# Fadi987/PL-BERT

Measured on AMD Instinct MI355X. Metric: phoneme-tokens/sec, higher is better.
Workload: dtype bf16; 1 GPU; PL-BERT masked-phoneme training step (fwd+loss+bwd+allreduce+AdamW), ALBERT hidden 768 / 12 shared layers / FFN 2048 / 12 heads, seq_len 512, batch 32 per GPU; global_batch=32, seq_len=512, parallelism=dp1

## Files before the change

plbert_amd/_lib.py:

```python
from __future__ import annotations

import ctypes as C
import os

import torch

HERE = os.path.dirname(os.path.abspath(__file__))
LIB_PATH = os.environ.get("PLBERT_HIP_LIB") or os.path.join(HERE, "libplbert_hip.so")

PLB_PARAM_NAMES = [
    "encoder.embeddings.word_embeddings.weight",
    "encoder.embeddings.position_embeddings.weight",
    "encoder.embeddings.token_type_embeddings.weight",
    "encoder.embeddings.LayerNorm.weight",
    "encoder.embeddings.LayerNorm.bias",
    "encoder.encoder.embedding_hidden_mapping_in.weight",
    "encoder.encoder.embedding_hidden_mapping_in.bias",
    "encoder.encoder.albert_layer_groups.0.albert_layers.0.full_layer_layer_norm.weight",
    "encoder.encoder.albert_layer_groups.0.albert_layers.0.full_layer_layer_norm.bias",
    "encoder.encoder.albert_layer_groups.0.albert_layers.0.attention.query.weight",
    "encoder.encoder.albert_layer_groups.0.albert_layers.0.attention.key.weight",
    "encoder.encoder.albert_layer_groups.0.albert_layers.0.attention.value.weight",
    "encoder.encoder.albert_layer_groups.0.albert_layers.0.attention.query.bias",
    "encoder.encoder.albert_layer_groups.0.albert_layers.0.attention.key.bias",
    "encoder.encoder.albert_layer_groups.0.albert_layers.0.attention.value.bias",
    "encoder.encoder.albert_layer_groups.0.albert_layers.0.attention.dense.weight",
    "encoder.encoder.albert_layer_groups.0.albert_layers.0.attention.dense.bias",
    "encoder.encoder.albert_layer_groups.0.albert_layers.0.attention.LayerNorm.weight",
    "encoder.encoder.albert_layer_groups.0.albert_layers.0.attention.LayerNorm.bias",
    "encoder.encoder.albert_layer_groups.0.albert_layers.0.ffn.weight",
    "encoder.encoder.albert_layer_groups.0.albert_layers.0.ffn.bias",
    "encoder.encoder.albert_layer_groups.0.albert_layers.0.ffn_output.weight",
    "encoder.encoder.albert_layer_groups.0.albert_layers.0.ffn_output.bias",
    "phoneme_predictor.weight",
    "phoneme_predictor.bias",
    "encoder.pooler.weight",
    "encoder.pooler.bias",
    "token_predictor.weight",
    "token_predictor.bias",
]
PLB_NPARAM = len(PLB_PARAM_NAMES)


class PlbConfig(C.Structure):
    _fields_ = [
        ("vocab_size", C.c_int32), ("embedding_size", C.c_int32), ("hidden_size", C.c_int32),
        ("num_attention_heads", C.c_int32), ("intermediate_size", C.c_int32), ("num_hidden_layers", C.c_int32),
        ("max_position_embeddings", C.c_int32), ("type_vocab_size", C.c_int32), ("layer_norm_eps", C.c_float),
        ("num_phonemes", C.c_int32), ("num_tokens", C.c_int32), ("max_batch", C.c_int32), ("max_seq", C.c_int32),
        ("inference_only", C.c_int32),
    ]


class PlbGemmNT(C.Structure):
    _fields_ = [
        ("A", C.c_void_p), ("lda", C.c_int), ("B", C.c_void_p), ("ldb", C.c_int),
        ("M", C.c_int), ("N", C.c_int), ("K", C.c_int), ("Mstore", C.c_int),
        ("bias", C.c_void_p), ("res", C.c_void_p), ("ldr", C.c_int), ("aux", C.c_void_p), ("ldaux", C.c_int),
        ("C", C.c_void_p), ("ldc", C.c_int), ("C2", C.c_void_p), ("ldc2", C.c_int), ("Cf", C.c_void_p), ("ldcf", C.c_int),
        ("colpart", C.c_void_p),
        ("ce_cols", C.c_int), ("ce_tgt", C.c_void_p), ("ce_pmax", C.c_void_p), ("ce_psum", C.c_void_p),
        ("ce_tlogit", C.c_void_p), ("ce_lse", C.c_void_p), ("ce_w", C.c_void_p),
        ("deq_a", C.c_void_p), ("deq_b", C.c_void_p), ("C8", C.c_void_p), ("ldc8", C.c_int), ("q_scale", C.c_void_p),
        ("q_amax", C.c_void_p), ("c8_bf8", C.c_int),
        ("ln_gamma", C.c_void_p), ("ln_beta", C.c_void_p), ("ln_mean", C.c_void_p), ("ln_rstd", C.c_void_p),
        ("ln_eps", C.c_float), ("ln_xchg", C.c_void_p), ("ln_err", C.c_void_p), ("ln_fault", C.c_int),
    ]


class PlbGemmTN(C.Structure):
    _fields_ = [
        ("A", C.c_void_p), ("lda", C.c_int), ("Ncols", C.c_int), ("B", C.c_void_p), ("ldb", C.c_int),
        ("Mtot", C.c_int), ("N", C.c_int), ("K", C.c_int), ("rows_per_split", C.c_int), ("splits", C.c_int),
        ("slab", C.c_void_p), ("deq_a", C.c_void_p), ("deq_b", C.c_void_p),
    ]


class PlbAttn(C.Structure):
    _fields_ = [
        ("qkv", C.c_void_p), ("ldqkv", C.c_int), ("lengths", C.c_void_p),
        ("B", C.c_int), ("S", C.c_int), ("NH", C.c_int), ("H", C.c_int), ("scale", C.c_float),
        ("ctx", C.c_void_p), ("ldctx", C.c_int), ("lse", C.c_void_p),
        ("dctx", C.c_void_p), ("lddctx", C.c_int), ("delta", C.c_void_p), ("dqkv", C.c_void_p), ("lddqkv", C.c_int),
        ("colpart", C.c_void_p), ("colpart_accumulate", C.c_int),
        ("ctx8", C.c_void_p), ("ldctx8", C.c_int), ("ctx_scale", C.c_void_p), ("ctx_amax", C.c_void_p),
        ("dqkv8", C.c_void_p), ("lddqkv8", C.c_int), ("dqkv_scale", C.c_void_p), ("dqkv_amax", C.c_void_p),
        ("qoff", C.c_void_p), ("q", C.c_void_p), ("ldq", C.c_int), ("nq_total", C.c_int), ("dq", C.c_void_p), ("lddq", C.c_int),
        ("dq8", C.c_void_p), ("lddq8", C.c_int),
        ("row_start", C.c_void_p),
    ]


class PlbEmbed(C.Structure):
    _fields_ = [
        ("ids", C.c_void_p), ("T", C.c_int), ("S", C.c_int), ("E", C.c_int), ("V", C.c_int),
        ("word", C.c_void_p), ("pos", C.c_void_p), ("type0", C.c_void_p), ("gamma", C.c_void_p), ("beta", C.c_void_p),
        ("eps", C.c_float), ("out", C.c_void_p), ("ldo", C.c_int), ("dout", C.c_void_p), ("lddo", C.c_int),
        ("dx", C.c_void_p), ("dword", C.c_void_p), ("dpos", C.c_void_p), ("partials", C.c_void_p), ("nblocks", C.c_int),
        ("row_start", C.c_void_p), ("lengths", C.c_void_p), ("B", C.c_int), ("fill_slots", C.c_int),
    ]


class PlbPacking(C.Structure):
    _fields_ = [("row_start", C.c_void_p), ("rows", C.c_int32), ("used", C.c_int32)]


class PlbMaskedReport(C.Structure):
    _fields_ = [
        ("pred", C.c_void_p), ("rank", C.c_void_p), ("nll", C.c_void_p), ("topk_ids", C.c_void_p), ("topk_logprob", C.c_void_p),
        ("logits", C.c_void_p), ("sample_loss", C.c_void_p), ("sample_top1", C.c_void_p), ("sample_topk", C.c_void_p),
        ("totals", C.c_void_p), ("token_totals", C.c_void_p),
    ]


class PlbLayerNorm(C.Structure):
    _fields_ = [
        ("x", C.c_void_p), ("ldx", C.c_int), ("gamma", C.c_void_p), ("beta", C.c_void_p), ("eps", C.c_float),
        ("y", C.c_void_p), ("ldy", C.c_int), ("mean", C.c_void_p), ("rstd", C.c_void_p),
        ("T", C.c_int), ("H", C.c_int), ("Tzero", C.c_int),
        ("dy", C.c_void_p), ("lddy", C.c_int), ("dx", C.c_void_p), ("lddx", C.c_int),
        ("partials", C.c_void_p), ("nblocks", C.c_int), ("accumulate", C.c_int),
        ("out8", C.c_void_p), ("ld8", C.c_int), ("q_scale", C.c_void_p), ("q_amax", C.c_void_p),
    ]


class PlbMask(C.Structure):
    _fields_ = [
        ("labels", C.c_void_p), ("lengths", C.c_void_p), ("B", C.c_int), ("S", C.c_int),
        ("seed", C.c_uint64), ("step", C.c_uint32),
        ("word_pred_prob", C.c_float), ("mask_prob", C.c_float), ("replace_prob", C.c_float),
        ("mask_id", C.c_int), ("sep_id", C.c_int),
        ("masked", C.c_void_p), ("counts", C.c_void_p), ("idx_padded", C.c_void_p), ("offsets", C.c_void_p),
        ("flat", C.c_void_p),
    ]


class PlbApplyMask(C.Structure):
    _fields_ = [
        ("ids", C.c_void_p), ("sample_off", C.c_void_p), ("word_off", C.c_void_p), ("word_begin", C.c_void_p),
        ("word_len", C.c_void_p), ("action", C.c_void_p), ("repl", C.c_void_p), ("word_token", C.c_void_p),
        ("sep_token", C.c_int64), ("crop_start", C.c_void_p), ("B", C.c_int), ("S", C.c_int), ("mask_id", C.c_int),
        ("labels", C.c_void_p), ("masked", C.c_void_p), ("tokens", C.c_void_p), ("lengths_out", C.c_void_p),
        ("counts", C.c_void_p), ("idx_padded", C.c_void_p), ("offsets", C.c_void_p), ("flat", C.c_void_p),
    ]


PLB_NORM_PARTS = 1024


def norm_chunk(n):
    return (n + PLB_NORM_PARTS * 1024 - 1) // (PLB_NORM_PARTS * 1024) * 1024


def norm_chain(n):
    return 4 * (norm_chunk(n) // 1024) + 6 + 3


vp, i32, u32, i64, u64, sz, f32, f64, P = (C.c_void_p, C.c_int32, C.c_uint32, C.c_int64, C.c_uint64, C.c_size_t, C.c_float,
                                           C.c_double, C.POINTER)
PUBLIC = {
    "plb_last_error": (C.c_char_p, []),
    "plb_create": (i32, [P(PlbConfig), P(vp)]),
    "plb_destroy": (None, [vp]),
    "plb_param_layout": (i32, [vp, P(i64), P(i64), P(i64), P(i64)]),
    "plb_workspace_bytes": (i64, [vp]),
    "plb_bind": (i32, [vp, vp, vp, vp, vp, vp, i64]),
    "plb_sync_weights": (i32, [vp, vp]),
    "plb_forward": (i32, [vp, vp, vp, i32, i32, vp, vp, vp, vp]),
    "plb_pooler": (i32, [vp, vp, i32, i32, vp, vp]),
    "plb_loss_fwd_bwd": (i32, [vp, vp, vp, vp, vp, vp, i32, i32, i32, vp, vp]),
    "plb_loss_fwd": (i32, [vp, vp, vp, vp, vp, vp, vp, i32, i32, i32, vp, vp, vp]),
    "plb_loss_fwd_bwd_dual": (i32, [vp, vp, vp, vp, vp, vp, vp, i32, i32, i32, vp, vp, vp]),
    "plb_adamw_step": (i32, [vp, f64, f64, f64, f64, f64, i32, f64, vp]),
    "plb_grad_norm_floats": (i64, [vp]),
    "plb_grad_accum_bind": (i32, [vp, vp]),
    "plb_grad_accum_add": (i32, [vp, i32, vp, vp]),
    "plb_grad_norm": (i32, [vp, f64, f64, vp, i32, vp]),
    "plb_adamw_step_clipped": (i32, [vp, f64, f64, f64, f64, f64, i32, f64, vp, vp]),
    "plb_set_fp8": (i32, [vp, i32, vp]),
    "plb_fp8_state": (i32, [vp, P(i32), P(i32)]),
    "plb_fp8_stats": (i32, [vp, P(f32), P(f32), vp]),
    "plb_token_head_steps": (i32, [vp]),
    "plb_set_token_head_steps": (i32, [vp, i32]),
    "plb_comm_unique_id": (i32, [vp]),
    "plb_comm_init": (i32, [vp, vp, i32, i32]),
    "plb_comm_destroy": (i32, [vp]),
    "plb_comm_info": (i32, [vp, P(i32), P(i32), P(i32)]),
    "plb_status": (i32, [vp, P(i32)]),
    "plb_status_ex": (i32, [vp, P(i32), P(i32)]),
    "plb_poll_status": (i32, [vp, P(i32)]),
    "plb_status_export": (i32, [vp, vp, vp]),
    "plb_status_import": (i32, [vp, vp, vp]),
    "plb_last_application_rows": (i32, [vp, P(i64), P(i64)]),
    "plb_packing_plan": (i32, [vp, i32, i32, vp, P(i32), P(i32)]),
    "plb_forward_packed": (i32, [vp, vp, vp, i32, i32, P(PlbPacking), vp, vp, vp, vp]),
    "plb_loss_fwd_bwd_packed": (i32, [vp, vp, vp, vp, vp, vp, i32, i32, i32, P(PlbPacking), vp, vp]),
    "plb_loss_fwd_packed": (i32, [vp, vp, vp, vp, vp, vp, vp, i32, i32, i32, P(PlbPacking), vp, vp, vp]),
    "plb_last_call_rows": (i32, [vp, P(i64), P(i64)]),
    "plb_set_packed_dual": (i32, [vp, i32]),
    "plb_loss_fwd_bwd_dual_packed": (i32, [vp, vp, vp, vp, vp, vp, vp, i32, i32, i32, P(PlbPacking), vp, vp, vp]),
    "plb_set_packed_fp8": (i32, [vp, i32]),
    "plb_encode": (i32, [vp, vp, vp, i32, i32, P(PlbPacking), vp, vp]),
    "plb_encode_bwd": (i32, [vp, vp, vp, i32, i32, P(PlbPacking), vp, vp]),
    "plb_masked_report": (i32, [vp, vp, i32, i32, P(PlbMaskedReport), vp]),
    "plb_comm_pieces": (i32, [vp, P(i32), P(i64)]),
    "plb_broadcast_params": (i32, [vp, i32, vp]),
    "plb_set_grad_overlap": (i32, [vp, i32]),
    "plb_allreduce_grads": (i32, [vp, vp]),
    "plb_apply_mask": (i32, [vp, vp, vp, vp, vp, vp, vp, vp, i64, vp, i32, i32, i32, vp, vp, vp, vp, vp, vp, vp, vp]),
    "plb_mask_batch": (i32, [vp, vp, i32, i32, u64, u32, f32, f32, f32, i32, i32, vp, vp, vp, vp, vp]),
    "plb_profile_enable": (None, [i32]),
    "plb_profile_num_classes": (i32, []),
    "plb_profile_class_name": (C.c_char_p, [i32]),
    "plb_profile_read": (i32, [P(f64), P(i64), P(f64), P(f64)]),
    "plb_debug_skip_piece": (None, [i32]),
    "plb_debug_ln_fault": (None, [i32, i32]),
    "plb_debug_hb_audit": (i32, [vp, i32, i32]),
    "plb_debug_hb_report": (i32, [vp, P(i64), P(i32), vp, i32]),
    "plb_comm_trace": (i32, [vp, i32]),
    "plb_comm_trace_read": (i32, [vp, i32, P(i32), P(i64), P(i64), P(f32), P(f32), P(f32)]),
    "plb_set_gemm_nt_tile": (None, [i32]),
    "plb_set_gemm_nt_prefetch": (None, [i32]),
    "plb_set_attn_bwd_fused": (None, [i32]),
    "plb_set_prune_last": (None, [i32]),
}
PUBLIC_SYMBOLS = list(PUBLIC)
INTERNAL = {
    **{name: PUBLIC[name] for name in ("plb_set_gemm_nt_tile", "plb_set_gemm_nt_prefetch", "plb_debug_skip_piece",
                                       "plb_debug_ln_fault", "plb_set_attn_bwd_fused")},
    "plb_prof_begin": (i32, [i32, vp, f64, f64]),
    "plb_prof_end": (None, [i32, vp]),
    "plb_launch_gemm_nt_ln": (i32, [P(PlbGemmNT), i32, vp]),
    "plb_launch_gemm_nt_gelud": (i32, [P(PlbGemmNT), i32, vp]),
    "plb_launch_gemm_nt_fp8": (i32, [P(PlbGemmNT), i32, i32, vp]),
    "plb_launch_gemm_nt_fp8_ln": (i32, [P(PlbGemmNT), i32, i32, vp]),
    "plb_launch_gemm_nt_fp8_gelud": (i32, [P(PlbGemmNT), i32, i32, vp]),
    "plb_gemm_nt_fp8_gelud_tile_rows": (i32, [i32]),
    "plb_ln_fault_take": (i32, []),
    "plb_launch_gemm_nt": (i32, [P(PlbGemmNT), i32, i32, vp]),
    "plb_launch_gemm_nt_big": (i32, [P(PlbGemmNT), i32, i32, i32, vp]),
    "plb_gemm_nt_colpart_rows": (i32, [i32, i32, i32]),
    "plb_launch_gemm_tn": (i32, [P(PlbGemmTN), vp]),
    "plb_launch_gemm_tn_fp8": (i32, [P(PlbGemmTN), vp]),
    "plb_launch_gemm_tn_big": (i32, [P(PlbGemmTN), vp]),
    "plb_launch_reduce_slabs": (i32, [vp, i32, sz, vp, i32, vp]),
    "plb_launch_embed_fwd": (i32, [P(PlbEmbed), vp]),
    "plb_launch_embed_bwd": (i32, [P(PlbEmbed), vp]),
    "plb_launch_embed_scatter": (i32, [P(PlbEmbed), i32, vp]),
    "plb_launch_amax": (i32, [vp, i32, sz, i32, i32, vp, vp]),
    "plb_launch_fp8_scales": (i32, [vp, vp, vp, i32, f32, i32, vp]),
    "plb_launch_fp8_scales2": (i32, [vp, vp, vp, i32, f32, i32, i32, f32, vp, i32, vp]),
    "plb_launch_quantize": (i32, [vp, i32, sz, i32, i32, vp, vp, i32, i32, vp]),
    "plb_launch_quantize_multi": (i32, [i32, vp, vp, vp, vp, vp, vp, vp]),
    "plb_launch_ln_fwd": (i32, [P(PlbLayerNorm), vp]),
    "plb_launch_ln_bwd": (i32, [P(PlbLayerNorm), vp]),
    "plb_launch_colsum": (i32, [vp, i32, sz, i32, i32, vp, i32, i32, vp, i32, vp]),
    "plb_launch_copy_cols": (i32, [vp, i32, i32, i32, i32, vp, vp]),
    "plb_launch_pooler": (i32, [vp, i32, i32, i32, vp, vp, vp, vp]),
    "plb_launch_attn_fwd": (i32, [P(PlbAttn), vp]),
    "plb_launch_attn_bwd": (i32, [P(PlbAttn), vp]),
    "plb_launch_attn_bwd_fused": (i32, [P(PlbAttn), vp]),
    "plb_launch_gather_rows": (i32, [vp, i32, vp, i32, i32, i32, vp, i32, vp]),
    "plb_launch_scatter_rows": (i32, [vp, i32, vp, i32, i32, vp, i32, vp]),
    "plb_launch_ce_prepare": (i32, [vp, vp, vp, i32, i32, vp, vp, vp, vp]),
    "plb_launch_ce_prepare_packed": (i32, [vp, vp, vp, i32, i32, vp, vp, vp, vp, vp]),
    "plb_launch_unpack_rows": (i32, [vp, i32, i32, vp, vp, i32, i32, i32, vp, vp]),
    "plb_launch_seed_dy": (i32, [vp, vp, vp, i32, i32, i32, i32, vp, vp]),
    "plb_launch_ce_fwd_bwd": (i32, [vp, i32, i32, vp, vp, i32, i32, vp, vp, i32, vp]),
    "plb_launch_sum_rows": (i32, [vp, i32, vp, vp]),
    "plb_launch_token_ce_combine": (i32, [vp, vp, i32, vp, vp, i32, i32, i32, vp, vp, vp, vp]),
    "plb_launch_token_ce_combine_packed": (i32, [vp, vp, i32, vp, vp, vp, i32, i32, i32, vp, vp, vp, vp]),
    "plb_launch_pack_token_targets": (i32, [vp, vp, vp, i32, i32, i32, vp, vp]),
    "plb_launch_add_scalar": (i32, [vp, vp, vp, vp]),
    "plb_launch_masked_report_rows": (i32, [vp, i32, i32, vp, i32, i32, vp, vp, vp, vp, vp, vp, vp]),
    "plb_launch_masked_report_samples": (i32, [vp, i32, vp, vp, i32, vp, vp, vp, vp, vp]),
    "plb_launch_token_top1": (i32, [vp, i32, vp, vp, i32, vp, vp, vp]),
    "plb_launch_mask": (i32, [P(PlbMask), vp]),
    "plb_launch_apply_mask": (i32, [P(PlbApplyMask), vp]),
    "plb_launch_adamw": (i32, [vp, vp, vp, vp, vp, sz, f64, f64, f64, f64, f64, i32, f64, vp, i32, vp]),
    "plb_launch_grad_accum": (i32, [vp, vp, sz, i32, vp, vp]),
    "plb_launch_grad_sumsq": (i32, [vp, sz, vp, vp]),
    "plb_launch_grad_norm_finish": (i32, [vp, i32, f64, f64, vp, vp]),
    "plb_launch_adamw_clipped": (i32, [vp, vp, vp, vp, vp, sz, f64, f64, f64, f64, f64, i32, f64, vp, i32, vp, i32, vp]),
    "plb_launch_step_status": (i32, [vp, vp, vp, vp, vp]),
    "plb_launch_status_export": (i32, [vp, vp, vp]),
    "plb_launch_cast_bf16": (i32, [vp, vp, sz, vp]),
    "plb_launch_transpose_cast": (i32, [vp, i32, i32, vp, i32, vp]),
    "plb_launch_transpose_cast_multi": (i32, [i32, vp, vp, vp, vp, vp, vp]),
    "plb_launch_bf16_to_f32": (i32, [vp, i32, vp, i32, i32, i32, vp]),
}


def declare(L):
    for name, (restype, argtypes) in {**PUBLIC, **INTERNAL}.items():
        fn = getattr(L, name, None)
        if fn is not None:
            fn.restype, fn.argtypes = restype, list(argtypes)
    return L


_lib = None


class HipLibraryMissing(RuntimeError):
    pass


def lib():
    global _lib
    if _lib is not None:
        return _lib
    if not os.path.exists(LIB_PATH):
        raise HipLibraryMissing(
            f"{LIB_PATH} is missing: build it with `python -m plbert_amd.build` (needs hipcc, gfx950). "
            "There is no CPU fallback for the PL-BERT hot path.")
    try:
        _lib = declare(C.CDLL(LIB_PATH, mode=C.RTLD_GLOBAL))
    except OSError as ex:
        raise HipLibraryMissing(f"cannot load {LIB_PATH}: {ex}") from ex
    return _lib


def profile_enable(on):
    lib().plb_profile_enable(int(bool(on)))


def profile_read():
    L = lib()
    n = L.plb_profile_num_classes()
    ms, fl, by = (C.c_double * n)(), (C.c_double * n)(), (C.c_double * n)()
    cnt = (C.c_int64 * n)()
    check(L.plb_profile_read(ms, cnt, fl, by), "plb_profile_read")
    return {L.plb_profile_class_name(i).decode(): dict(ms=ms[i], launches=int(cnt[i]), flops=fl[i], bytes=by[i])
            for i in range(n) if cnt[i]}


def check(rc, what):
    if rc != 0:
        msg = lib().plb_last_error().decode("utf-8", "replace")
        raise RuntimeError(f"{what} failed: {msg or 'rc=%d' % rc}")
```

plbert_amd/build.py:

```python
from __future__ import annotations

import os
import subprocess
import sys

HERE = os.path.dirname(os.path.abspath(__file__))
CSRC = os.path.join(HERE, "csrc")
LIB = os.path.join(HERE, "libplbert_hip.so")
SOURCES = ["gemm.hip", "gemm_big.hip", "gemm_fp8.hip", "gemm_fp8_ln.hip", "gemm_tn_fp8.hip", "gemm_ln.hip", "attn.hip", "attn_bwd_fused.hip", "mask.hip",
           "embed.hip", "layernorm.hip", "reduce.hip", "loss_rows.hip", "eval_rows.hip", "optim.hip", "operand_images.hip",
           "engine.cpp", "engine_prof.cpp", "engine_comm.cpp", "engine_fp8.cpp", "engine_layers.cpp", "engine_calls.cpp", "engine_eval.cpp", "engine_optim.cpp"]
HEADERS = ["exports.map", "common.h", "plbert_kernels.h", "gemm_epilogue.h", "gemm_nt_pipeline.h", "attn_common.h", "row_common.h", "engine_internal.h", os.path.join("..", "..", "include", "plbert.h")]
FLAGS = ["--offload-arch=gfx950", "-O3", "-std=c++17", "-fPIC", "-Wall", "-Wno-unused-function"]
_NO_SINK = ["-mllvm", "-disable-machine-sink"]
EXTRA_FLAGS = {"attn_bwd_fused.hip": ["-mllvm", "-amdgpu-mfma-vgpr-form=1"],
               "gemm_fp8.hip": _NO_SINK, "gemm_fp8_ln.hip": _NO_SINK, "gemm_tn_fp8.hip": _NO_SINK}


def _hipcc():
    for cand in (os.environ.get("HIPCC"), "/opt/rocm/bin/hipcc", "hipcc"):
        if cand and (os.path.isabs(cand) and os.path.exists(cand) or not os.path.isabs(cand)):
            return cand
    raise RuntimeError("hipcc not found")


def needs_build():
    if not os.path.exists(LIB):
        return True
    t = os.path.getmtime(LIB)
    deps = [os.path.join(CSRC, s) for s in SOURCES + HEADERS]
    return any(os.path.getmtime(d) > t for d in deps)


OBJDUMP = "/opt/rocm/lib/llvm/bin/llvm-objdump"


def disassemble_code_objects(lib, workdir):
    import glob
    import shutil
    cp = shutil.copy(lib, workdir)
    subprocess.run([OBJDUMP, "--offloading", cp], check=True, stdout=subprocess.PIPE, stderr=subprocess.STDOUT)
    cos = sorted(glob.glob(cp + ".*gfx950"))
    if not cos:
        raise RuntimeError("no gfx950 code object extracted from " + lib)
    for co in cos:
        yield co, subprocess.run([OBJDUMP, "-d", "--no-show-raw-insn", co], check=True, stdout=subprocess.PIPE,
                                 text=True).stdout


def verify_m0(lib=LIB, workdir=None):
    import re
    import tempfile
    if not os.path.exists(OBJDUMP):
        return None
    own = workdir is None
    tmp = tempfile.mkdtemp(prefix="plbert_m0_") if own else workdir
    n_asm = 0
    try:
        for co, text in disassemble_code_objects(lib, tmp):
            funcs, cur = {}, None
            for ln in text.splitlines():
                i = ln.split("//")[0].strip()
                m = re.match(r"^[0-9a-f]+ <(.+)>:$", i)
                if m:
                    cur = funcs.setdefault(m.group(1), [])
                elif cur is not None and i and not i.endswith(":"):
                    cur.append(i)
            for name, ins in funcs.items():
                def dma(i):
                    return i.startswith("global_load_lds") or (i.startswith("buffer_load") and i.rstrip().endswith("lds"))
                sig = [k for k in range(len(ins) - 2) if re.match(r"s_mov_b32 m0, s\d+$", ins[k]) and ins[k + 1] == "s_nop 0"
                       and dma(ins[k + 2]) and " s[" in ins[k + 2]]
                for i in ins:
                    if re.match(r"(s_movrel|v_movrel|ds_gws|ds_ordered|s_sendmsg|v_interp)", i):
                        raise RuntimeError(f"M0 check: {name}: instruction that reads M0: {i}")
                    if re.search(r"\bm0\b", i):
                        if not (re.match(r"s_\w+ m0, ", i) and not re.search(r"\bm0\b", i.split(",", 1)[1])):
                            raise RuntimeError(f"M0 check: {name}: M0 used as a source: {i}")
                if not sig:
                    continue
                n_asm += len(sig)
                owned = set(sig) | {k + 2 for k in sig}
                for k, i in enumerate(ins):
                    if (dma(i) or re.search(r"\bm0\b", i)) and k not in owned:
                        raise RuntimeError(f"M0 check: {name}: M0 / LDS-DMA outside the asm DMA statements: {ins[max(0, k - 2):k + 3]}")
    finally:
        if own:
            import shutil
            shutil.rmtree(tmp, ignore_errors=True)
    return n_asm


def build(force=False, verbose=True):
    if not force and not needs_build():
        return LIB
    hipcc = _hipcc()
    objdir = os.path.join(HERE, "build")
    os.makedirs(objdir, exist_ok=True)
    procs = []
    for src in SOURCES:
        obj = os.path.join(objdir, os.path.splitext(src)[0] + ".o")
        cmd = [hipcc, *FLAGS, *EXTRA_FLAGS.get(src, []), "-x", "hip", "-c", os.path.join(CSRC, src), "-o", obj]
        procs.append((src, obj, subprocess.Popen(cmd, stdout=subprocess.PIPE, stderr=subprocess.STDOUT, text=True)))
    objs = []
    for src, obj, p in procs:
        out, _ = p.communicate()
        if p.returncode != 0:
            raise RuntimeError(f"hipcc failed on {src}:\n{out}")
        if verbose and out.strip():
            print(out, file=sys.stderr)
        objs.append(obj)
    cmd = [hipcc, "--offload-arch=gfx950", "-shared", "-fPIC", "-Wl,--version-script=" + os.path.join(CSRC, "exports.map"),
           "-o", LIB, *objs]
    r = subprocess.run(cmd, stdout=subprocess.PIPE, stderr=subprocess.STDOUT, text=True)
    if r.returncode != 0:
        raise RuntimeError("link failed:\n" + r.stdout)
    try:
        verify_m0(LIB)
    except Exception:
        os.remove(LIB)
        raise
    return LIB


if __name__ == "__main__":
    print(build(force="--force" in sys.argv))
```

plbert_amd/csrc/engine_internal.h:

```cpp
#pragma once
#include <hip/hip_runtime.h>
#include <stdint.h>
#include <stdio.h>
#include <stdlib.h>
#include <string.h>

#include <array>
#include <map>
#include <string>
#include <vector>

#include "../../include/plbert.h"
#include "plbert_kernels.h"

#pragma GCC visibility push(hidden)

int fail(const char* fmt, ...);

static const unsigned kStreamOrderEvent = hipEventDisableTiming | hipEventReleaseToDevice;

inline int64_t rup(int64_t x, int64_t m) { return (x + m - 1) / m * m; }

#define TRY(x)                                                                    \
  do {                                                                            \
    int rc_ = (x);                                                                \
    if (rc_) return fail("%s failed (rc %d) at %s:%d", #x, rc_, __FILE__, __LINE__); \
  } while (0)
#define HIPTRY(x)                                                                                   \
  do {                                                                                              \
    hipError_t e_ = (x);                                                                            \
    if (e_ != hipSuccess) return fail("%s: %s at %s:%d", #x, hipGetErrorString(e_), __FILE__, __LINE__); \
  } while (0)
#define HB_R(stream, ptr, bytes, what) do { if (e->hb.on) e->hb.access(hb_idx(e, stream), (ptr), (size_t)(bytes), false, what); } while (0)
#define HB_W(stream, ptr, bytes, what) do { if (e->hb.on) e->hb.access(hb_idx(e, stream), (ptr), (size_t)(bytes), true, what); } while (0)

typedef void* RcclComm;

struct HbAudit {
  enum { MAIN = 0, SIDE = 1, COMM = 2, NS = 3 };
  typedef std::array<uint64_t, NS> VC;
  struct Acc { const char* what; uintptr_t a, b; int st; uint64_t tick; bool wr; };
  bool on = false;
  int break_wait = -1;
  int waits = 0;
  VC vc[NS] = {{0, 0, 0}, {0, 0, 0}, {0, 0, 0}};
  std::map<hipEvent_t, VC> ev;
  std::vector<Acc> log;
  int64_t checks = 0;
  int violations = 0;
  std::string first;
  static const char* name(int st) { return st == MAIN ? "main" : st == SIDE ? "side" : "comm"; }
  void record(hipEvent_t e, int st) { vc[st][st] += 1; ev[e] = vc[st]; }
  void wait(int st, hipEvent_t e);
  void access(int st, const void* p, size_t bytes, bool wr, const char* what);
  void new_call() { log.clear(); waits = 0; }
};

struct PlbEngine {
  PlbConfig c;
  int64_t poff[PLB_NPARAM], psize[PLB_NPARAM], ptotal, ptrain;
  int E, H, I, L, NH, V, P, NP, NT;
  int64_t Tcap;
  int64_t NMcap;
  int NTp = 0;
  bool infer = false;
  int qkvcol_rows = 0;
  int64_t slab2_floats;
  int64_t slab_floats;
  int64_t ws_bytes;
  int ln_blocks, emb_blocks;
  int part_rows = 0;
  int ln_fuse = 3;
  int64_t lnx_bytes = 0;
  bool gelu_dstash_on = true;
  bool fp8_tn = true;
  int f8n = 0;
  bool packed_dual = false;
  bool packed_fp8 = false;
  int64_t o_wbf, o_wqkvT, o_wdT, o_w1T, o_w2T, o_wpT, o_winT;
  int64_t o_e, o_x, o_qkv, o_ctx, o_pre1, o_a, o_u, o_g, o_pre2;
  int64_t o_lse, o_delta, o_mean1, o_rstd1, o_mean2, o_rstd2;
  int64_t o_dqkv, o_dpre1, o_du, o_dpre2;
  int64_t o_dy0, o_dy1, o_da, o_dctx, o_de;
  int64_t o_hm, o_logm, o_dlog, o_dhm, o_rows, o_tgt, o_w, o_lrows;
  int64_t o_slab, o_part1, o_part2, o_parte, o_scratch, o_dxe, o_ducol, o_slab2, o_scratch2, o_qkvcol = 0;
  int64_t o_lnx = 0, o_lnerr = 0;
  int64_t o_rep_rank = 0, o_rep_nll = 0, o_rep_tok = 0;
  int64_t o_bt = 0, o_wtT = 0, o_tdl = 0, o_tlrows = 0, o_tscr = 0, o_tgrad = 0, o_tloss = 0;
  int64_t o_tpmax = 0, o_tpsum = 0, o_ttl = 0, o_tlse = 0, o_tw = 0, o_ttgt = 0, o_tcolp = 0;
  int64_t o_x8 = 0, o_a8 = 0, o_g8 = 0, o_c8 = 0, o_dp8 = 0, o_du8 = 0, o_dp18 = 0, o_dq8 = 0;
  int64_t o_wq8 = 0, o_wd8 = 0, o_w18 = 0, o_w28 = 0, o_w2T8 = 0, o_w1T8 = 0, o_wqT8 = 0, o_wdT8 = 0;
  int64_t o_f8amax = 0, o_f8scale = 0, o_f8deq = 0, o_f8stats = 0;
  bool fp8_on = false, fp8_ready = false, fp8_bwd_ready = false, fp8_wstale = true;
  bool u_is_derivative = false;
  bool tn8_call = false;
  int part_rows_used = 0;
  int pruned_rows = 0;
  int64_t last_app_rows[2] = {0, 0};
  int64_t last_exec_rows[2] = {0, 0};
  bool tok_grads_live = false;
  bool head_grads_live = true;
  bool tok_pad_zeroed = false;
  int tok_steps = 0;
  bool rep_valid = false, rep_dual = false;
  int rep_n = 0, rep_B = 0;
  int64_t rep_tok_rows = 0;
  float* accum = nullptr;
  bool grads_fresh = false;
  bool win_open = false;
  const char* win_closed_by = "no FIRST add has opened one";
  bool win_head = false, win_tok = false;
  bool win_reduced = false;
  const float* norm_src = nullptr;
  int norm_nparts = 0;
  bool norm_reduced = false;
  bool stash_live = false;
  const char* stash_dead_by = "no plb_encode has run on this engine";
  int stash_B = 0, stash_S = 0;
  int64_t stash_rows = 0, stash_used = 0;
  const int32_t* stash_row_start = nullptr;
  RcclComm comm = nullptr;
  int comm_rank = 0, comm_world = 1;
  hipStream_t comm_stream = nullptr;
  hipEvent_t ev_piece = nullptr, ev_comm_done = nullptr;
  bool overlap = true;
  bool comm_pending = false;
  bool grads_reduced = false;
  int64_t piece_floats = 0;
  int32_t piece_count = 0;
  hipEvent_t ev_status = nullptr;
  bool status_pending = false;
  int32_t status_collectives = 0;
  float* last_loss = nullptr;
  HbAudit hb;
  struct PieceTrace { int64_t a, b; hipEvent_t released, done; };
  bool trace_on = false;
  std::vector<PieceTrace> trace;
  std::vector<hipEvent_t> trace_pool;
  hipEvent_t tr_call0 = nullptr, tr_tail0 = nullptr, tr_tail1 = nullptr;
  bool tr_tail_valid = false;
  hipStream_t side = nullptr;
  hipEvent_t ev_fork = nullptr, ev_join = nullptr;
  unsigned int* host_err = nullptr;
  unsigned int* host_err_dev = nullptr;
  float *params = nullptr, *grads = nullptr, *m = nullptr, *v = nullptr;
  char* ws = nullptr;

  template <typename T>
  T* at(int64_t off) const { return reinterpret_cast<T*>(ws + off); }
  bf16_t* wbf(int which) const { return at<bf16_t>(o_wbf) + poff[which]; }
  float* par(int which) const { return params + poff[which]; }
  float* grd(int which) const { return grads + poff[which]; }
};

enum { F8_X = 0, F8_A, F8_G, F8_C, F8_DP, F8_DU, F8_DP1, F8_DQ, F8_NSITE };
enum { F8_AMAX_WORDS = 64 * 16 };
enum { F8W_QKV = 0, F8W_D, F8W_1, F8W_2, F8W_2T, F8W_1T, F8W_QKVT, F8W_DT, F8W_N };

struct Rows {
  const int32_t* row_start;
  int T; int64_t Tp;
};

struct F8Site {
  float* scale = nullptr;
  float* amax = nullptr;
  float* deq = nullptr;
  F8Site() = default;
  F8Site(const PlbEngine* e, int kind, int l);
};
struct F8Weight {
  const uint8_t* img;
  const float* deq;
  F8Weight(const PlbEngine* e, int w);
};

struct F8Op { const uint8_t* A8; const uint8_t* B8; const float* deq_a; const float* deq_b; int a_bf8; };

struct Slots {
  bf16_t *x, *y;
  bf16_t *qkv, *ctx, *pre1, *a, *u, *g, *pre2;
  float *mean1, *rstd1, *mean2, *rstd2, *lse;
  uint8_t *x8, *x8n, *c8, *a8, *g8;
  bf16_t *dqkv, *dpre1, *du, *dpre2;
  uint8_t *dp8, *du8, *dp18, *dq8;
  float *part1, *part2, *qkvcol, *ducol;
};

struct LnSlot { const float* gamma; const float* beta; const bf16_t* pre; float* mean; float* rstd; float* partials; };

struct Prune { const int32_t* rows; int n; int Mc; };

struct Bwd {
  const int32_t* lengths;
  const int32_t* row_start;
  int B, S, T;
  int64_t Tp;
  bool f8, calib;
  bool fuse_b;
  int prows;
  int du_rows;
  hipStream_t s;
};

enum { kPieceHead = 0, kPieceQkvW, kPieceFfnW, kPieceSmall, kPieceFfnoW = kPieceSmall + 5, kPieceDenseW, kNPieces };

int hb_idx(const PlbEngine* e, hipStream_t s);
hipError_t ev_record(PlbEngine* e, hipEvent_t ev, hipStream_t s);
hipError_t ev_wait(PlbEngine* e, hipStream_t s, hipEvent_t ev);
int reduce_piece(PlbEngine* e, int64_t a, int64_t b, hipStream_t after);
bool overlapping(const PlbEngine* e);
int pieces_done(PlbEngine* e);
int64_t piece_begin(const PlbEngine* e, int i);
int64_t piece_end(const PlbEngine* e, int i);
int reduce_pieces(PlbEngine* e, int from, int to, hipStream_t after);
int status_exchange(PlbEngine* e, hipStream_t s);
int status_finish(PlbEngine* e, float* loss, hipStream_t s);
int f8_site(const PlbEngine* e, int site, int l);
float* f8_deq(const PlbEngine* e, int i);
int fp8_quantize_weights(PlbEngine* e, hipStream_t s, bool exact = true);
int fp8_update_scales(PlbEngine* e, hipStream_t s);
bool f8_call(const PlbEngine* e, int64_t Tp, bool train);
bool tn8_ok(const PlbEngine* e, int64_t Mtot);
PlbGemmNT nt_desc(const bf16_t* A, const bf16_t* B, int64_t M, int N, int K);
int qkvcol_rows(int B, int S);
Slots slots(const PlbEngine* e, int64_t Tp, int B, int S, int l, bool stash, int prows = 0, int du_rows = 0);
bool prune_enabled();
int run_encoder(PlbEngine* e, const int64_t* ids, const int32_t* lengths, int B, int S, const Rows& rw, bool stash,
                bf16_t** xout, hipStream_t s, const Prune* pr = nullptr);
int tn_splits(int64_t Mtot, int N, int K, int* rows_per_split);
int weight_grad(PlbEngine* e, const bf16_t* A, int lda, int Ncols, const bf16_t* Bm, int ldb, int64_t Mtot, int N,
                int K, float* out, hipStream_t s, bool side_slab = false);
int weight_grad8(PlbEngine* e, const uint8_t* A8, const uint8_t* B8, int64_t Mtot, int N, int K, int site_a, int site_b,
                 float* out, hipStream_t s);
int encoder_bwd(PlbEngine* e, const Prune* pr, const int32_t* lengths, int B, int S, const Rows& rw, bf16_t** dy,
                int* du_rows, hipStream_t s);
void drop_stash(PlbEngine* e, const char* by);
int sync_transposes(PlbEngine* e, hipStream_t s, bool exact_fp8 = true);
void end_accum_window(PlbEngine* e, const char* by);

#pragma GCC visibility pop
```

plbert_amd/csrc/engine_layers.cpp:

```cpp
#include "engine_internal.h"

static bool tn_big(int64_t Mtot, int Ncols, int K) { return Ncols % 256 == 0 && K % 256 == 0 && Mtot >= 8192; }
static bool tn_fill_chip() {
  static const bool v = [] { const char* e = getenv("PLBERT_TN_SPLITS"); return !(e && !strcmp(e, "xcd")); }();
  return v;
}
static int tn_cus() {
  static const int v = [] {
    const char* e = getenv("PLBERT_TN_CUS");
    const int n = e ? atoi(e) : 256;
    return (n >= 64 && n <= 256) ? n : 256;
  }();
  return v;
}
int tn_splits(int64_t Mtot, int N, int K, int* rows_per_split) {
  const bool big = tn_big(Mtot, N, K);
  const int tiles = big ? (N / 256) * (K / 256) : ((N + 127) / 128) * ((K + 127) / 128);
  int splits = 768 / tiles;
  if (big) {
    int s = 32 / tiles;
    if (s < 1) s = 1;
    splits = tiles >= 256 ? 1 : (tn_fill_chip() ? (tn_cus() / tiles > 0 ? tn_cus() / tiles : 1) : 8 * s);
  }
  const int64_t maxs = Mtot / 64;
  if (splits > maxs) splits = (int)maxs;
  if (splits < 1) splits = 1;
  int64_t rps = rup((Mtot + splits - 1) / splits, 64);
  splits = (int)((Mtot + rps - 1) / rps);
  *rows_per_split = (int)rps;
  return splits;
}

PlbGemmNT nt_desc(const bf16_t* A, const bf16_t* B, int64_t M, int N, int K) {
  PlbGemmNT g;
  memset(&g, 0, sizeof(g));
  g.A = A; g.lda = K; g.B = B; g.ldb = K; g.M = (int)M; g.N = N; g.K = K; g.Mstore = (int)M;
  return g;
}

static F8Op f8_op(const uint8_t* a8, const F8Site& a, const F8Weight& w, int a_bf8) { return F8Op{a8, w.img, a.deq, w.deq, a_bf8}; }
static PlbGemmNT f8_operands(const PlbGemmNT* g, const F8Op* f8) {
  PlbGemmNT q = *g;
  q.A = reinterpret_cast<const bf16_t*>(f8->A8); q.B = reinterpret_cast<const bf16_t*>(f8->B8);
  q.deq_a = f8->deq_a; q.deq_b = f8->deq_b;
  return q;
}
static int gemm_nt_any(PlbGemmNT* g, int act, const F8Op* f8, hipStream_t s) {
  if (!f8) return plb_launch_gemm_nt(g, act, 0, s);
  PlbGemmNT q = f8_operands(g, f8);
  return plb_launch_gemm_nt_fp8(&q, act, f8->a_bf8, s);
}
static int gemm_nt_ln_any(PlbGemmNT* g, int mode, const F8Op* f8, hipStream_t s) {
  if (!f8) return plb_launch_gemm_nt_ln(g, mode, s);
  PlbGemmNT q = f8_operands(g, f8);
  return plb_launch_gemm_nt_fp8_ln(&q, mode, f8->a_bf8, s);
}
static int gemm_nt_gelud_any(PlbGemmNT* g, int backward, const F8Op* f8, hipStream_t s) {
  if (!f8) return plb_launch_gemm_nt_gelud(g, backward, s);
  PlbGemmNT q = f8_operands(g, f8);
  return plb_launch_gemm_nt_fp8_gelud(&q, backward, f8->a_bf8, s);
}
static void f8_out(PlbGemmNT* g, uint8_t* img, int ld, const F8Site& q, int bf8) {
  g->C8 = img; g->ldc8 = ld; g->q_scale = q.scale; g->q_amax = q.amax; g->c8_bf8 = bf8;
}

int qkvcol_rows(int B, int S) { return B * ((S + 127) / 128) * 4; }
Slots slots(const PlbEngine* e, int64_t Tp, int B, int S, int l, bool stash, int prows, int du_rows) {
  const int64_t H = e->H, I = e->I, sl = stash ? l : 0;
  auto bf = [&](int64_t off, int64_t width) { return e->at<bf16_t>(off) + sl * Tp * width; };
  auto u8 = [&](int64_t off, int64_t width) { return e->at<uint8_t>(off) + sl * Tp * width; };
  auto f32 = [&](int64_t off, int64_t per_layer) { return e->at<float>(off) + sl * per_layer; };
  Slots v;
  memset(&v, 0, sizeof(v));
  v.x = e->at<bf16_t>(e->o_x) + (int64_t)(stash ? l : l & 1) * Tp * H;
  v.y = e->at<bf16_t>(e->o_x) + (int64_t)(stash ? l + 1 : (l + 1) & 1) * Tp * H;
  v.qkv = bf(e->o_qkv, 3 * H); v.ctx = bf(e->o_ctx, H); v.pre1 = bf(e->o_pre1, H); v.a = bf(e->o_a, H);
  v.u = bf(e->o_u, I); v.g = bf(e->o_g, I); v.pre2 = bf(e->o_pre2, H);
  v.mean1 = f32(e->o_mean1, Tp); v.rstd1 = f32(e->o_rstd1, Tp); v.mean2 = f32(e->o_mean2, Tp); v.rstd2 = f32(e->o_rstd2, Tp);
  v.lse = f32(e->o_lse, (int64_t)B * e->NH * S);
  v.x8 = u8(e->o_x8, H); v.c8 = u8(e->o_c8, H); v.a8 = u8(e->o_a8, H); v.g8 = u8(e->o_g8, I);
  v.x8n = e->at<uint8_t>(e->o_x8) + (stash ? l + 1 : 0) * Tp * H;
  if (stash) {
    v.dqkv = bf(e->o_dqkv, 3 * H); v.dpre1 = bf(e->o_dpre1, H); v.du = bf(e->o_du, I); v.dpre2 = bf(e->o_dpre2, H);
    v.dp8 = u8(e->o_dp8, H); v.du8 = u8(e->o_du8, I); v.dp18 = u8(e->o_dp18, H); v.dq8 = u8(e->o_dq8, 3 * H);
    v.part1 = f32(e->o_part1, (int64_t)prows * 3 * H); v.part2 = f32(e->o_part2, (int64_t)prows * 3 * H);
    v.qkvcol = f32(e->o_qkvcol, (int64_t)qkvcol_rows(B, S) * 3 * H); v.ducol = f32(e->o_ducol, (int64_t)du_rows * I);
  }
  return v;
}

static bool ln_fusable(const PlbEngine* e, int64_t Tp, int bit) {
  const int H = e->H;
  return (e->ln_fuse & bit) && Tp % 1024 == 0 && (H % 384 == 0 ? H / 384 : H % 256 == 0 ? H / 256 : 99) <= 4;
}
static bool gelu_dstash(PlbEngine* e, int64_t Tp, bool f8_call) {
  e->u_is_derivative = e->gelu_dstash_on && (f8_call ? Tp % 128 == 0 : Tp % 256 == 0) && e->I % 256 == 0;
  return e->u_is_derivative;
}
static void ln_fields(const PlbEngine* e, PlbGemmNT* g, const float* gamma, const float* beta, float* mean, float* rstd) {
  g->ln_gamma = gamma; g->ln_beta = beta; g->ln_mean = mean; g->ln_rstd = rstd; g->ln_eps = e->c.layer_norm_eps;
  g->ln_xchg = e->at<unsigned long long>(e->o_lnx); g->ln_err = e->at<unsigned int>(e->o_lnerr);
}
static LnSlot ln1_slot(const PlbEngine* e, const Slots& v) {
  return LnSlot{e->par(PLB_LN1_W), e->par(PLB_LN1_B), v.pre1, v.mean1, v.rstd1, v.part1};
}
static LnSlot ln2_slot(const PlbEngine* e, const Slots& v) {
  return LnSlot{e->par(PLB_LN2_W), e->par(PLB_LN2_B), v.pre2, v.mean2, v.rstd2, v.part2};
}
static int gemm_ln_fwd(PlbEngine* e, PlbGemmNT* g, const F8Op* f8, bool fused, const LnSlot& ln, bf16_t* y, int T,
                       uint8_t* y8, const F8Site& q, hipStream_t s) {
  const int H = e->H;
  if (fused) {
    g->C2 = y; g->ldc2 = H;
    ln_fields(e, g, ln.gamma, ln.beta, ln.mean, ln.rstd);
    if (y8) f8_out(g, y8, H, q, 0);
    TRY(gemm_nt_ln_any(g, 5, f8, s));
    return 0;
  }
  TRY(gemm_nt_any(g, 0, f8, s));
  PlbLayerNorm p;
  memset(&p, 0, sizeof(p));
  p.x = g->C; p.ldx = H; p.gamma = ln.gamma; p.beta = ln.beta; p.eps = e->c.layer_norm_eps;
  p.y = y; p.ldy = H; p.T = T; p.H = H; p.mean = ln.mean; p.rstd = ln.rstd;
  if (y8) { p.out8 = y8; p.ld8 = H; p.q_scale = q.scale; p.q_amax = q.amax; }
  TRY(plb_launch_ln_fwd(&p, s));
  return 0;
}
static int ln_bwd(PlbEngine* e, const LnSlot& ln, int nblocks, const bf16_t* dy, bf16_t* dx, int T, int Tzero, uint8_t* dx8,
                  const F8Site& q, hipStream_t s) {
  const int H = e->H;
  PlbLayerNorm p;
  memset(&p, 0, sizeof(p));
  p.x = ln.pre; p.ldx = H; p.gamma = ln.gamma; p.T = T; p.H = H; p.Tzero = Tzero; p.mean = ln.mean; p.rstd = ln.rstd;
  p.dy = dy; p.lddy = H; p.dx = dx; p.lddx = H; p.partials = ln.partials; p.nblocks = nblocks;
  if (dx8) { p.out8 = dx8; p.ld8 = H; p.q_scale = q.scale; p.q_amax = q.amax; }
  TRY(plb_launch_ln_bwd(&p, s));
  return 0;
}
static int gemm_ln_bwd(PlbEngine* e, PlbGemmNT* g, const F8Op* f8, bool fused, const LnSlot& ln, int nblocks, bf16_t* dx, int T,
                       int Tzero, uint8_t* dx8, const F8Site& q, hipStream_t s) {
  if (fused) {
    g->C = dx; g->aux = ln.pre; g->ldaux = e->H; g->colpart = ln.partials;
    ln_fields(e, g, ln.gamma, nullptr, ln.mean, ln.rstd);
    if (dx8) f8_out(g, dx8, e->H, q, 1);
    TRY(gemm_nt_ln_any(g, 6, f8, s));
    return 0;
  }
  TRY(gemm_nt_any(g, 0, f8, s));
  return ln_bwd(e, ln, nblocks, g->C, dx, T, Tzero, dx8, q, s);
}

static int g_prune_last = -1;
extern "C" void plb_set_prune_last(int on) { g_prune_last = on < 0 ? -1 : (on ? 1 : 0); }
bool prune_enabled() {
  static const bool v = [] { const char* e = getenv("PLBERT_PRUNE_LAST"); return !(e && !strcmp(e, "0")); }();
  return g_prune_last < 0 ? v : g_prune_last != 0;
}
static int last_application_fwd_pruned(PlbEngine* e, const Prune* pr, bool stash, bool calib, bool tn8, const Slots& sl,
                                       const bf16_t* ctx_att, hipStream_t s) {
  const int H = e->H, I = e->I, L = e->L, Mc = pr->Mc, n = pr->n;
  const F8Site sA(e, F8_A, L - 1), sG(e, F8_G, L - 1), sC(e, F8_C, L - 1);
  bf16_t* ctxc = stash ? sl.ctx : sl.pre1;
  bf16_t* xc = stash ? e->at<bf16_t>(e->o_da) : sl.a;
  bf16_t* pre1c = stash ? sl.pre1 : sl.ctx;
  bf16_t* ac = stash ? sl.a : sl.pre1;
  TRY(plb_launch_gather_rows(ctx_att, H, pr->rows, n, Mc, H, ctxc, H, s));
  TRY(plb_launch_gather_rows(sl.x, H, pr->rows, n, Mc, H, xc, H, s));
  PlbGemmNT g = nt_desc(ctxc, e->wbf(PLB_DENSE_W), Mc, H, H);
  g.bias = e->par(PLB_DENSE_B); g.res = xc; g.ldr = H; g.C = pre1c; g.ldc = H;
  const LnSlot ln1 = {e->par(PLB_LN1_W), e->par(PLB_LN1_B), pre1c, sl.mean1, sl.rstd1, nullptr};
  if (gemm_ln_fwd(e, &g, nullptr, false, ln1, ac, Mc, nullptr, F8Site(), s)) return 1;
  if (calib) TRY(plb_launch_amax(ac, 1, (size_t)n, H, H, sA.amax, s));
  g = nt_desc(ac, e->wbf(PLB_FFN_W), Mc, I, H);
  g.bias = e->par(PLB_FFN_B); g.C = sl.u; g.ldc = I; g.C2 = sl.g; g.ldc2 = I;
  TRY(plb_launch_gemm_nt(&g, 1, 0, s));
  if (calib) TRY(plb_launch_amax(sl.g, 1, (size_t)n, I, I, sG.amax, s));
  g = nt_desc(sl.g, e->wbf(PLB_FFNO_W), Mc, H, I);
  g.bias = e->par(PLB_FFNO_B); g.res = ac; g.ldr = H; g.C = sl.pre2; g.ldc = H;
  if (gemm_ln_fwd(e, &g, nullptr, false, ln2_slot(e, sl), e->at<bf16_t>(e->o_hm), Mc, nullptr, F8Site(), s)) return 1;
  if (tn8) {
    const void* src[3] = {ctxc, ac, sl.g}; const int fl[3] = {1, 1, 1};
    const size_t nel[3] = {(size_t)Mc * H, (size_t)Mc * H, (size_t)Mc * I};
    const float* sc[3] = {sC.scale, sA.scale, sG.scale};
    uint8_t* dst[3] = {sl.c8, sl.a8, sl.g8};
    float* am[3] = {sC.amax, sA.amax, sG.amax};
    TRY(plb_launch_quantize_multi(3, src, fl, nel, sc, dst, am, s));
  }
  return 0;
}

int run_encoder(PlbEngine* e, const int64_t* ids, const int32_t* lengths, int B, int S, const Rows& rw, bool stash,
                       bf16_t** xout, hipStream_t s, const Prune* pr) {
  const int E = e->E, H = e->H, I = e->I, L = e->L;
  const int T = rw.T;
  const int64_t Tp = rw.Tp;
  const bool f8 = f8_call(e, Tp, stash);
  const bool calib = e->fp8_on && !f8;
  const int T8 = (f8 && rw.row_start) ? (int)Tp : T;
  if (e->fp8_on && e->fp8_wstale) TRY(fp8_quantize_weights(e, s));
  PlbEmbed em;
  memset(&em, 0, sizeof(em));
  em.ids = ids; em.T = T; em.S = S; em.E = E; em.V = e->V;
  em.word = e->par(PLB_WORD_EMB); em.pos = e->par(PLB_POS_EMB); em.type0 = e->par(PLB_TYPE_EMB);
  em.gamma = e->par(PLB_EMB_LN_W); em.beta = e->par(PLB_EMB_LN_B); em.eps = e->c.layer_norm_eps;
  em.out = e->at<bf16_t>(e->o_e); em.ldo = E;
  if (rw.row_start) {
    em.row_start = rw.row_start; em.lengths = lengths; em.B = B; em.T = (int)Tp;
    em.fill_slots = e->fp8_on;
  }
  TRY(plb_launch_embed_fwd(&em, s));

  const Slots first = slots(e, Tp, B, S, 0, stash);
  PlbGemmNT g = nt_desc(em.out, e->wbf(PLB_MAP_W), Tp, H, E);
  g.bias = e->par(PLB_MAP_B); g.C = first.x; g.ldc = H;
  TRY(plb_launch_gemm_nt(&g, 0, 0, s));
  if (f8) {
    const F8Site sX(e, F8_X, 0);
    const void* src1[1] = {first.x}; const int bf1[1] = {1}; const size_t n1[1] = {(size_t)T8 * H};
    const float* sc1[1] = {sX.scale}; uint8_t* dst1[1] = {first.x8}; float* am1[1] = {sX.amax};
    TRY(plb_launch_quantize_multi(1, src1, bf1, n1, sc1, dst1, am1, s));
  }
  const bool fuse_f = ln_fusable(e, Tp, 1);
  const bool dstash = gelu_dstash(e, Tp, f8);
  if (stash) e->tn8_call = f8 && e->fp8_tn && dstash && tn8_ok(e, (int64_t)L * Tp);
  const bool tn8 = stash && e->tn8_call;

  for (int l = 0; l < L; ++l) {
    const Slots sl = slots(e, Tp, B, S, l, stash);
    const F8Site sX(e, F8_X, l), sA(e, F8_A, l), sG(e, F8_G, l), sC(e, F8_C, l);
    if (calib) TRY(plb_launch_amax(sl.x, 1, (size_t)T, H, H, sX.amax, s));
    g = nt_desc(sl.x, e->wbf(PLB_Q_W), Tp, 3 * H, H);
    g.bias = e->par(PLB_Q_B); g.C = sl.qkv; g.ldc = 3 * H;
    const F8Op oq = f8_op(sl.x8, sX, F8Weight(e, F8W_QKV), 0);
    TRY(gemm_nt_any(&g, 0, f8 ? &oq : nullptr, s));
    PlbAttn at;
    memset(&at, 0, sizeof(at));
    at.qkv = sl.qkv; at.ldqkv = 3 * H; at.lengths = lengths; at.B = B; at.S = S; at.NH = e->NH; at.H = H;
    at.row_start = rw.row_start;
    const bool pruned_layer = pr != nullptr && l == L - 1;
    bf16_t* const ctx_att = (pruned_layer && stash) ? e->at<bf16_t>(e->o_dy1) : sl.ctx;
    at.scale = 0.125f; at.ctx = ctx_att; at.ldctx = H; at.lse = sl.lse;
    if (f8 && !pruned_layer) { at.ctx8 = sl.c8; at.ldctx8 = H; at.ctx_scale = sC.scale; at.ctx_amax = sC.amax; }
    if (rw.row_start && e->fp8_on && S % 128) {
      HIPTRY(hipMemsetAsync(ctx_att, 0, (size_t)T * H * 2, s));
      if (at.ctx8) HIPTRY(hipMemsetAsync(sl.c8, 0, (size_t)T * H, s));
    }
    TRY(plb_launch_attn_fwd(&at, s));
    if (rw.row_start && Tp > T) {
      HIPTRY(hipMemsetAsync(ctx_att + (int64_t)T * H, 0, (size_t)(Tp - T) * H * 2, s));
      if (at.ctx8) HIPTRY(hipMemsetAsync(sl.c8 + (int64_t)T * H, 0, (size_t)(Tp - T) * H, s));
    }
    if (calib) TRY(plb_launch_amax(ctx_att, 1, (size_t)T, H, H, sC.amax, s));
    if (pruned_layer) {
      if (last_application_fwd_pruned(e, pr, stash, calib, tn8, sl, ctx_att, s)) return 1;
      *xout = e->at<bf16_t>(e->o_hm);
      break;
    }
    g = nt_desc(sl.ctx, e->wbf(PLB_DENSE_W), Tp, H, H);
    g.bias = e->par(PLB_DENSE_B); g.res = sl.x; g.ldr = H; g.C = sl.pre1; g.ldc = H;
    const F8Op od = f8_op(sl.c8, sC, F8Weight(e, F8W_D), 0);
    if (gemm_ln_fwd(e, &g, f8 ? &od : nullptr, fuse_f, ln1_slot(e, sl), sl.a, T8, f8 ? sl.a8 : nullptr, sA, s)) return 1;
    if (calib) TRY(plb_launch_amax(sl.a, 1, (size_t)T, H, H, sA.amax, s));
    g = nt_desc(sl.a, e->wbf(PLB_FFN_W), Tp, I, H);
    g.bias = e->par(PLB_FFN_B); g.C = sl.u; g.ldc = I; g.C2 = sl.g; g.ldc2 = I;
    if (f8) f8_out(&g, sl.g8, I, sG, 0);
    const F8Op o1 = f8_op(sl.a8, sA, F8Weight(e, F8W_1), 0);
    if (dstash) {
      if (tn8) { g.C2 = nullptr; g.ldc2 = 0; }
      TRY(gemm_nt_gelud_any(&g, 0, f8 ? &o1 : nullptr, s));
    } else {
      TRY(gemm_nt_any(&g, 1, f8 ? &o1 : nullptr, s));
    }
    if (calib) TRY(plb_launch_amax(sl.g, 1, (size_t)T, I, I, sG.amax, s));
    g = nt_desc(sl.g, e->wbf(PLB_FFNO_W), Tp, H, I);
    g.bias = e->par(PLB_FFNO_B); g.res = sl.a; g.ldr = H; g.C = sl.pre2; g.ldc = H;
    const F8Op o2 = f8_op(sl.g8, sG, F8Weight(e, F8W_2), 0);
    const bool next8 = f8 && l + 1 < L;
    if (gemm_ln_fwd(e, &g, f8 ? &o2 : nullptr, fuse_f, ln2_slot(e, sl), sl.y, T8, next8 ? sl.x8n : nullptr,
                    next8 ? F8Site(e, F8_X, l + 1) : F8Site(), s))
      return 1;
    *xout = sl.y;
  }
  return 0;
}

int weight_grad(PlbEngine* e, const bf16_t* A, int lda, int Ncols, const bf16_t* Bm, int ldb, int64_t Mtot, int N,
                       int K, float* out, hipStream_t s, bool side_slab) {
  PlbGemmTN t;
  memset(&t, 0, sizeof(t));
  t.A = A; t.lda = lda; t.Ncols = Ncols; t.B = Bm; t.ldb = ldb; t.Mtot = (int)Mtot; t.N = N; t.K = K;
  t.splits = tn_splits(Mtot, N, K, &t.rows_per_split);
  const bool direct = t.splits == 1 && N == Ncols;
  if (!direct && (int64_t)t.splits * N * K > (side_slab ? e->slab2_floats : e->slab_floats)) return fail("weight_grad: slab too small");
  t.slab = direct ? out : e->at<float>(side_slab ? e->o_slab2 : e->o_slab);
  if (N == Ncols && tn_big(Mtot, Ncols, K)) {
    const int tok = plb_prof_begin(PLB_K_GEMM_TN, s, 2.0 * (double)Mtot * N * K, 0.0);
    TRY(plb_launch_gemm_tn_big(&t, s));
    plb_prof_end(tok, s);
  } else {
    TRY(plb_launch_gemm_tn(&t, s));
  }
  if (!direct) TRY(plb_launch_reduce_slabs(t.slab, t.splits, (size_t)N * K, out, 0, s));
  return 0;
}

int weight_grad8(PlbEngine* e, const uint8_t* A8, const uint8_t* B8, int64_t Mtot, int N, int K, int site_a, int site_b,
                        float* out, hipStream_t s) {
  PlbGemmTN t;
  memset(&t, 0, sizeof(t));
  t.A = reinterpret_cast<const bf16_t*>(A8); t.lda = N; t.Ncols = N; t.B = reinterpret_cast<const bf16_t*>(B8); t.ldb = K;
  t.Mtot = (int)Mtot; t.N = N; t.K = K;
  t.splits = tn_splits(Mtot, N, K, &t.rows_per_split);
  t.rows_per_split = (int)rup(t.rows_per_split, 128);
  t.splits = (int)((Mtot + t.rows_per_split - 1) / t.rows_per_split);
  if ((int64_t)t.splits * N * K > e->slab_floats) return fail("weight_grad8: slab too small");
  t.slab = e->at<float>(e->o_slab);
  t.deq_a = f8_deq(e, f8_site(e, site_a, 0)); t.deq_b = f8_deq(e, f8_site(e, site_b, 0));
  const int tok = plb_prof_begin(PLB_K_GEMM_TN_FP8, s, 2.0 * (double)Mtot * N * K, 0.0);
  TRY(plb_launch_gemm_tn_fp8(&t, s));
  plb_prof_end(tok, s);
  TRY(plb_launch_reduce_slabs(t.slab, t.splits, (size_t)N * K, out, 0, s));
  return 0;
}

static int post_attention_bwd(PlbEngine* e, const Bwd& c, int l, const Slots& sl, const bf16_t* dy) {
  const int H = e->H, I = e->I, T = c.T, Tp = (int)c.Tp;
  hipStream_t s = c.s;
  const F8Site sDP(e, F8_DP, l), sDU(e, F8_DU, l), sDP1(e, F8_DP1, l);
  if (l == e->L - 1 && ln_bwd(e, ln2_slot(e, sl), c.prows, dy, sl.dpre2, T, Tp, c.f8 ? sl.dp8 : nullptr, sDP, s)) return 1;
  if (c.calib) TRY(plb_launch_amax(sl.dpre2, 1, (size_t)T, H, H, sDP.amax, s));
  PlbGemmNT g = nt_desc(sl.dpre2, e->at<bf16_t>(e->o_w2T), Tp, I, H);
  g.aux = sl.u; g.ldaux = I; g.C = sl.du; g.ldc = I;
  if (c.du_rows > 0) g.colpart = sl.ducol;
  if (c.f8) f8_out(&g, sl.du8, I, sDU, 1);
  const F8Op ou = f8_op(sl.dp8, sDP, F8Weight(e, F8W_2T), 1);
  if (e->u_is_derivative) {
    if (e->tn8_call) g.C = nullptr;
    TRY(gemm_nt_gelud_any(&g, 1, c.f8 ? &ou : nullptr, s));
  } else {
    TRY(gemm_nt_any(&g, 2, c.f8 ? &ou : nullptr, s));
  }
  if (c.calib) TRY(plb_launch_amax(sl.du, 1, (size_t)T, I, I, sDU.amax, s));
  g = nt_desc(sl.du, e->at<bf16_t>(e->o_w1T), Tp, H, I);
  g.res = sl.dpre2; g.ldr = H; g.C = e->at<bf16_t>(e->o_da); g.ldc = H;
  const F8Op oa = f8_op(sl.du8, sDU, F8Weight(e, F8W_1T), 1);
  if (gemm_ln_bwd(e, &g, c.f8 ? &oa : nullptr, c.fuse_b, ln1_slot(e, sl), c.prows, sl.dpre1, T, Tp, c.f8 ? sl.dp18 : nullptr,
                  sDP1, s))
    return 1;
  if (c.calib) TRY(plb_launch_amax(sl.dpre1, 1, (size_t)T, H, H, sDP1.amax, s));
  g = nt_desc(sl.dpre1, e->at<bf16_t>(e->o_wdT), Tp, H, H);
  g.C = e->at<bf16_t>(e->o_dctx); g.ldc = H;
  const F8Op oc = f8_op(sl.dp18, sDP1, F8Weight(e, F8W_DT), 1);
  TRY(gemm_nt_any(&g, 0, c.f8 ? &oc : nullptr, s));
  return 0;
}

static int last_application_bwd_pruned(PlbEngine* e, const Bwd& c, const Slots& sl, const Prune* pr) {
  const int H = e->H, I = e->I, L = e->L, Mc = pr->Mc, n = pr->n;
  hipStream_t s = c.s;
  const F8Site sDP(e, F8_DP, L - 1), sDU(e, F8_DU, L - 1), sDP1(e, F8_DP1, L - 1);
  bf16_t* const dac = e->at<bf16_t>(e->o_da);
  bf16_t* const dctxc = e->at<bf16_t>(e->o_dy0);
  bf16_t* const dctx = e->at<bf16_t>(e->o_dctx);
  if (ln_bwd(e, ln2_slot(e, sl), c.prows, e->at<bf16_t>(e->o_dhm), sl.dpre2, Mc, Mc, nullptr, F8Site(), s)) return 1;
  if (c.calib) TRY(plb_launch_amax(sl.dpre2, 1, (size_t)n, H, H, sDP.amax, s));
  PlbGemmNT g = nt_desc(sl.dpre2, e->at<bf16_t>(e->o_w2T), Mc, I, H);
  g.aux = sl.u; g.ldaux = I; g.C = sl.du; g.ldc = I;
  TRY(plb_launch_gemm_nt(&g, 2, 0, s));
  if (c.calib) TRY(plb_launch_amax(sl.du, 1, (size_t)n, I, I, sDU.amax, s));
  if (c.du_rows > 0) {
    TRY(plb_launch_colsum(sl.du, 1, (size_t)Mc, I, I, sl.ducol, I, 0, e->at<float>(e->o_scratch), 16, s));
    if (c.du_rows > 1) HIPTRY(hipMemsetAsync(sl.ducol + I, 0, (size_t)(c.du_rows - 1) * I * 4, s));
  }
  g = nt_desc(sl.du, e->at<bf16_t>(e->o_w1T), Mc, H, I);
  g.res = sl.dpre2; g.ldr = H; g.C = dac; g.ldc = H;
  if (gemm_ln_bwd(e, &g, nullptr, false, ln1_slot(e, sl), c.prows, sl.dpre1, Mc, Mc, nullptr, F8Site(), s)) return 1;
  if (c.calib) TRY(plb_launch_amax(sl.dpre1, 1, (size_t)n, H, H, sDP1.amax, s));
  if (e->tn8_call) {
    const void* src[3] = {sl.dpre2, sl.du, sl.dpre1}; const int fl[3] = {3, 3, 3};
    const size_t nel[3] = {(size_t)Mc * H, (size_t)Mc * I, (size_t)Mc * H};
    const float* sc[3] = {sDP.scale, sDU.scale, sDP1.scale};
    uint8_t* dst[3] = {sl.dp8, sl.du8, sl.dp18};
    float* am[3] = {sDP.amax, sDU.amax, sDP1.amax};
    TRY(plb_launch_quantize_multi(3, src, fl, nel, sc, dst, am, s));
  }
  g = nt_desc(sl.dpre1, e->at<bf16_t>(e->o_wdT), Mc, H, H);
  g.C = dctxc; g.ldc = H;
  TRY(plb_launch_gemm_nt(&g, 0, 0, s));
  HIPTRY(hipMemsetAsync(dctx, 0, (size_t)c.Tp * H * 2, s));
  TRY(plb_launch_scatter_rows(dctxc, H, pr->rows, n, H, dctx, H, s));
  HIPTRY(hipMemsetAsync(dac, 0, (size_t)c.Tp * H * 2, s));
  TRY(plb_launch_scatter_rows(sl.dpre1, H, pr->rows, n, H, dac, H, s));
  return 0;
}

static int attention_bwd_dx(PlbEngine* e, const Bwd& c, int l, const Slots& sl, bf16_t* ctx, const bf16_t* res,
                            bf16_t* dx) {
  const int H = e->H, T = c.T;
  hipStream_t s = c.s;
  const F8Site sDQ(e, F8_DQ, l);
  PlbAttn at;
  memset(&at, 0, sizeof(at));
  at.qkv = sl.qkv; at.ldqkv = 3 * H; at.lengths = c.lengths; at.B = c.B; at.S = c.S; at.NH = e->NH; at.H = H; at.scale = 0.125f;
  at.row_start = c.row_start;
  at.ctx = ctx; at.ldctx = H; at.lse = sl.lse;
  at.dctx = e->at<bf16_t>(e->o_dctx); at.lddctx = H; at.delta = e->at<float>(e->o_delta); at.dqkv = sl.dqkv; at.lddqkv = 3 * H;
  at.colpart = sl.qkvcol; at.colpart_accumulate = 0;
  if (c.f8) {
    at.dqkv8 = sl.dq8; at.lddqkv8 = 3 * H; at.dqkv_scale = sDQ.scale; at.dqkv_amax = sDQ.amax;
    if (e->tn8_call) at.dqkv = nullptr;
  }
  if (c.row_start && c.S % 128 && at.dqkv) HIPTRY(hipMemsetAsync(sl.dqkv, 0, (size_t)T * 3 * H * 2, s));
  if (c.row_start && c.S % 128 && at.dqkv8) HIPTRY(hipMemsetAsync(sl.dq8, 0, (size_t)T * 3 * H, s));
  TRY(plb_launch_attn_bwd(&at, s));
  if (c.Tp > T) {
    if (at.dqkv) HIPTRY(hipMemsetAsync(sl.dqkv + (int64_t)T * 3 * H, 0, (size_t)(c.Tp - T) * 3 * H * 2, s));
    if (c.f8) HIPTRY(hipMemsetAsync(sl.dq8 + (int64_t)T * 3 * H, 0, (size_t)(c.Tp - T) * 3 * H, s));
  }
  if (c.calib) TRY(plb_launch_amax(sl.dqkv, 1, (size_t)T, 3 * H, 3 * H, sDQ.amax, s));
  PlbGemmNT g = nt_desc(sl.dqkv, e->at<bf16_t>(e->o_wqkvT), c.Tp, H, 3 * H);
  g.res = res; g.ldr = H; g.C = dx; g.ldc = H;
  const F8Op ox = f8_op(sl.dq8, sDQ, F8Weight(e, F8W_QKVT), 1);
  if (l == 0) {
    TRY(gemm_nt_any(&g, 0, c.f8 ? &ox : nullptr, s));
    return 0;
  }
  const Slots below = slots(e, c.Tp, c.B, c.S, l - 1, true, c.prows, c.du_rows);
  return gemm_ln_bwd(e, &g, c.f8 ? &ox : nullptr, c.fuse_b, ln2_slot(e, below), c.prows, below.dpre2, T, (int)c.Tp,
                     c.f8 ? below.dp8 : nullptr, F8Site(e, F8_DP, l - 1), s);
}

int encoder_bwd(PlbEngine* e, const Prune* pr, const int32_t* lengths, int B, int S, const Rows& rw, bf16_t** dy,
                       int* du_rows, hipStream_t s) {
  const int I = e->I, L = e->L;
  Bwd c;
  c.lengths = lengths; c.row_start = rw.row_start; c.B = B; c.S = S; c.T = rw.T; c.Tp = rw.Tp; c.s = s;
  const int Tp = (int)c.Tp;
  c.f8 = f8_call(e, Tp, true);
  c.calib = e->fp8_on && !c.f8;
  c.du_rows = e->u_is_derivative ? (c.f8 ? 2 * (Tp / plb_gemm_nt_fp8_gelud_tile_rows(Tp)) : 2 * (Tp / 256))
                                 : (c.f8 ? 2 * (Tp / 128) : plb_gemm_nt_colpart_rows(Tp, I, e->H));
  c.fuse_b = ln_fusable(e, Tp, 2);
  c.prows = c.fuse_b ? 2 * Tp / 128 : e->ln_blocks;
  e->part_rows_used = c.prows;
  bf16_t* dx = e->at<bf16_t>(e->o_dy1);
  for (int l = L - 1; l >= 0; --l) {
    const Slots sl = slots(e, c.Tp, B, S, l, true, c.prows, c.du_rows);
    if (pr && l == L - 1) {
      if (last_application_bwd_pruned(e, c, sl, pr)) return 1;
      if (attention_bwd_dx(e, c, l, sl, e->at<bf16_t>(e->o_dy1), e->at<bf16_t>(e->o_da), dx)) return 1;
    } else {
      if (post_attention_bwd(e, c, l, sl, *dy)) return 1;
      if (attention_bwd_dx(e, c, l, sl, sl.ctx, sl.dpre1, dx)) return 1;
    }
    bf16_t* tmp = *dy; *dy = dx; dx = tmp;
  }
  *du_rows = c.du_rows;
  return 0;
}
```

plbert_amd/csrc/gemm.hip:

```cpp
#include "common.h"
#include "plbert_kernels.h"
#include "gemm_epilogue.h"

namespace {

constexpr int BM = 128, BN = 128, BK = 64;

DEVI int nt_lds_off(int row, int chunk) { return row * BK + ((chunk ^ ((row >> 1) & 7)) << 3); }

template <int ACT, bool OUTF32>
__global__ __launch_bounds__(256) void gemm_nt_kernel(PlbGemmNT p) {
  __shared__ __attribute__((aligned(16))) bf16_t smem[2][2][BM * BK];
  const int tid = threadIdx.x, lane = tid & 63, wave = tid >> 6;
  const int wr = wave >> 1, wc = wave & 1;
  const int nbn = (p.N + BN - 1) / BN;
  const int nwg = gridDim.x;
  const int logical = xcd_remap(blockIdx.x, nwg);
  const int bm = logical / nbn, bn = logical % nbn;

  const int uw = __builtin_amdgcn_readfirstlane(wave);
  const int drow = lane >> 3, dch = lane & 7;
  const bf16_t* gA = p.A + (size_t)(bm * BM + uw * 32 + drow) * p.lda;
  const bf16_t* gB = p.B + (size_t)(bn * BN + uw * 32 + drow) * p.ldb;
  const size_t sa = (size_t)8 * p.lda, sb = (size_t)8 * p.ldb;
  int sch[4];
#pragma unroll
  for (int i = 0; i < 4; ++i) sch[i] = (dch ^ ((4 * i + (lane >> 4)) & 7)) * 8;
  typedef __attribute__((address_space(1))) const void* gptr_t;
  typedef __attribute__((address_space(3))) void* lptr_t;
#define NT_STAGE(st, kt)                                                                              \
  do {                                                                                                \
    _Pragma("unroll") for (int i = 0; i < 4; ++i) {                                                   \
      __builtin_amdgcn_global_load_lds((gptr_t)(gA + i * sa + (size_t)(kt) * BK + sch[i]),            \
                                       (lptr_t)&smem[st][0][(uw * 32 + i * 8) * BK], 16, 0, 0);       \
      __builtin_amdgcn_global_load_lds((gptr_t)(gB + i * sb + (size_t)(kt) * BK + sch[i]),            \
                                       (lptr_t)&smem[st][1][(uw * 32 + i * 8) * BK], 16, 0, 0);       \
    }                                                                                                 \
  } while (0)
#define NT_LANDED() asm volatile("s_waitcnt vmcnt(0)" ::: "memory")

  f32x4 acc[4][4];
#pragma unroll
  for (int i = 0; i < 4; ++i)
#pragma unroll
    for (int j = 0; j < 4; ++j) acc[i][j] = f32x4{0.f, 0.f, 0.f, 0.f};

  const int frow = lane & 15, fq = lane >> 4;
  const int fsw = (frow >> 1) & 7;
  const int offA = (wr * 64 + frow) * BK, offB = (wc * 64 + frow) * BK;
#define NT_COMPUTE(st)                                                                                   \
  do {                                                                                                   \
    const bf16_t* sA = smem[st][0];                                                                      \
    const bf16_t* sB = smem[st][1];                                                                      \
    _Pragma("unroll") for (int kk = 0; kk < 2; ++kk) {                                                   \
      const int ch = ((kk * 4 + fq) ^ fsw) << 3;                                                         \
      bf16x8 af[4], bfr[4];                                                                              \
      _Pragma("unroll") for (int i = 0; i < 4; ++i) {                                                    \
        af[i] = *(const bf16x8*)&sA[offA + i * 16 * BK + ch];                                            \
        bfr[i] = *(const bf16x8*)&sB[offB + i * 16 * BK + ch];                                           \
      }                                                                                                  \
      _Pragma("unroll") for (int mi = 0; mi < 4; ++mi)                                                   \
        _Pragma("unroll") for (int ni = 0; ni < 4; ++ni)                                                 \
          acc[mi][ni] = __builtin_amdgcn_mfma_f32_16x16x32_bf16(bfr[ni], af[mi], acc[mi][ni], 0, 0, 0);  \
    }                                                                                                    \
  } while (0)

  const int nk = p.K / BK;
  NT_STAGE(0, 0);
  NT_LANDED();
  __syncthreads();
  for (int kt = 0; kt < nk; ++kt) {
    const int cur = kt & 1;
    if (kt + 1 < nk) NT_STAGE(cur ^ 1, kt + 1);
    NT_COMPUTE(cur);
    NT_LANDED();
    __syncthreads();
  }
#undef NT_STAGE
#undef NT_LANDED
#undef NT_COMPUTE

#pragma unroll
  for (int mi = 0; mi < 4; ++mi) {
    const int m = bm * BM + wr * 64 + mi * 16 + frow;
#pragma unroll
    for (int ni = 0; ni < 4; ++ni)
      nt_epilogue<ACT, OUTF32>(p, acc[mi][ni], m, bn * BN + wc * 64 + ni * 16 + fq * 4);
  }
}

DEVI int tn_unit(int t) { return (t & 3) | (((t >> 3) & 1) << 2) | (((t >> 2) & 1) << 3) | (t & 48); }
DEVI int tn_lds_off(int t, int col) {
  int s = col >> 4;
  return s * 1024 + (((tn_unit(t) + s) & 63) << 4) + (col & 15);
}

__global__ __launch_bounds__(256) void gemm_tn_kernel(PlbGemmTN p) {
  __shared__ __attribute__((aligned(16))) bf16_t smem[2][2][64 * 128];
  const int tid = threadIdx.x, lane = tid & 63, wave = tid >> 6;
  const int wn = wave >> 1, wk = wave & 1;
  const int nbk = (p.K + 127) / 128;
  const int bn = blockIdx.x / nbk, bk = blockIdx.x % nbk;
  const int split = blockIdx.y;
  const int t_begin = split * p.rows_per_split;
  int t_end = t_begin + p.rows_per_split;
  if (t_end > p.Mtot) t_end = p.Mtot;
  const int nt = (t_end - t_begin) / 64;

  const int lc = tid & 15, lr = tid >> 4;
  const int colA = bn * 128 + lc * 8, colB = bk * 128 + lc * 8;
  const bool okA = colA < p.Ncols, okB = colB < p.K;
  uint4 ra[4], rb[4];
  auto load_tile = [&](int it) {
    const size_t t0 = (size_t)t_begin + (size_t)it * 64 + lr;
#pragma unroll
    for (int i = 0; i < 4; ++i) {
      ra[i] = okA ? *(const uint4*)(p.A + (t0 + 16 * i) * p.lda + colA) : make_uint4(0, 0, 0, 0);
      rb[i] = okB ? *(const uint4*)(p.B + (t0 + 16 * i) * p.ldb + colB) : make_uint4(0, 0, 0, 0);
    }
  };
  auto store_tile = [&](int st) {
#pragma unroll
    for (int i = 0; i < 4; ++i) {
      int off = tn_lds_off(lr + 16 * i, lc * 8);
      *(uint4*)&smem[st][0][off] = ra[i];
      *(uint4*)&smem[st][1][off] = rb[i];
    }
  };

  f32x4 acc[4][4];
#pragma unroll
  for (int i = 0; i < 4; ++i)
#pragma unroll
    for (int j = 0; j < 4; ++j) acc[i][j] = f32x4{0.f, 0.f, 0.f, 0.f};

  const int g = lane >> 4, li = lane & 15, q = li >> 2, pp = li & 3;
  if (nt > 0) {
    load_tile(0);
    store_tile(0);
  }
  __syncthreads();
  for (int it = 0; it < nt; ++it) {
    const int cur = it & 1;
    if (it + 1 < nt) load_tile(it + 1);
    const bf16_t* sA = smem[cur][0];
    const bf16_t* sB = smem[cur][1];
#pragma unroll
    for (int ks = 0; ks < 2; ++ks) {
      const int t0 = ks * 32 + 8 * g + q;
      bf16x8 af[4], bfr[4];
#pragma unroll
      for (int i = 0; i < 4; ++i) {
        const int ca = wn * 64 + i * 16 + 4 * pp, cb = wk * 64 + i * 16 + 4 * pp;
        s16x4 a0 = lds_read_tr16(&sA[tn_lds_off(t0, ca)]);
        s16x4 a1 = lds_read_tr16(&sA[tn_lds_off(t0 + 4, ca)]);
        s16x4 b0 = lds_read_tr16(&sB[tn_lds_off(t0, cb)]);
        s16x4 b1 = lds_read_tr16(&sB[tn_lds_off(t0 + 4, cb)]);
        af[i] = bf16x8{a0[0], a0[1], a0[2], a0[3], a1[0], a1[1], a1[2], a1[3]};
        bfr[i] = bf16x8{b0[0], b0[1], b0[2], b0[3], b1[0], b1[1], b1[2], b1[3]};
      }
#pragma unroll
      for (int ni = 0; ni < 4; ++ni)
#pragma unroll
        for (int ki = 0; ki < 4; ++ki)
          acc[ni][ki] = __builtin_amdgcn_mfma_f32_16x16x32_bf16(bfr[ki], af[ni], acc[ni][ki], 0, 0, 0);
    }
    if (it + 1 < nt) store_tile(cur ^ 1);
    __syncthreads();
  }

  float* out = p.slab + (size_t)split * p.N * p.K;
#pragma unroll
  for (int ni = 0; ni < 4; ++ni) {
    const int n = bn * 128 + wn * 64 + ni * 16 + li;
    if (n >= p.N) continue;
#pragma unroll
    for (int ki = 0; ki < 4; ++ki) {
      const int k0 = bk * 128 + wk * 64 + ki * 16 + 4 * g;
      if (k0 >= p.K) continue;
      f32x4 v = acc[ni][ki];
      *(float4*)(out + (size_t)n * p.K + k0) = make_float4(v[0], v[1], v[2], v[3]);
    }
  }
}

}

static int g_nt_tile = 0;
extern "C" void plb_set_gemm_nt_tile(int tile) { g_nt_tile = tile; }

static int pick_tile(const PlbGemmNT* p) {
  const bool ok256 = p->M % 256 == 0 && p->N % 256 == 0, ok384 = p->M % 128 == 0 && p->N % 384 == 0;
  const bool ok1256 = p->M % 128 == 0 && p->N % 256 == 0;
  if (g_nt_tile == 128) return 128;
  if (g_nt_tile == 256) return ok256 ? 256 : 128;
  if (g_nt_tile == 384) return ok384 ? 384 : (ok256 ? 256 : 128);
  if (g_nt_tile == 1256) return ok1256 ? 1256 : 128;
  if ((long)p->M * p->N < 256L * 256 * 64) return 128;
  double e256 = 0, e384 = 0, e1256 = 0;
  if (ok256) { const long t = (long)(p->M / 256) * (p->N / 256); e256 = (double)t / (double)(((t + 255) / 256) * 256); }
  if (ok384) { const long t = (long)(p->M / 128) * (p->N / 384); e384 = 0.95 * (double)t / (double)(((t + 255) / 256) * 256); }
  if (ok1256) { const long t = (long)(p->M / 128) * (p->N / 256); e1256 = 0.85 * (double)t / (double)(((t + 255) / 256) * 256); }
  if (e256 == 0 && e384 == 0 && e1256 == 0) return 128;
  if (e1256 > e256 && e1256 > e384) return 1256;
  return e384 > e256 ? 384 : 256;
}

extern "C" int plb_gemm_nt_colpart_rows(int M, int N, int K) {
  PlbGemmNT q;
  q.M = M; q.N = N; q.K = K;
  const int tile = pick_tile(&q);
  return tile == 256 ? 2 * (M / 256) : (tile == 384 || tile == 1256) ? 2 * (M / 128) : 0;
}

extern "C" int plb_launch_gemm_nt(const PlbGemmNT* p, int act, int out_f32, hipStream_t stream) {
  if (p->M % BM || p->K % BK || p->N % 4 || p->M <= 0 || p->N <= 0 || p->K <= 0) return 1;
  const int nbn = (p->N + BN - 1) / BN;
  dim3 grid((p->M / BM) * nbn), block(256);
  const int cls = out_f32 ? PLB_K_GEMM_NT_F32 : act == 1 ? PLB_K_GEMM_NT_GELU : act == 2 ? PLB_K_GEMM_NT_GELUBWD : PLB_K_GEMM_NT;
  const int tile = pick_tile(p);
  if (p->colpart && tile == 128) return 1;
  const double mnk = (double)p->M * p->N * p->K;
  const double algo_bytes = 2.0 * ((double)p->M * p->K + (double)p->N * p->K) +
                            (double)p->M * p->N * (out_f32 ? 4 : act == 1 ? 4 : 2) +
                            (p->res ? 2.0 * p->M * p->N : 0.0) + (act == 2 ? 2.0 * p->M * p->N : 0.0);
  if (tile != 128) {
    const int tokb = plb_prof_begin(cls, stream, 2.0 * mnk, algo_bytes);
    const int rc = plb_launch_gemm_nt_big(p, tile, act, out_f32, stream);
    plb_prof_end(tokb, stream);
    return rc;
  }
  const int tok = plb_prof_begin(out_f32 ? PLB_K_GEMM_NT_F32 : PLB_K_GEMM_NT_SMALL, stream, 2.0 * mnk, algo_bytes);
  if (out_f32) {
    if (act != 0) return 1;
    hipLaunchKernelGGL((gemm_nt_kernel<0, true>), grid, block, 0, stream, *p);
  } else if (act == 0) {
    hipLaunchKernelGGL((gemm_nt_kernel<0, false>), grid, block, 0, stream, *p);
  } else if (act == 1) {
    hipLaunchKernelGGL((gemm_nt_kernel<1, false>), grid, block, 0, stream, *p);
  } else if (act == 2) {
    hipLaunchKernelGGL((gemm_nt_kernel<2, false>), grid, block, 0, stream, *p);
  } else {
    return 1;
  }
  plb_prof_end(tok, stream);
  return hipGetLastError() == hipSuccess ? 0 : 2;
}

extern "C" int plb_launch_gemm_tn(const PlbGemmTN* p, hipStream_t stream) {
  if (p->Mtot % 64 || p->rows_per_split % 64 || p->K % 4 || p->N <= 0 || p->splits <= 0) return 1;
  if ((long)p->splits * p->rows_per_split < p->Mtot) return 1;
  dim3 grid(((p->N + 127) / 128) * ((p->K + 127) / 128), p->splits), block(256);
  const int tok = plb_prof_begin(PLB_K_GEMM_TN, stream, 2.0 * p->Mtot * (double)p->N * p->K,
                                 2.0 * p->Mtot * ((double)p->N + p->K) + 4.0 * p->splits * (double)p->N * p->K);
  hipLaunchKernelGGL(gemm_tn_kernel, grid, block, 0, stream, *p);
  plb_prof_end(tok, stream);
  return hipGetLastError() == hipSuccess ? 0 : 2;
}
```

plbert_amd/csrc/gemm_big.hip:

```cpp
#include "gemm_nt_pipeline.h"

namespace {

template <int V, bool PF>
int launch_big(const PlbGemmNT* p, int act, int out_f32, hipStream_t stream) {
  constexpr int TM = (V == 2 ? 2 : 1) * 128, TN = (V == 3 ? 3 : 2) * 128;
  if (p->M % TM || p->N % TN || p->K % 64 || p->M <= 0 || p->N <= 0 || p->K <= 0) return 1;
  dim3 grid((p->M / TM) * (p->N / TN)), block(512);
  if (out_f32) {
    if (act != 0) return 1;
    hipLaunchKernelGGL((gemm_nt_big_kernel<V, 0, true, PF>), grid, block, 0, stream, *p);
  } else if (act == 0) {
    if (p->colpart) hipLaunchKernelGGL((gemm_nt_big_kernel<V, 0, false, PF>), grid, block, 0, stream, *p);
    else hipLaunchKernelGGL((gemm_nt_big_kernel<V, 0, false, PF, false, false, true>), grid, block, 0, stream, *p);
  } else if (act == 1) {
    hipLaunchKernelGGL((gemm_nt_big_kernel<V, 1, false, PF>), grid, block, 0, stream, *p);
  } else if (act == 2) {
    hipLaunchKernelGGL((gemm_nt_big_kernel<V, 2, false, PF>), grid, block, 0, stream, *p);
  } else if (act == 3 || act == 4) {
    if constexpr (TN == 256) {
      if (!p->ce_tgt || p->ce_cols < 1 || p->ce_cols > p->N) return 1;
      if (act == 3) {
        if (!p->ce_pmax || !p->ce_psum || !p->ce_tlogit) return 1;
        hipLaunchKernelGGL((gemm_nt_big_kernel<V, 3, false, PF>), grid, block, 0, stream, *p);
      } else {
        if (!p->ce_lse || !p->ce_w || !p->C) return 1;
        hipLaunchKernelGGL((gemm_nt_big_kernel<V, 4, false, PF>), grid, block, 0, stream, *p);
      }
    } else {
      return 1;
    }
  } else {
    return 1;
  }
  return hipGetLastError() == hipSuccess ? 0 : 2;
}

DEVI int tn_g(int row) { return ((row >> 1) & 1) | (((row >> 3) & 1) << 1); }

__global__ __launch_bounds__(512) __attribute__((amdgpu_num_vgpr(224))) void gemm_tn_big_kernel(PlbGemmTN p) {
  __shared__ __attribute__((aligned(16))) bf16_t smem[2 * 4 * HT];
  const int tid = threadIdx.x, lane = tid & 63;
  const int uw = __builtin_amdgcn_readfirstlane(tid >> 6);
  const int wm = uw >> 2, wn = uw & 3;
  const int nbk = p.K >> 8;
  const int tiles = (p.Ncols >> 8) * nbk;
  const int logical = xcd_remap(blockIdx.x, gridDim.x);
  const int split = logical / tiles, tile = logical % tiles;
  const int bn = tile / nbk, bk = tile % nbk;
  const int t_begin = split * p.rows_per_split;
  int t_end = t_begin + p.rows_per_split;
  if (t_end > p.Mtot) t_end = p.Mtot;
  const int nk = (t_end - t_begin) >> 6;

  const int i0 = 2 * uw, i1 = 2 * uw + 1;
  const int r0 = (i0 & 7) * 8 + (lane >> 3), r1 = (i1 & 7) * 8 + (lane >> 3);
  const int sc0 = (((lane & 7) ^ (2 * tn_g(r0))) * 8) + (i0 >> 3) * 64;
  const int sc1 = (((lane & 7) ^ (2 * tn_g(r1))) * 8) + (i1 >> 3) * 64;
  const int dst0 = (i0 >> 3) * 4096 + (i0 & 7) * 8 * 64, dst1 = (i1 >> 3) * 4096 + (i1 & 7) * 8 * 64;
  const int fg = lane >> 4, li = lane & 15, q4 = li >> 2, p4 = li & 3;
  const int gsw = 2 * (((q4 >> 1) & 1) | ((fg & 1) << 1));
  const int rowbase = (8 * fg + q4) * 64 + (p4 & 1) * 4;
  int aoff[4], boff[2];
#pragma unroll
  for (int mi = 0; mi < 4; ++mi) aoff[mi] = wm * 4096 + rowbase + (((2 * mi + (p4 >> 1)) ^ gsw) << 3);
#pragma unroll
  for (int ni = 0; ni < 2; ++ni)
    boff[ni] = (wn >> 1) * 4096 + rowbase + (((4 * (wn & 1) + 2 * ni + (p4 >> 1)) ^ gsw) << 3);
  const unsigned lds0 = (unsigned)(size_t)&smem[0];
#define FRAG(r, kk) (bf16x8{r[2 * (kk)][0], r[2 * (kk)][1], r[2 * (kk)][2], r[2 * (kk)][3],              \
                            r[2 * (kk) + 1][0], r[2 * (kk) + 1][1], r[2 * (kk) + 1][2], r[2 * (kk) + 1][3]})

  f32x4 acc[2][4][2][2];
#pragma unroll
  for (int a = 0; a < 2; ++a)
#pragma unroll
    for (int b = 0; b < 4; ++b)
#pragma unroll
      for (int c = 0; c < 2; ++c)
#pragma unroll
        for (int d = 0; d < 2; ++d) acc[a][b][c][d] = f32x4{0.f, 0.f, 0.f, 0.f};
#ifndef TN_DBG
#define TN_DBG 0
#endif
#if TN_DBG
  unsigned long long tnw_ = 0, tnq_ = 0;
#define TN_W0() tnq_ = __builtin_readcyclecounter()
#define TN_W1() tnw_ += __builtin_readcyclecounter() - tnq_
#else
#define TN_W0()
#define TN_W1()
#endif
#define LANDED(more)                                                      \
  do {                                                                    \
    TN_W0();                                                              \
    if (more) asm volatile("s_waitcnt vmcnt(6)" ::: "memory");            \
    else asm volatile("s_waitcnt vmcnt(0)" ::: "memory");                 \
    TN_W1();                                                              \
  } while (0)

  s16x4 ra1[4][4], rb2[2][2][4];
#define TR1(dst, addr, OFF) dst = lds_read_tr16_addr((addr) + (OFF))
#define RD4(dst, ad_, o_)   \
  do { TR1(dst[0], ad_, (o_)); TR1(dst[1], ad_, (o_) + 512); TR1(dst[2], ad_, (o_) + 4096); TR1(dst[3], ad_, (o_) + 4608); PIN(); } while (0)
#define RA4(buf, h, mi) RD4(ra1[mi], abase[buf][mi], (h) * 16384)
#define RB4(bb, buf, h, ni) RD4(rb2[bb][ni], bbase[buf][ni], (2 + (h)) * 16384)
#define SA_(h, kt) ((const char*)p.A + ((size_t)(t_begin + (kt) * 64) * p.lda + bn * 256 + (h) * 128) * 2)
#define SB_(h, kt) ((const char*)p.B + ((size_t)(t_begin + (kt) * 64) * p.ldb + bk * 256 + (h) * 128) * 2)
#define STG_A(buf, h, kt)                                                                     \
  do {                                                                                        \
    const char* sb_ = SA_(h, kt);                                                             \
    DMA16(sb_, vA0, ldsb + (((buf) * 4 + (h)) * HT + dst0) * 2);                              \
    DMA16(sb_, vA1, ldsb + (((buf) * 4 + (h)) * HT + dst1) * 2);                              \
    PIN();                                                                                    \
  } while (0)
#define STG_B(buf, h, kt)                                                                     \
  do {                                                                                        \
    const char* sb_ = SB_(h, kt);                                                             \
    DMA16(sb_, vB0, ldsb + (((buf) * 4 + 2 + (h)) * HT + dst0) * 2);                          \
    DMA16(sb_, vB1, ldsb + (((buf) * 4 + 2 + (h)) * HT + dst1) * 2);                          \
    PIN();                                                                                    \
  } while (0)
  const uint32_t vA0 = (uint32_t)(r0 * p.lda + sc0) * 2, vA1 = (uint32_t)(r1 * p.lda + sc1) * 2;
  const uint32_t vB0 = (uint32_t)(r0 * p.ldb + sc0) * 2, vB1 = (uint32_t)(r1 * p.ldb + sc1) * 2;
  const uint32_t ldsb = LDS_ADDR(&smem[0]);
  unsigned abase[2][4], bbase[2][2];
#pragma unroll
  for (int bf = 0; bf < 2; ++bf) {
#pragma unroll
    for (int mi = 0; mi < 4; ++mi) abase[bf][mi] = lds0 + 65536u * bf + 2u * aoff[mi];
#pragma unroll
    for (int ni = 0; ni < 2; ++ni) bbase[bf][ni] = lds0 + 65536u * bf + 2u * boff[ni];
  }
#define PO_(pc) ((pc) == 0 ? 0 : (pc) == 1 ? 512 : (pc) == 2 ? 4096 : 4608)
#define RA1(buf, h, mi, pc) do { TR1(ra1[mi][pc], abase[buf][mi], (h) * 16384 + PO_(pc)); PIN(); } while (0)
#define RB1(bb, buf, h, ni, pc) do { TR1(rb2[bb][ni][pc], bbase[buf][ni], (2 + (h)) * 16384 + PO_(pc)); PIN(); } while (0)
#define MF1(mh, nh, bb, j)                                                                                      \
  do {                                                                                                          \
    acc[mh][(j) >> 2][nh][(j) & 1] = __builtin_amdgcn_mfma_f32_16x16x32_bf16(                                   \
        FRAG(rb2[bb][(j) & 1], ((j) >> 1) & 1), FRAG(ra1[(j) >> 2], ((j) >> 1) & 1), acc[mh][(j) >> 2][nh][(j) & 1], 0, 0, 0); \
    PIN();                                                                                                      \
  } while (0)
#define PH1(mh, nh, bb, s0, s1, s2, s3, s4, s5, s6, s7, s8, s9, s10, s11, s12, s13, s14, s15)                    \
  do {                                                                                                          \
    BARRIER(); PIN();                                                                                           \
    MF1(mh, nh, bb, 0); s0; MF1(mh, nh, bb, 1); s1; MF1(mh, nh, bb, 2); s2; MF1(mh, nh, bb, 3); s3;             \
    MF1(mh, nh, bb, 4); s4; MF1(mh, nh, bb, 5); s5; MF1(mh, nh, bb, 6); s6; MF1(mh, nh, bb, 7); s7;             \
    MF1(mh, nh, bb, 8); s8; MF1(mh, nh, bb, 9); s9; MF1(mh, nh, bb, 10); s10; MF1(mh, nh, bb, 11); s11;         \
    MF1(mh, nh, bb, 12); s12; MF1(mh, nh, bb, 13); s13; MF1(mh, nh, bb, 14); s14; MF1(mh, nh, bb, 15); s15;     \
  } while (0)
#define NOP_ (void)0
#define TWO(x, y) do { x; y; } while (0)
#define TN_STEP(bb)                                                                                             \
  do {                                                                                                          \
    constexpr int b = (bb);  \
    const bool n1 = t + 1 < nk, n2 = t + 2 < nk;                                                                \
                                  \
    PH1(0, 0, bb, RA1(b, 0, 3, 0), RA1(b, 0, 3, 1), RA1(b, 0, 3, 2), RA1(b, 0, 3, 3),                           \
        RB1(1 - bb, b, 1, 0, 0), RB1(1 - bb, b, 1, 0, 1), RB1(1 - bb, b, 1, 0, 2), RB1(1 - bb, b, 1, 0, 3),     \
        RB1(1 - bb, b, 1, 1, 0), RB1(1 - bb, b, 1, 1, 1), RB1(1 - bb, b, 1, 1, 2), RB1(1 - bb, b, 1, 1, 3),     \
        TWO(if (n1) STG_A(b ^ 1, 1, t + 1), NOP_), NOP_, NOP_, NOP_);                                           \
                              \
    PH1(0, 1, 1 - bb, NOP_, NOP_, NOP_, NOP_, RA1(b, 1, 0, 0), RA1(b, 1, 0, 1), RA1(b, 1, 0, 2), RA1(b, 1, 0, 3), \
        RA1(b, 1, 1, 0), RA1(b, 1, 1, 1), RA1(b, 1, 1, 2), RA1(b, 1, 1, 3),                                     \
        RA1(b, 1, 2, 0), RA1(b, 1, 2, 1), RA1(b, 1, 2, 2), TWO(RA1(b, 1, 2, 3), TWO(if (n2) STG_A(b, 0, t + 2), NOP_))); \
                                                                             \
    PH1(1, 1, 1 - bb, RA1(b, 1, 3, 0), RA1(b, 1, 3, 1), RA1(b, 1, 3, 2), RA1(b, 1, 3, 3),                       \
        TWO(if (n2) STG_B(b, 0, t + 2), NOP_), NOP_, NOP_, NOP_, TWO(if (n2) STG_B(b, 1, t + 2), NOP_), NOP_, NOP_, NOP_, \
        NOP_, NOP_, NOP_, NOP_);                                                                                \
    LANDED(n2);                                                                                                 \
                    \
    PH1(1, 0, bb, RB1(1 - bb, b ^ 1, 0, 0, 0), RB1(1 - bb, b ^ 1, 0, 0, 1), RB1(1 - bb, b ^ 1, 0, 0, 2),        \
        RB1(1 - bb, b ^ 1, 0, 0, 3),                                                                            \
        TWO(RA1(b ^ 1, 0, 0, 0), RB1(1 - bb, b ^ 1, 0, 1, 0)), TWO(RA1(b ^ 1, 0, 0, 1), RB1(1 - bb, b ^ 1, 0, 1, 1)), \
        TWO(RA1(b ^ 1, 0, 0, 2), RB1(1 - bb, b ^ 1, 0, 1, 2)), TWO(RA1(b ^ 1, 0, 0, 3), RB1(1 - bb, b ^ 1, 0, 1, 3)), \
        RA1(b ^ 1, 0, 1, 0), RA1(b ^ 1, 0, 1, 1), RA1(b ^ 1, 0, 1, 2), RA1(b ^ 1, 0, 1, 3),                     \
        RA1(b ^ 1, 0, 2, 0), RA1(b ^ 1, 0, 2, 1), RA1(b ^ 1, 0, 2, 2), RA1(b ^ 1, 0, 2, 3));                    \
  } while (0)
  if (nk > 0) {
    STG_A(0, 0, 0); STG_B(0, 0, 0); STG_B(0, 1, 0); STG_A(0, 1, 0);
    if (nk > 1) { STG_A(1, 0, 1); STG_B(1, 0, 1); STG_B(1, 1, 1); }
    LANDED(nk > 1);
  }
  BARRIER();
#if TN_DBG
  tnw_ = 0;
  const unsigned long long tn_c0 = __builtin_readcyclecounter(), tn_r0 = __builtin_amdgcn_s_memrealtime();
#endif
  if (nk > 0) {
    RA4(0, 0, 0); RA4(0, 0, 1); RA4(0, 0, 2); RB4(0, 0, 0, 0); RB4(0, 0, 0, 1);
    int t = 0;
    while (true) {
      TN_STEP(0);
      if (++t >= nk) break;
      TN_STEP(1);
      if (++t >= nk) break;
    }
    BARRIER();
  }
#if TN_DBG
  if ((blockIdx.x == 17 || blockIdx.x == 130) && lane == 0 && (uw == 0 || uw == 5)) {
    const unsigned long long dc = __builtin_readcyclecounter() - tn_c0, dr = __builtin_amdgcn_s_memrealtime() - tn_r0;
    printf("TN blk %d wave %d: %d K-tiles, %.3f us per K-tile, %.0f MHz, vmcnt wait %.1f %% of the loop\n", (int)blockIdx.x, uw, nk,
           (double)dr / 100.0 / nk, (double)dc / ((double)dr / 100.0), 100.0 * (double)tnw_ / (double)dc);
  }
#endif
#undef TN_STEP
#undef TWO
#undef NOP_
#undef PH1
#undef MF1
#undef RA1
#undef RB1
#undef PO_
#undef RA4
#undef RB4
#undef RD4
#undef TR1
#undef STG_A
#undef STG_B
#undef SA_
#undef SB_
#undef FRAG
#undef LANDED

  float* out = p.slab + (size_t)split * p.N * p.K;
  int lane_e = (int)__builtin_amdgcn_mbcnt_hi(~0u, __builtin_amdgcn_mbcnt_lo(~0u, 0u));
  asm volatile("" : "+v"(lane_e));
  const int li_e = lane_e & 15, fg_e = lane_e >> 4;
#pragma unroll
  for (int mh = 0; mh < 2; ++mh)
#pragma unroll
    for (int mi = 0; mi < 4; ++mi) {
      const int n = bn * 256 + mh * 128 + wm * 64 + mi * 16 + li_e;
      if (n >= p.N) continue;
#pragma unroll
      for (int nh = 0; nh < 2; ++nh)
#pragma unroll
        for (int ni = 0; ni < 2; ++ni) {
          const int k0 = bk * 256 + nh * 128 + wn * 32 + ni * 16 + 4 * fg_e;
          const f32x4 v = acc[mh][mi][nh][ni];
          *(float4*)(out + (size_t)n * p.K + k0) = make_float4(v[0], v[1], v[2], v[3]);
        }
    }
}

}

extern "C" int plb_launch_gemm_tn_big(const PlbGemmTN* p, hipStream_t stream) {
  if (p->Ncols % 256 || p->K % 256 || p->rows_per_split % 64 || p->Mtot % 64 || p->splits <= 0) return 1;
  if ((long)p->splits * p->rows_per_split < p->Mtot) return 1;
  dim3 grid((p->Ncols / 256) * (p->K / 256) * p->splits), block(512);
  hipLaunchKernelGGL(gemm_tn_big_kernel, grid, block, 0, stream, *p);
  return hipGetLastError() == hipSuccess ? 0 : 2;
}

static int g_nt_prefetch = -1;
extern "C" void plb_set_gemm_nt_prefetch(int on) { g_nt_prefetch = on; }

extern "C" int plb_launch_gemm_nt_big(const PlbGemmNT* p, int tile, int act, int out_f32, hipStream_t stream) {
  const bool pf = g_nt_prefetch < 0 ? (tile != 256 || act != 0) : (g_nt_prefetch != 0);
  if (pf)
    return tile == 384 ? launch_big<3, true>(p, act, out_f32, stream)
           : tile == 1256 ? launch_big<1, true>(p, act, out_f32, stream) : launch_big<2, true>(p, act, out_f32, stream);
  return tile == 384 ? launch_big<3, false>(p, act, out_f32, stream)
         : tile == 1256 ? launch_big<1, false>(p, act, out_f32, stream) : launch_big<2, false>(p, act, out_f32, stream);
}
```

plbert_amd/csrc/gemm_ln.hip:

```cpp
#include "gemm_nt_pipeline.h"

static int g_ln_fault_mode = 0, g_ln_fault_launches = 0;
extern "C" void plb_debug_ln_fault(int mode, int launches) { g_ln_fault_mode = mode; g_ln_fault_launches = launches; }
extern "C" int plb_ln_fault_take(void) {
  if (g_ln_fault_launches <= 0) return 0;
  --g_ln_fault_launches;
  return g_ln_fault_mode;
}

extern "C" int plb_launch_gemm_nt_ln(const PlbGemmNT* p_in, int mode, hipStream_t stream) {
  PlbGemmNT q_ = *p_in;
  q_.ln_fault = plb_ln_fault_take();
  const PlbGemmNT* p = &q_;
  if (const int rc = ln_launch_check(p, mode, 64)) return rc;
  const int tile = p->N % 384 == 0 ? 384 : 256;
  dim3 grid((p->M / 128) * (p->N / tile)), block(512);
  const double mnk = (double)p->M * p->N * p->K;
  const double bytes = 2.0 * ((double)p->M * p->K + (double)p->N * p->K) + (double)p->M * p->N * (mode == 5 ? 4 : 4) +
                       (p->res ? 2.0 * p->M * p->N : 0.0);
  const int tok = plb_prof_begin(mode == 5 ? PLB_K_GEMM_NT_LNFWD : PLB_K_GEMM_NT_LNBWD, stream, 2.0 * mnk, bytes);
  if (tile == 384) {
    if (mode == 5) hipLaunchKernelGGL((gemm_nt_big_kernel<3, 5, false, true>), grid, block, 0, stream, *p);
    else hipLaunchKernelGGL((gemm_nt_big_kernel<3, 6, false, true>), grid, block, 0, stream, *p);
  } else {
    if (mode == 5) hipLaunchKernelGGL((gemm_nt_big_kernel<1, 5, false, true>), grid, block, 0, stream, *p);
    else hipLaunchKernelGGL((gemm_nt_big_kernel<1, 6, false, true>), grid, block, 0, stream, *p);
  }
  plb_prof_end(tok, stream);
  return hipGetLastError() == hipSuccess ? 0 : 2;
}

extern "C" int plb_launch_gemm_nt_gelud(const PlbGemmNT* p, int backward, hipStream_t stream) {
  if (p->M % 256 || p->N % 256 || p->K % 64 || p->M <= 0 || p->N <= 0 || p->K <= 0) return 3;
  if (!p->C || (!backward && !p->C2) || (backward && !p->aux)) return 1;
  dim3 grid((p->M / 256) * (p->N / 256)), block(512);
  const double mnk = (double)p->M * p->N * p->K;
  const double bytes = 2.0 * ((double)p->M * p->K + (double)p->N * p->K) + 4.0 * p->M * p->N;
  const int tok = plb_prof_begin(backward ? PLB_K_GEMM_NT_GELUBWD : PLB_K_GEMM_NT_GELU, stream, 2.0 * mnk, bytes);
  if (backward) hipLaunchKernelGGL((gemm_nt_big_kernel<2, 8, false, true>), grid, block, 0, stream, *p);
  else if (p->colpart) hipLaunchKernelGGL((gemm_nt_big_kernel<2, 7, false, true>), grid, block, 0, stream, *p);
  else hipLaunchKernelGGL((gemm_nt_big_kernel<2, 7, false, true, false, false, true>), grid, block, 0, stream, *p);
  plb_prof_end(tok, stream);
  return hipGetLastError() == hipSuccess ? 0 : 2;
}
```

plbert_amd/csrc/gemm_nt_pipeline.h:

```cpp
#pragma once
#include <type_traits>
#include "common.h"
#include "plbert_kernels.h"
#include "gemm_epilogue.h"

#ifndef NT_DBG
#define NT_DBG 0
#endif
typedef unsigned int u32x4nt __attribute__((ext_vector_type(4)));
template <bool NT>
DEVI void out_store(bf16_t* ptr, std::conditional_t<NT, const uint4, const uint4&> v) {
  if constexpr (NT) __builtin_nontemporal_store(u32x4nt{v.x, v.y, v.z, v.w}, (u32x4nt*)ptr);
  else *(uint4*)ptr = v;
}

typedef int i32x4v __attribute__((ext_vector_type(4)));
typedef int i32x8v __attribute__((ext_vector_type(8)));
template <bool ABF8>
DEVI f32x4 mfma_fp8(const i32x8v& bv, const i32x8v& av, const f32x4& c) {
  return __builtin_amdgcn_mfma_scale_f32_16x16x128_f8f6f4(bv, av, c, 0, ABF8 ? 1 : 0, 0, 0x7F7F7F7F, 0, 0x7F7F7F7F);
}
template <int HALF>
DEVI void set_half(i32x8v& v, const i32x4v t) {
  v[4 * HALF + 0] = t[0]; v[4 * HALF + 1] = t[1]; v[4 * HALF + 2] = t[2]; v[4 * HALF + 3] = t[3];
}

namespace {

constexpr int HT = 128 * 64;
constexpr int RING = 10;
DEVI int ring_slot(int x) { return x >= 2 * RING ? x - 2 * RING : (x >= RING ? x - RING : x); }

typedef __attribute__((address_space(1))) const void* gptr_t;
typedef __attribute__((address_space(3))) void* lptr_t;

#define BARRIER()                                        \
  do {                                                   \
    __builtin_amdgcn_s_waitcnt(0xC07F);                  \
    asm volatile("s_barrier" ::: "memory");              \
  } while (0)
#define PIN() __builtin_amdgcn_sched_barrier(0)

template <int V, int ACT, bool OUTF32, bool PF, bool FP8 = false, bool ABF8 = false, bool NOCS = false>
__global__ __launch_bounds__(512) void gemm_nt_big_kernel(PlbGemmNT p) {
  constexpr int NAH = (V == 2) ? 2 : 1;
  constexpr int NBH = (V == 3) ? 3 : 2;
  constexpr int TM = NAH * 128, TN = NBH * 128;
  constexpr int NH = NAH + NBH;
  __shared__ __attribute__((aligned(16))) bf16_t smem[RING * HT];
  int tid = threadIdx.x, lane = tid & 63;
  const int uw = __builtin_amdgcn_readfirstlane(tid >> 6);
  const int wm = uw >> 2, wn = uw & 3;
  const int nbn = p.N / TN;
  int bm, bn;
  if constexpr (ACT == 5 || ACT == 6) {
    const int xcd = blockIdx.x & 7, slot = blockIdx.x >> 3, gpx = (p.M / TM) >> 3;
    bm = xcd * gpx + slot / nbn; bn = slot % nbn;
  } else {
    const int logical = xcd_remap(blockIdx.x, gridDim.x);
    bm = logical / nbn; bn = logical % nbn;
  }
  constexpr int EPK = FP8 ? 128 : 64;
  const int nk = p.K / EPK;
#if NT_DBG & 16
  const unsigned long long dbg_c0 = __builtin_readcyclecounter(), dbg_r0 = __builtin_amdgcn_s_memrealtime();
#endif
#if NT_DBG & 32
  unsigned long long st_[6];
  st_[0] = __builtin_amdgcn_s_memrealtime();
#endif

  const int drow = lane >> 3;
  constexpr int EB = FP8 ? 1 : 2;
  const int ch0 = ((lane & 7) ^ ((lane >> 4) & 7)) * 16;
  const int ch1 = ((lane & 7) ^ ((4 + (lane >> 4)) & 7)) * 16;
  const uint32_t vA0 = (uint32_t)(((2 * uw) * 8 + drow) * p.lda * EB + ch0), vA1 = (uint32_t)(((2 * uw + 1) * 8 + drow) * p.lda * EB + ch1);
  const uint32_t vB0 = (uint32_t)(((2 * uw) * 8 + drow) * p.ldb * EB + ch0), vB1 = (uint32_t)(((2 * uw + 1) * 8 + drow) * p.ldb * EB + ch1);
  const char* const sA_ = (const char*)p.A + (size_t)(bm * TM) * p.lda * EB;
  const char* const sB_ = (const char*)p.B + (size_t)(bn * TN) * p.ldb * EB;
  const size_t hA = (size_t)128 * p.lda * EB, hB = (size_t)128 * p.ldb * EB;
  const int dst0 = (2 * uw) * 8 * 64, dst1 = (2 * uw + 1) * 8 * 64;
  const uint32_t ldsb_ = LDS_ADDR(&smem[0]);
#define STAGE_A(slot, h, kt)                                                                                  \
  do {                                                                                                        \
    const char* b_ = sA_ + (h) * hA + (size_t)(kt) * 128;                                                     \
    DMA16(b_, vA0, ldsb_ + 2u * ((slot) * HT + dst0));                                                        \
    DMA16(b_, vA1, ldsb_ + 2u * ((slot) * HT + dst1));                                                        \
  } while (0)
#define STAGE_B(slot, h, kt)                                                                                  \
  do {                                                                                                        \
    const char* b_ = sB_ + (h) * hB + (size_t)(kt) * 128;                                                     \
    DMA16(b_, vB0, ldsb_ + 2u * ((slot) * HT + dst0));                                                        \
    DMA16(b_, vB1, ldsb_ + 2u * ((slot) * HT + dst1));                                                        \
  } while (0)
#define STAGE_I(i, slot, kt)                                              \
  do {                                                                    \
    if (V == 2 && (i) == 3) STAGE_A(slot, 1, kt);                         \
    else if ((i) == 0) STAGE_A(slot, 0, kt);                              \
    else STAGE_B(slot, (i) - 1, kt);                                      \
  } while (0)
#define ISSUE(c)                                                          \
  do {                                                                    \
    if (NH * t + (c) < htot) STAGE_I((c) % NH, ring_slot(rb + (c)), t + (c) / NH); \
  } while (0)

  int frow = lane & 15, fq = lane >> 4;
  const int fsw = (frow >> 1) & 7;
  const int offA = (wm * 64 + frow) * 64, offB = (wn * 32 + frow) * 64;
  const int c0 = ((0 + fq) ^ fsw) << 3, c1 = ((4 + fq) ^ fsw) << 3;
  bf16x8 afr[2][4][2], bfr[2][2][2];
  i32x8v afr8[2][4], bfr8[2][2];
#define READ_A(ab, slot)                                                             \
  do {                                                                               \
    const bf16_t* s_ = &smem[(slot) * HT + offA];                                    \
    if constexpr (FP8) _Pragma("unroll") for (int mi = 0; mi < 4; ++mi) {            \
      set_half<0>(afr8[ab][mi], *(const i32x4v*)&s_[mi * 16 * 64 + c0]);             \
      set_half<1>(afr8[ab][mi], *(const i32x4v*)&s_[mi * 16 * 64 + c1]);             \
    } else _Pragma("unroll") for (int mi = 0; mi < 4; ++mi) {                        \
      afr[ab][mi][0] = *(const bf16x8*)&s_[mi * 16 * 64 + c0];                       \
      afr[ab][mi][1] = *(const bf16x8*)&s_[mi * 16 * 64 + c1];                       \
    }                                                                                \
  } while (0)
#define READ_B(bb, slot)                                                             \
  do {                                                                               \
    const bf16_t* s_ = &smem[(slot) * HT + offB];                                    \
    if constexpr (FP8) _Pragma("unroll") for (int ni = 0; ni < 2; ++ni) {            \
      set_half<0>(bfr8[bb][ni], *(const i32x4v*)&s_[ni * 16 * 64 + c0]);             \
      set_half<1>(bfr8[bb][ni], *(const i32x4v*)&s_[ni * 16 * 64 + c1]);             \
    } else _Pragma("unroll") for (int ni = 0; ni < 2; ++ni) {                        \
      bfr[bb][ni][0] = *(const bf16x8*)&s_[ni * 16 * 64 + c0];                       \
      bfr[bb][ni][1] = *(const bf16x8*)&s_[ni * 16 * 64 + c1];                       \
    }                                                                                \
  } while (0)

  f32x4 acc[NAH][4][NBH][2];
#pragma unroll
  for (int a = 0; a < NAH; ++a)
#pragma unroll
    for (int b = 0; b < 4; ++b)
#pragma unroll
      for (int c = 0; c < NBH; ++c)
#pragma unroll
        for (int d = 0; d < 2; ++d) acc[a][b][c][d] = f32x4{0.f, 0.f, 0.f, 0.f};
#define MFMA_Q(mh, nh, ab, bb)                                                                                 \
  do {                                                                                                         \
    if constexpr (FP8) {                                                                                       \
      _Pragma("unroll") for (int mi = 0; mi < 4; ++mi)                                                         \
        _Pragma("unroll") for (int ni = 0; ni < 2; ++ni)                                                       \
          acc[mh][mi][nh][ni] = mfma_fp8<ABF8>(bfr8[bb][ni], afr8[ab][mi], acc[mh][mi][nh][ni]);               \
    } else _Pragma("unroll") for (int kk = 0; kk < 2; ++kk)                                                    \
      _Pragma("unroll") for (int mi = 0; mi < 4; ++mi)                                                         \
        _Pragma("unroll") for (int ni = 0; ni < 2; ++ni)                                                       \
          acc[mh][mi][nh][ni] = __builtin_amdgcn_mfma_f32_16x16x32_bf16(bfr[bb][ni][kk], afr[ab][mi][kk],     \
                                                                        acc[mh][mi][nh][ni], 0, 0, 0);         \
  } while (0)
#define MFMA_PART(mh, nh, bb)            \
  do {                                   \
    BARRIER(); PIN();                    \
    __builtin_amdgcn_s_setprio(1);       \
    MFMA_Q(mh, nh, 0, bb);               \
    __builtin_amdgcn_s_setprio(0);       \
    PIN(); BARRIER(); PIN();             \
  } while (0)
#define LANDED(more, N)                                                        \
  do {                                                                         \
    if (more) asm volatile("s_waitcnt vmcnt(" #N ")" ::: "memory");            \
    else asm volatile("s_waitcnt vmcnt(0)" ::: "memory");                      \
  } while (0)

  const int htot = NH * nk;
  int rb = 0;
  {
    const int t = 0;
    ISSUE(0); ISSUE(1); ISSUE(2); ISSUE(3); ISSUE(4); ISSUE(5); ISSUE(6); ISSUE(7); ISSUE(8);
    if constexpr (V == 2) {
      ISSUE(9);
      LANDED(htot > 9, 12);
    } else if constexpr (V == 3) {
      LANDED(htot > 8, 10);
    } else {
      LANDED(htot > 8, 12);
    }
  }
  BARRIER();
#if NT_DBG & 32
  st_[1] = __builtin_amdgcn_s_memrealtime();
#endif
  if constexpr (PF) {
    READ_A(0, 0);
    READ_B(0, 1);
    int t = 0;
#define NEXT_T() do { ++t; rb += NH; rb = rb >= RING ? rb - RING : rb; } while (0)
#define MF(mh, nh, ab, bb, j)                                                                          \
  do {                                                                                                 \
    if constexpr (FP8) {        \
      if (((j) & 1) == 0)                                                                              \
        acc[mh][((j) >> 2) & 3][nh][((j) >> 1) & 1] = mfma_fp8<ABF8>(                                  \
            bfr8[bb][((j) >> 1) & 1], afr8[ab][((j) >> 2) & 3], acc[mh][((j) >> 2) & 3][nh][((j) >> 1) & 1]); \
    } else                                                                                             \
      acc[mh][((j) >> 1) & 3][nh][(j) & 1] = __builtin_amdgcn_mfma_f32_16x16x32_bf16(                  \
          bfr[bb][(j) & 1][(j) >> 3], afr[ab][((j) >> 1) & 3][(j) >> 3], acc[mh][((j) >> 1) & 3][nh][(j) & 1], 0, 0, 0); \
    PIN();                                                                                             \
  } while (0)
#define RA(ab, slot, i)                                                                                \
  do {                                                                                                 \
    if constexpr (FP8)                                                                                 \
      set_half<(i) & 1>(afr8[ab][(i) >> 1], *(const i32x4v*)&smem[(slot) * HT + offA + ((i) >> 1) * 16 * 64 + (((i) & 1) ? c1 : c0)]); \
    else                                                                                               \
      afr[ab][(i) >> 1][(i) & 1] = *(const bf16x8*)&smem[(slot) * HT + offA + ((i) >> 1) * 16 * 64 + (((i) & 1) ? c1 : c0)]; \
    PIN();                                                                                             \
  } while (0)
#define RB(bb, slot, i)                                                                                \
  do {                                                                                                 \
    if constexpr (FP8)                                                                                 \
      set_half<(i) & 1>(bfr8[bb][(i) >> 1], *(const i32x4v*)&smem[(slot) * HT + offB + ((i) >> 1) * 16 * 64 + (((i) & 1) ? c1 : c0)]); \
    else                                                                                               \
      bfr[bb][(i) >> 1][(i) & 1] = *(const bf16x8*)&smem[(slot) * HT + offB + ((i) >> 1) * 16 * 64 + (((i) & 1) ? c1 : c0)]; \
    PIN();                                                                                             \
  } while (0)
#define IS(c) do { ISSUE(c); PIN(); } while (0)
#define PH(mh, nh, ab, bb, s0, s1, s2, s3, s4, s5, s6, s7, s8, s9, s10, s11, s12, s13, s14, s15)      \
  do {                                                                                                 \
    BARRIER(); PIN();                                                                                  \
    MF(mh, nh, ab, bb, 0); s0; MF(mh, nh, ab, bb, 1); s1; MF(mh, nh, ab, bb, 2); s2; MF(mh, nh, ab, bb, 3); s3;       \
    MF(mh, nh, ab, bb, 4); s4; MF(mh, nh, ab, bb, 5); s5; MF(mh, nh, ab, bb, 6); s6; MF(mh, nh, ab, bb, 7); s7;       \
    MF(mh, nh, ab, bb, 8); s8; MF(mh, nh, ab, bb, 9); s9; MF(mh, nh, ab, bb, 10); s10; MF(mh, nh, ab, bb, 11); s11;   \
    MF(mh, nh, ab, bb, 12); s12; MF(mh, nh, ab, bb, 13); s13; MF(mh, nh, ab, bb, 14); s14; MF(mh, nh, ab, bb, 15); s15; \
  } while (0)
#define NOP_ (void)0
#define STEP1(ab)                                                                                       \
  do {                                                                                                  \
    const int sB1 = ring_slot(rb + 2), sA = ring_slot(rb + 3), sB0 = ring_slot(rb + 4);                 \
    PH(0, 0, ab, 0, RB(1, sB1, 0), NOP_, RB(1, sB1, 1), NOP_, RB(1, sB1, 2), NOP_, RB(1, sB1, 3), NOP_,  \
       IS(9), NOP_, NOP_, NOP_, NOP_, NOP_, NOP_, NOP_);                                                \
    LANDED(NH * t + 9 < htot, 8);                                                                       \
    PH(0, 1, ab, 1, RA(1 - ab, sA, 0), RA(1 - ab, sA, 1), RA(1 - ab, sA, 2), RA(1 - ab, sA, 3),         \
       RA(1 - ab, sA, 4), RA(1 - ab, sA, 5), RA(1 - ab, sA, 6), RA(1 - ab, sA, 7),                      \
       RB(0, sB0, 0), RB(0, sB0, 1), RB(0, sB0, 2), RB(0, sB0, 3), IS(10), NOP_, IS(11), NOP_);         \
  } while (0)
#define STEP2(bb)                                                                                       \
  do {                                                                                                  \
    const int sB1 = ring_slot(rb + 2), sA1 = ring_slot(rb + 3), sA0 = ring_slot(rb + 4), sB0 = ring_slot(rb + 5); \
    PH(0, 0, 0, bb, RB(1 - bb, sB1, 0), NOP_, RB(1 - bb, sB1, 1), NOP_, RB(1 - bb, sB1, 2), NOP_,        \
       RB(1 - bb, sB1, 3), NOP_, NOP_, NOP_, NOP_, NOP_, NOP_, NOP_, NOP_, NOP_);                       \
    PH(0, 1, 0, 1 - bb, RA(1, sA1, 0), RA(1, sA1, 1), RA(1, sA1, 2), RA(1, sA1, 3), RA(1, sA1, 4),      \
       RA(1, sA1, 5), RA(1, sA1, 6), RA(1, sA1, 7), IS(10), NOP_, NOP_, IS(11), NOP_, NOP_, NOP_, NOP_); \
    PH(1, 1, 1, 1 - bb, NOP_, NOP_, IS(12), NOP_, NOP_, NOP_, NOP_, NOP_, NOP_, NOP_, NOP_, NOP_, NOP_, \
       NOP_, NOP_, NOP_);                                                                               \
    LANDED(NH * t + 12 < htot, 10);                                                                     \
    PH(1, 0, 1, bb, RA(0, sA0, 0), RA(0, sA0, 1), RA(0, sA0, 2), RA(0, sA0, 3), RA(0, sA0, 4),          \
       RA(0, sA0, 5), RA(0, sA0, 6), RA(0, sA0, 7), RB(1 - bb, sB0, 0), RB(1 - bb, sB0, 1),             \
       RB(1 - bb, sB0, 2), RB(1 - bb, sB0, 3), IS(13), NOP_, NOP_, NOP_);                               \
  } while (0)
#define STEP3(ab, bb)                                                                                   \
  do {                                                                                                  \
    const int sB1 = ring_slot(rb + 2), sB2 = ring_slot(rb + 3), sA = ring_slot(rb + 4), sB0 = ring_slot(rb + 5); \
    PH(0, 0, ab, bb, RB(1 - bb, sB1, 0), NOP_, RB(1 - bb, sB1, 1), NOP_, RB(1 - bb, sB1, 2), NOP_,       \
       RB(1 - bb, sB1, 3), NOP_, IS(9), NOP_, NOP_, NOP_, NOP_, NOP_, NOP_, NOP_);                      \
    PH(0, 1, ab, 1 - bb, RB(bb, sB2, 0), NOP_, RB(bb, sB2, 1), NOP_, RB(bb, sB2, 2), NOP_,               \
       RB(bb, sB2, 3), NOP_, IS(10), NOP_, NOP_, IS(11), NOP_, NOP_, NOP_, NOP_);                       \
    LANDED(NH * t + 11 < htot, 8);                                                                      \
    PH(0, 2, ab, bb, RA(1 - ab, sA, 0), RA(1 - ab, sA, 1), RA(1 - ab, sA, 2), RA(1 - ab, sA, 3),        \
       RA(1 - ab, sA, 4), RA(1 - ab, sA, 5), RA(1 - ab, sA, 6), RA(1 - ab, sA, 7),                      \
       RB(1 - bb, sB0, 0), RB(1 - bb, sB0, 1), RB(1 - bb, sB0, 2), RB(1 - bb, sB0, 3), IS(12), NOP_, NOP_, NOP_); \
  } while (0)
    while (true) {
      if constexpr (V == 1) STEP1(0); else if constexpr (V == 2) STEP2(0); else STEP3(0, 0);
      NEXT_T();
      if (t >= nk) break;
      if constexpr (V == 1) STEP1(1); else if constexpr (V == 2) STEP2(1); else STEP3(1, 1);
      NEXT_T();
      if (t >= nk) break;
    }
    BARRIER();
#undef STEP1
#undef STEP2
#undef STEP3
#undef NEXT_T
#undef MF
#undef RA
#undef RB
#undef IS
#undef PH
#undef NOP_
  } else {
  if (wm == 1) BARRIER();

  for (int t = 0; t < nk; ++t) {
    if constexpr (V == 1) {
      ISSUE(9);
      READ_B(0, ring_slot(rb + 1));
      READ_A(0, ring_slot(rb));
      MFMA_PART(0, 0, 0);
      ISSUE(10); ISSUE(11);
      LANDED(NH * t + 11 < htot, 12);
      READ_B(1, ring_slot(rb + 2));
      MFMA_PART(0, 1, 1);
    } else if constexpr (V == 2) {
      READ_B(0, ring_slot(rb + 1));
      READ_A(0, ring_slot(rb));
      MFMA_PART(0, 0, 0);
      ISSUE(10); ISSUE(11);
      READ_B(1, ring_slot(rb + 2));
      MFMA_PART(0, 1, 1);
      ISSUE(12);
      READ_A(0, ring_slot(rb + 3));
      MFMA_PART(1, 1, 1);
      ISSUE(13);
      LANDED(NH * t + 13 < htot, 12);
      MFMA_PART(1, 0, 0);
    } else {
      ISSUE(9);
      READ_B(0, ring_slot(rb + 1));
      READ_A(0, ring_slot(rb));
      MFMA_PART(0, 0, 0);
      ISSUE(10); ISSUE(11);
      READ_B(1, ring_slot(rb + 2));
      MFMA_PART(0, 1, 1);
      ISSUE(12);
      LANDED(NH * t + 12 < htot, 10);
      READ_B(0, ring_slot(rb + 3));
      MFMA_PART(0, 2, 0);
    }
    rb += NH;
    rb = rb >= RING ? rb - RING : rb;
  }
  if (wm == 0) BARRIER();
  }
#undef STAGE_I
#undef ISSUE
#undef STAGE_A
#undef STAGE_B
#undef READ_A
#undef READ_B
#undef MFMA_Q
#undef MFMA_PART
#undef LANDED

#if NT_DBG & 16
  if (blockIdx.x == 17 && tid == 0) {
    const unsigned long long dc = __builtin_readcyclecounter() - dbg_c0, dr = __builtin_amdgcn_s_memrealtime() - dbg_r0;
    printf("K loop: %llu cycles in %llu ticks of 100 MHz -> %.0f MHz, %.3f us per K-tile\n", dc, dr,
           (double)dc / ((double)dr / 100.0), (double)dr / 100.0 / nk);
  }
#endif
  if constexpr (FP8) {
    lane = (int)__builtin_amdgcn_mbcnt_hi(~0u, __builtin_amdgcn_mbcnt_lo(~0u, 0u));
    asm volatile("" : "+v"(lane));
    tid = lane + 64 * uw;
    frow = lane & 15; fq = lane >> 4;
  }
#if NT_DBG & 32
  st_[2] = __builtin_amdgcn_s_memrealtime();
#endif
  constexpr int OROW_PAD = 8;
  constexpr int OROW = TN + OROW_PAD;
  constexpr bool OUT_NT = ACT == 1 || ACT == 2 || ACT == 5 || ACT == 6 || ACT == 7 || ACT == 8;
  static_assert(TM * OROW <= RING * HT, "output image must fit the ring");
  f32x4 csum[NBH][2];
  float4 bz[NBH][2];
#pragma unroll
  for (int nh = 0; nh < NBH; ++nh)
#pragma unroll
    for (int ni = 0; ni < 2; ++ni) {
      csum[nh][ni] = f32x4{0.f, 0.f, 0.f, 0.f};
      bz[nh][ni] = p.bias ? *(const float4*)(p.bias + bn * TN + nh * 128 + wn * 32 + ni * 16 + fq * 4)
                          : make_float4(0.f, 0.f, 0.f, 0.f);
    }
  const int ncol0 = bn * TN + wn * 32 + fq * 4;
  float deq = 1.0f;
  if constexpr (FP8) deq = p.deq_a[0] * p.deq_b[0];
  if constexpr (ACT == 3) {
    float* const stat = reinterpret_cast<float*>(smem);
#pragma unroll
    for (int mh = 0; mh < NAH; ++mh)
#pragma unroll
      for (int mi = 0; mi < 4; ++mi) {
        const int lrow = mh * 128 + wm * 64 + mi * 16 + frow;
        const int m = bm * TM + lrow;
        const int tg = (int)p.ce_tgt[m];
        float mx = -INFINITY;
#pragma unroll
        for (int nh = 0; nh < NBH; ++nh)
#pragma unroll
          for (int ni = 0; ni < 2; ++ni) {
            f32x4& v = acc[mh][mi][nh][ni];
            const int n0 = ncol0 + nh * 128 + ni * 16;
            v[0] += bz[nh][ni].x; v[1] += bz[nh][ni].y; v[2] += bz[nh][ni].z; v[3] += bz[nh][ni].w;
            if ((unsigned)(tg - n0) < 4u) p.ce_tlogit[m] = v[tg - n0];
            if (n0 + 3 >= p.ce_cols) {
#pragma unroll
              for (int r = 0; r < 4; ++r) v[r] = (n0 + r < p.ce_cols) ? v[r] : -INFINITY;
            }
            mx = fmaxf(mx, fmaxf(fmaxf(v[0], v[1]), fmaxf(v[2], v[3])));
          }
        float sm = 0.f;
        if (mx > -INFINITY) {
#pragma unroll
          for (int nh = 0; nh < NBH; ++nh)
#pragma unroll
            for (int ni = 0; ni < 2; ++ni) {
              const f32x4 v = acc[mh][mi][nh][ni];
              sm += (__expf(v[0] - mx) + __expf(v[1] - mx)) + (__expf(v[2] - mx) + __expf(v[3] - mx));
            }
        }
#pragma unroll
        for (int o = 16; o < 64; o <<= 1) {
          const float m2 = __shfl_xor(mx, o, 64), s2 = __shfl_xor(sm, o, 64);
          const float mm = fmaxf(mx, m2);
          sm = mm > -INFINITY ? sm * __expf(mx - mm) + s2 * __expf(m2 - mm) : 0.f;
          mx = mm;
        }
        if (fq == 0) { stat[(lrow * 4 + wn) * 2] = mx; stat[(lrow * 4 + wn) * 2 + 1] = sm; }
      }
    __syncthreads();
    const int ntile = p.N / TN;
    for (int r = tid; r < TM; r += 512) {
      float mx = -INFINITY, sm = 0.f;
#pragma unroll
      for (int w4 = 0; w4 < 4; ++w4) {
        const float m2 = stat[(r * 4 + w4) * 2], s2 = stat[(r * 4 + w4) * 2 + 1];
        const float mm = fmaxf(mx, m2);
        sm = mm > -INFINITY ? sm * __expf(mx - mm) + s2 * __expf(m2 - mm) : 0.f;
        mx = mm;
      }
      p.ce_pmax[(size_t)(bm * TM + r) * ntile + bn] = mx;
      p.ce_psum[(size_t)(bm * TM + r) * ntile + bn] = sm;
    }
    return;
  }
  if constexpr (ACT == 5 || ACT == 6) {
    static_assert(NAH == 1, "LayerNorm epilogues: 128-row tiles");
    if constexpr (FP8) {
#pragma unroll
      for (int mi = 0; mi < 4; ++mi)
#pragma unroll
        for (int nh = 0; nh < NBH; ++nh)
#pragma unroll
          for (int ni = 0; ni < 2; ++ni) acc[0][mi][nh][ni] *= deq;
    }
    constexpr int IMG = TM * OROW * 2;
    float* const tab = reinterpret_cast<float*>(reinterpret_cast<char*>(smem) + IMG);
    float* const tab2 = tab + 128 * 4 * 2;
    constexpr bool LEAN = FP8 && ACT == 6;
    typedef __attribute__((address_space(1))) unsigned long long gu64_t;
    gu64_t* const xq = (gu64_t*)(p.ln_xchg);
    const float invN = 1.0f / (float)p.N;
    float rmean[4], rrstd[4];
    uint2 rr[4][NBH][2], ux[4][NBH][2];
    constexpr int R2OFF = IMG + 128 * 4 * 2 * 4 + 128 * 2 * 4;
    constexpr int GAMOFF = R2OFF + 64 * OROW * 2;
    constexpr int TAB3OFF = GAMOFF + TN * 4;
    static_assert(GAMOFF + (ACT == 6 ? TN * 4 : 0) + (LEAN ? 1024 : 0) <= RING * HT * 2, "staging regions must fit the LDS");
    float* const tab3 = reinterpret_cast<float*>(reinterpret_cast<char*>(smem) + TAB3OFF);
    if constexpr (LEAN) {
      if (tid < TM) { tab3[tid * 2] = p.ln_mean[bm * TM + tid]; tab3[tid * 2 + 1] = p.ln_rstd[bm * TM + tid]; }
    }
    float* const gam_lds = reinterpret_cast<float*>(reinterpret_cast<char*>(smem) + GAMOFF);
    if constexpr (ACT == 6) {
      if (tid < TN / 4) reinterpret_cast<float4*>(gam_lds)[tid] = *(const float4*)(p.ln_gamma + bn * TN + tid * 4);
    }
    bf16_t* const r2 = reinterpret_cast<bf16_t*>(reinterpret_cast<char*>(smem) + R2OFF);
    const uint32_t stg_voff = (uint32_t)lane * 16u;
    auto stage_rows = [&](const bf16_t* src, int ld, int nrows, uint32_t lds_base, int half) {
      for (int i = 0; i < nrows / 8; ++i) {
        const int q = i * 8 + uw;
        const int trow = half < 0 ? q : (q >> 5) * 64 + half * 32 + (q & 31);
        const char* b = reinterpret_cast<const char*>(src + (size_t)(bm * TM + trow) * ld + bn * TN);
        if (lane < TN / 8) DMA16(b, stg_voff, lds_base + (uint32_t)q * (OROW * 2));
      }
    };
    const uint32_t img_lds = LDS_ADDR(&smem[0]), r2_lds = img_lds + R2OFF;
    if constexpr (ACT == 5) {
      if (p.res) { stage_rows(p.res, p.ldr, TM, img_lds, -1); DMA_WAIT(); }
      __syncthreads();
    } else {
      stage_rows(p.aux, p.ldaux, TM, img_lds, -1);
      if (p.res) stage_rows(p.res, p.ldr, 64, r2_lds, 0);
      DMA_WAIT();
      __syncthreads();
    }
#pragma unroll
    for (int mi = 0; mi < 4; ++mi) {
      const int m = bm * TM + wm * 64 + mi * 16 + frow;
      if constexpr (ACT == 6 && !LEAN) { rmean[mi] = p.ln_mean[m]; rrstd[mi] = p.ln_rstd[m]; }
      if constexpr (LEAN) {
        const float2 ms = *(const float2*)&tab3[(wm * 64 + mi * 16 + frow) * 2];
        rmean[mi] = ms.x; rrstd[mi] = ms.y;
      }
    }
    float s1[4] = {0.f, 0.f, 0.f, 0.f}, s2[4] = {0.f, 0.f, 0.f, 0.f};
#pragma unroll
    for (int hf = 0; hf < (ACT == 6 ? 2 : 1); ++hf) {
    if constexpr (ACT == 6) {
      if (p.res) {
        if (hf == 1) { DMA_WAIT(); __syncthreads(); }
#pragma unroll
        for (int mq = 0; mq < 2; ++mq)
#pragma unroll
          for (int nh = 0; nh < NBH; ++nh)
#pragma unroll
            for (int ni = 0; ni < 2; ++ni) {
              const uint2 r = *(const uint2*)&r2[(wm * 32 + mq * 16 + frow) * OROW + nh * 128 + wn * 32 + ni * 16 + fq * 4];
              f32x4& a = acc[0][hf * 2 + mq][nh][ni];
              a[0] += bf_lo(r.x); a[1] += bf_hi(r.x); a[2] += bf_lo(r.y); a[3] += bf_hi(r.y);
            }
        if (hf == 0) { __syncthreads(); stage_rows(p.res, p.ldr, 64, r2_lds, 1); }
      }
    }
#pragma unroll
    for (int nh = 0; nh < NBH; ++nh)
#pragma unroll
      for (int ni = 0; ni < 2; ++ni) {
        if constexpr (ACT == 6) PIN();
        const float4 gz = ACT == 6 ? *(const float4*)(gam_lds + (ncol0 - bn * TN) + nh * 128 + ni * 16)
                                   : *(const float4*)(p.ln_gamma + ncol0 + nh * 128 + ni * 16);
#pragma unroll
        for (int mi = (ACT == 6 ? hf * 2 : 0); mi < (ACT == 6 ? hf * 2 + 2 : 4); ++mi) {
          const int lrow = wm * 64 + mi * 16 + frow;
          if constexpr (ACT == 6) PIN();
          const uint2 t = *(const uint2*)&smem[lrow * OROW + nh * 128 + wn * 32 + ni * 16 + fq * 4];
          if constexpr (ACT == 5) rr[mi][nh][ni] = t; else ux[mi][nh][ni] = t;
          f32x4 v = acc[0][mi][nh][ni];
          if constexpr (ACT == 5) { v[0] += bz[nh][ni].x; v[1] += bz[nh][ni].y; v[2] += bz[nh][ni].z; v[3] += bz[nh][ni].w; }
          if constexpr (ACT == 5) {
            if (p.res) {
              v[0] += bf_lo(rr[mi][nh][ni].x); v[1] += bf_hi(rr[mi][nh][ni].x);
              v[2] += bf_lo(rr[mi][nh][ni].y); v[3] += bf_hi(rr[mi][nh][ni].y);
            }
          }
          uint2 o; o.x = pack_bf2(v[0], v[1]); o.y = pack_bf2(v[2], v[3]);
          v = f32x4{bf_lo(o.x), bf_hi(o.x), bf_lo(o.y), bf_hi(o.y)};
          if constexpr (ACT == 5) {
            *(uint2*)&smem[lrow * OROW + nh * 128 + wn * 32 + ni * 16 + fq * 4] = o;
            s1[mi] += (v[0] + v[1]) + (v[2] + v[3]);
            s2[mi] += (v[0] * v[0] + v[1] * v[1]) + (v[2] * v[2] + v[3] * v[3]);
          } else {
            const uint2 u = ux[mi][nh][ni];
            const f32x4 xh = {(bf_lo(u.x) - rmean[mi]) * rrstd[mi], (bf_hi(u.x) - rmean[mi]) * rrstd[mi],
                              (bf_lo(u.y) - rmean[mi]) * rrstd[mi], (bf_hi(u.y) - rmean[mi]) * rrstd[mi]};
            const f32x4 g = {v[0] * gz.x, v[1] * gz.y, v[2] * gz.z, v[3] * gz.w};
            s1[mi] += (g[0] + g[1]) + (g[2] + g[3]);
            s2[mi] += (g[0] * xh[0] + g[1] * xh[1]) + (g[2] * xh[2] + g[3] * xh[3]);
          }
          acc[0][mi][nh][ni] = v;
        }
      }
    }
#pragma unroll
    for (int mi = 0; mi < 4; ++mi) {
      const int lrow = wm * 64 + mi * 16 + frow;
      float a1 = s1[mi], a2 = s2[mi];
      a1 += __shfl_xor(a1, 16, 64); a1 += __shfl_xor(a1, 32, 64);
      a2 += __shfl_xor(a2, 16, 64); a2 += __shfl_xor(a2, 32, 64);
      if (fq == 0) { tab[(lrow * 4 + wn) * 2] = a1; tab[(lrow * 4 + wn) * 2 + 1] = a2; }
    }
    __syncthreads();
#if NT_DBG & 32
    unsigned long long ls_[6];
    ls_[0] = __builtin_amdgcn_s_memrealtime();
#endif
    float pa = 0.f, pb = 0.f;
    if (tid < TM) {
      pa = (tab[(tid * 4 + 0) * 2] + tab[(tid * 4 + 1) * 2]) + (tab[(tid * 4 + 2) * 2] + tab[(tid * 4 + 3) * 2]);
      pb = (tab[(tid * 4 + 0) * 2 + 1] + tab[(tid * 4 + 1) * 2 + 1]) + (tab[(tid * 4 + 2) * 2 + 1] + tab[(tid * 4 + 3) * 2 + 1]);
      if constexpr (ACT == 5) {
        const float mt = pa * (1.0f / (float)TN);
        pb = pb - pa * mt;
        pa = mt;
      }
      const unsigned long long wa = (1ull << 32) | __float_as_uint(pa), wb = (1ull << 32) | __float_as_uint(pb);
      const bool mute = p.ln_fault == 1 && bn == nbn - 1;
      for (int c = 0; c < nbn; ++c)
        if (c != bn && !mute) {
          gu64_t* g = xq + (((size_t)(bm * nbn + bn) * nbn + c) * TM + tid) * 2;
          __hip_atomic_store(g, wa, __ATOMIC_RELAXED, __HIP_MEMORY_SCOPE_AGENT);
          __hip_atomic_store(g + 1, wb, __ATOMIC_RELAXED, __HIP_MEMORY_SCOPE_AGENT);
        }
    }
    if constexpr (ACT == 5) {
      constexpr int CPR = TN / 8;
      bf16_t* const cbase = p.C + (size_t)(bm * TM) * p.ldc + bn * TN;
      const int rows_ok = p.Mstore - bm * TM;
#pragma unroll 4
      for (int c = tid; c < TM * CPR; c += 512) {
        const int r = c / CPR, cc = c - r * CPR;
        const uint4 v = *(const uint4*)&smem[r * OROW + cc * 8];
        if (r < rows_ok)
          __builtin_nontemporal_store(u32x4nt{v.x, v.y, v.z, v.w}, (u32x4nt*)(cbase + (size_t)r * p.ldc + cc * 8));
      }
    }
#if NT_DBG & 32
    ls_[1] = __builtin_amdgcn_s_memrealtime();
#endif
    if (tid < TM) {
      float qa[4], qb[4];
#pragma unroll
      for (int j = 0; j < 4; ++j) {
        qa[j] = 0.f; qb[j] = 0.f;
        if (j < nbn) {
          if (j == bn) { qa[j] = pa; qb[j] = pb; }
          else {
            gu64_t* g = xq + (((size_t)(bm * nbn + j) * nbn + bn) * TM + tid) * 2;
            unsigned long long wa = 0, wb = 0;
            bool seen = false;
            for (unsigned spins = 0; spins < (1u << 18); ++spins) {
              wa = __hip_atomic_load(g, __ATOMIC_RELAXED, __HIP_MEMORY_SCOPE_AGENT);
              wb = __hip_atomic_load(g + 1, __ATOMIC_RELAXED, __HIP_MEMORY_SCOPE_AGENT);
              if ((wa >> 32) == 1ull && (wb >> 32) == 1ull) { seen = true; break; }
              __builtin_amdgcn_s_sleep(4);
            }
            const bool late = p.ln_fault == 2 && bn == 0;
            if (!seen || late) atomicAdd(p.ln_err, 1u);
            if (!late) {
              __hip_atomic_store(g, 0ull, __ATOMIC_RELAXED, __HIP_MEMORY_SCOPE_AGENT);
              __hip_atomic_store(g + 1, 0ull, __ATOMIC_RELAXED, __HIP_MEMORY_SCOPE_AGENT);
            }
            qa[j] = __uint_as_float((unsigned int)wa); qb[j] = __uint_as_float((unsigned int)wb);
          }
        }
      }
      if constexpr (ACT == 5) {
        float mean = 0.f;
        for (int j = 0; j < nbn; ++j) mean += qa[j];
        mean *= 1.0f / (float)nbn;
        float m2 = 0.f;
        for (int j = 0; j < nbn; ++j) m2 += qb[j] + (float)TN * (qa[j] - mean) * (qa[j] - mean);
        m2 = fmaxf(m2, 0.f);
        const float rstd = rsqrtf(m2 * invN + p.ln_eps);
        tab2[tid * 2] = mean; tab2[tid * 2 + 1] = rstd;
        const int m = bm * TM + tid;
        if (bn == 0 && m < p.Mstore) { p.ln_mean[m] = mean; p.ln_rstd[m] = rstd; }
      } else {
        float a = 0.f, b = 0.f;
        for (int j = 0; j < nbn; ++j) { a += qa[j]; b += qb[j]; }
        tab2[tid * 2] = a * invN; tab2[tid * 2 + 1] = b * invN;
      }
    }
    __syncthreads();
#if NT_DBG & 32
    ls_[2] = __builtin_amdgcn_s_memrealtime();
#endif
    float t0[4], t1[4];
    if constexpr (!LEAN) {
#pragma unroll
      for (int mi = 0; mi < 4; ++mi) { t0[mi] = tab2[(wm * 64 + mi * 16 + frow) * 2]; t1[mi] = tab2[(wm * 64 + mi * 16 + frow) * 2 + 1]; }
    }
    if constexpr (LEAN) asm volatile("" ::: "memory");
    int ncol2 = ncol0;
    asm volatile("" : "+v"(ncol2));
#pragma unroll
    for (int nh = 0; nh < NBH; ++nh)
#pragma unroll
      for (int ni = 0; ni < 2; ++ni) {
        if constexpr (ACT == 6) PIN();
        float4 bt = make_float4(0.f, 0.f, 0.f, 0.f);
        const float4 gz = ACT == 6 ? *(const float4*)(gam_lds + (ncol2 - bn * TN) + nh * 128 + ni * 16)
                                   : *(const float4*)(p.ln_gamma + ncol2 + nh * 128 + ni * 16);
        if constexpr (ACT == 5) bt = *(const float4*)(p.ln_beta + ncol2 + nh * 128 + ni * 16);
        f32x4 cs = {0.f, 0.f, 0.f, 0.f}, dg = {0.f, 0.f, 0.f, 0.f}, db = {0.f, 0.f, 0.f, 0.f};
#pragma unroll
        for (int mi = 0; mi < 4; ++mi) {
          const int lrow = wm * 64 + mi * 16 + frow;
          const f32x4 x = acc[0][mi][nh][ni];
          f32x4 y;
          if constexpr (LEAN) {
            const float2 tt = *(const float2*)&tab2[lrow * 2], ms = *(const float2*)&tab3[lrow * 2];
            t0[mi] = tt.x; t1[mi] = tt.y; rmean[mi] = ms.x; rrstd[mi] = ms.y;
            asm volatile("" : "+v"(t0[mi]), "+v"(t1[mi]), "+v"(rmean[mi]), "+v"(rrstd[mi]));
          }
          if constexpr (ACT == 5) {
            y = f32x4{(x[0] - t0[mi]) * t1[mi] * gz.x + bt.x, (x[1] - t0[mi]) * t1[mi] * gz.y + bt.y,
                      (x[2] - t0[mi]) * t1[mi] * gz.z + bt.z, (x[3] - t0[mi]) * t1[mi] * gz.w + bt.w};
          } else {
            const float mu = rmean[mi], rs = rrstd[mi];
            uint2 u = *(const uint2*)&smem[lrow * OROW + nh * 128 + wn * 32 + ni * 16 + fq * 4];
            asm volatile("" : "+v"(u.x), "+v"(u.y));
            const f32x4 xh = {(bf_lo(u.x) - mu) * rs, (bf_hi(u.x) - mu) * rs, (bf_lo(u.y) - mu) * rs, (bf_hi(u.y) - mu) * rs};
            dg += x * xh; db += x;
            y = f32x4{rs * (x[0] * gz.x - t0[mi] - xh[0] * t1[mi]), rs * (x[1] * gz.y - t0[mi] - xh[1] * t1[mi]),
                      rs * (x[2] * gz.z - t0[mi] - xh[2] * t1[mi]), rs * (x[3] * gz.w - t0[mi] - xh[3] * t1[mi])};
          }
          uint2 o; o.x = pack_bf2(y[0], y[1]); o.y = pack_bf2(y[2], y[3]);
          *(uint2*)&smem[lrow * OROW + nh * 128 + wn * 32 + ni * 16 + fq * 4] = o;
          if (ACT == 6 && bm * TM + lrow < p.Mstore) cs += f32x4{bf_lo(o.x), bf_hi(o.x), bf_lo(o.y), bf_hi(o.y)};

        }
        if constexpr (ACT == 6) {
#pragma unroll
          for (int q3 = 0; q3 < 3; ++q3) {
            f32x4 v = q3 == 0 ? dg : q3 == 1 ? db : cs;
            v = f32x4{row16_sum(v[0]), row16_sum(v[1]), row16_sum(v[2]), row16_sum(v[3])};
            if (frow == 0)
              *(float4*)(p.colpart + ((size_t)(bm * 2 + wm) * 3 + q3) * p.N + ncol2 + nh * 128 + ni * 16) =
                  make_float4(v[0], v[1], v[2], v[3]);
          }
        }
      }
    __syncthreads();
#if NT_DBG & 32
    ls_[3] = __builtin_amdgcn_s_memrealtime();
#endif
    {
      constexpr int CPR = TN / 8;
      bf16_t* const obase = (ACT == 5 ? p.C2 + (size_t)(bm * TM) * p.ldc2 : p.C + (size_t)(bm * TM) * p.ldc) + bn * TN;
      const int ldo = ACT == 5 ? p.ldc2 : p.ldc;
      const int rows_ok = p.Mstore - bm * TM;
      const bool img8 = FP8 && p.C8 != nullptr;
      const float qs8 = img8 ? p.q_scale[0] : 1.0f;
      constexpr bool bf8o = ACT == 6;
      float amax8 = 0.f;
      unsigned char* const qbase = img8 ? p.C8 + (size_t)(bm * TM) * p.ldc8 + bn * TN : nullptr;
#pragma unroll 4
      for (int c = tid; c < TM * CPR; c += 512) {
        const int r = c / CPR, cc = c - r * CPR;
        const uint4 v = *(const uint4*)&smem[r * OROW + cc * 8];
        if (r < rows_ok) {
          __builtin_nontemporal_store(u32x4nt{v.x, v.y, v.z, v.w}, (u32x4nt*)(obase + (size_t)r * ldo + cc * 8));
          if constexpr (FP8) {
            if (img8) {
              const float f0 = bf_lo(v.x), f1 = bf_hi(v.x), f2 = bf_lo(v.y), f3 = bf_hi(v.y);
              const float f4 = bf_lo(v.z), f5 = bf_hi(v.z), f6 = bf_lo(v.w), f7 = bf_hi(v.w);
              uint2 w;
              w.x = pack_fp8x4(f0 * qs8, f1 * qs8, f2 * qs8, f3 * qs8, bf8o);
              w.y = pack_fp8x4(f4 * qs8, f5 * qs8, f6 * qs8, f7 * qs8, bf8o);
              *(uint2*)(qbase + (size_t)r * p.ldc8 + cc * 8) = w;
              amax8 = fmaxf(amax8, fmaxf(fmaxf(fmaxf(fabsf(f0), fabsf(f1)), fmaxf(fabsf(f2), fabsf(f3))),
                                         fmaxf(fmaxf(fabsf(f4), fabsf(f5)), fmaxf(fabsf(f6), fabsf(f7)))));
            }
          }
        }
      }
      if constexpr (FP8) {
        if (img8 && p.q_amax) {
          amax8 = wave_max(amax8);
          if (lane == 0) atomic_max_abs(p.q_amax, amax8, blockIdx.x * 8 + uw);
        }
      }
    }
#if NT_DBG & 32
    ls_[4] = __builtin_amdgcn_s_memrealtime();
    asm volatile("s_waitcnt vmcnt(0)" ::: "memory");
    ls_[5] = __builtin_amdgcn_s_memrealtime();
    if ((blockIdx.x % 256) == 17 && tid == 0)
      printf("blk %d LN form %d: fill %llu | kloop %llu | pass 1 %llu | publish + image 1 out %llu | partners' partials %llu | pass 2 %llu | "
             "stores issued %llu | drained %llu (x10 ns)\n", (int)blockIdx.x, ACT, st_[1] - st_[0], st_[2] - st_[1], ls_[0] - st_[2],
             ls_[1] - ls_[0], ls_[2] - ls_[1], ls_[3] - ls_[2], ls_[4] - ls_[3], ls_[5] - ls_[4]);
#endif
    return;
  }
  uint4* const lane_stash = reinterpret_cast<uint4*>(ACT == 7 ? p.C : const_cast<bf16_t*>(p.aux));
  constexpr int SQD = 3;
  uint4 sq[SQD + 1][NBH];
  uint2 keep[NAH][4][NBH][2];
  uint32_t k8[NAH][4][NBH][2];
  const bool want8 = FP8 && p.C8 != nullptr;
  const float qs = want8 ? p.q_scale[0] : 1.0f;
  float amax = 0.f;
  const bool want16 = !FP8 || (ACT == 7 ? p.C2 : p.C) != nullptr;
#pragma unroll
  for (int mh = 0; mh < NAH; ++mh)
#pragma unroll
    for (int mi = 0; mi < 4; ++mi) {
      const int lrow = mh * 128 + wm * 64 + mi * 16 + frow;
      const int m = bm * TM + lrow;
      uint2 rr[NBH][2], ux[NBH][2];
      if (p.res) {
#pragma unroll
        for (int nh = 0; nh < NBH; ++nh)
#pragma unroll
          for (int ni = 0; ni < 2; ++ni)
            rr[nh][ni] = *(const uint2*)(p.res + (size_t)m * p.ldr + ncol0 + nh * 128 + ni * 16);
      }
      if (ACT == 2) {
#pragma unroll
        for (int nh = 0; nh < NBH; ++nh)
#pragma unroll
          for (int ni = 0; ni < 2; ++ni)
            ux[nh][ni] = *(const uint2*)(p.aux + (size_t)m * p.ldaux + ncol0 + nh * 128 + ni * 16);
      }
      if (ACT == 8) {
        constexpr int NS = NAH * 4;
        const int sl = mh * 4 + mi;
        if (sl == 0) {
#pragma unroll
          for (int a = 0; a < SQD && a < NS; ++a)
#pragma unroll
            for (int nh = 0; nh < NBH; ++nh)
              sq[a][nh] = lane_stash[((size_t)(bm * nbn + bn) * (NS * NBH) + a * NBH + nh) * 512 + tid];
        }
        if (sl + SQD < NS) {
#pragma unroll
          for (int nh = 0; nh < NBH; ++nh)
            sq[(sl + SQD) % (SQD + 1)][nh] = lane_stash[((size_t)(bm * nbn + bn) * (NS * NBH) + (sl + SQD) * NBH + nh) * 512 + tid];
        }
#pragma unroll
        for (int nh = 0; nh < NBH; ++nh) {
          const uint4 q = sq[sl % (SQD + 1)][nh];
          ux[nh][0] = make_uint2(q.x, q.y); ux[nh][1] = make_uint2(q.z, q.w);
        }
      }
      const bool st = m < p.Mstore;
      float ce_l = 0.f, ce_wt = 0.f;
      int ce_t = -1;
      if (ACT == 4) { ce_l = p.ce_lse[m]; ce_wt = p.ce_w[m]; ce_t = (int)p.ce_tgt[m]; }
      uint2 dpair = make_uint2(0u, 0u);
#pragma unroll
      for (int nh = 0; nh < NBH; ++nh)
#pragma unroll
        for (int ni = 0; ni < 2; ++ni) {
          f32x4 v = acc[mh][mi][nh][ni];
          const int n0 = ncol0 + nh * 128 + ni * 16;
          if constexpr (FP8) { v[0] *= deq; v[1] *= deq; v[2] *= deq; v[3] *= deq; }
          v[0] += bz[nh][ni].x; v[1] += bz[nh][ni].y; v[2] += bz[nh][ni].z; v[3] += bz[nh][ni].w;
          if (ACT == 4) {
#pragma unroll
            for (int r = 0; r < 4; ++r) {
              float gq = (ce_wt != 0.f && n0 + r < p.ce_cols) ? __expf(v[r] - ce_l) * ce_wt : 0.f;
              gq -= (n0 + r == ce_t) ? ce_wt : 0.f;
              v[r] = gq;
            }
          }
          if (p.res) {
            v[0] += bf_lo(rr[nh][ni].x); v[1] += bf_hi(rr[nh][ni].x);
            v[2] += bf_lo(rr[nh][ni].y); v[3] += bf_hi(rr[nh][ni].y);
          }
          if (ACT == 2) {
            v[0] = v[0] != 0.f ? v[0] * gelu_new_grad_f(bf_lo(ux[nh][ni].x)) : 0.f;
            v[1] = v[1] != 0.f ? v[1] * gelu_new_grad_f(bf_hi(ux[nh][ni].x)) : 0.f;
            v[2] = v[2] != 0.f ? v[2] * gelu_new_grad_f(bf_lo(ux[nh][ni].y)) : 0.f;
            v[3] = v[3] != 0.f ? v[3] * gelu_new_grad_f(bf_hi(ux[nh][ni].y)) : 0.f;
          }
          if (ACT == 8) {
            v[0] = v[0] != 0.f ? v[0] * bf_lo(ux[nh][ni].x) : 0.f; v[1] = v[1] != 0.f ? v[1] * bf_hi(ux[nh][ni].x) : 0.f;
            v[2] = v[2] != 0.f ? v[2] * bf_lo(ux[nh][ni].y) : 0.f; v[3] = v[3] != 0.f ? v[3] * bf_hi(ux[nh][ni].y) : 0.f;
          }
          uint2 gpk = make_uint2(0u, 0u);
          if (ACT == 7) {
            f32x4 gg;
#pragma unroll
            for (int r = 0; r < 4; ++r) {
              const float x = v[r], x2 = x * x;
              const float sg = gelu_sigmoid(x, x2);
              gg[r] = x * sg;
              v[r] = __builtin_fmaf(sg, x * __builtin_fmaf(x2, 0.21406444f, 1.5957691f) * (1.0f - sg), sg);
            }
            gpk.x = pack_bf2(gg[0], gg[1]); gpk.y = pack_bf2(gg[2], gg[3]);
            asm volatile("" : "+v"(gpk.x), "+v"(gpk.y));
          }
          if (OUTF32) {
            if (st) *(float4*)(p.Cf + (size_t)m * p.ldcf + n0) = make_float4(v[0], v[1], v[2], v[3]);
          } else {
            uint2 o; o.x = pack_bf2(v[0], v[1]); o.y = pack_bf2(v[2], v[3]);
            if (ACT == 7) {
              if (ni == 0) dpair = o;
              else
                __builtin_nontemporal_store(u32x4nt{dpair.x, dpair.y, o.x, o.y},
                    (u32x4nt*)(lane_stash + ((size_t)(bm * nbn + bn) * (NAH * 4 * NBH) + (mh * 4 + mi) * NBH + nh) * 512 + tid));
              if (want16) *(uint2*)&smem[lrow * OROW + nh * 128 + wn * 32 + ni * 16 + fq * 4] = gpk;
            } else {
              if (want16) *(uint2*)&smem[lrow * OROW + nh * 128 + wn * 32 + ni * 16 + fq * 4] = o;
            }
            if (ACT == 1) keep[mh][mi][nh][ni] = o;
            v = f32x4{bf_lo(o.x), bf_hi(o.x), bf_lo(o.y), bf_hi(o.y)};
            if constexpr (FP8 && ACT != 1) {
              if (want8) {
                const f32x4 z = ACT == 7 ? f32x4{bf_lo(gpk.x), bf_hi(gpk.x), bf_lo(gpk.y), bf_hi(gpk.y)} : v;
                k8[mh][mi][nh][ni] = pack_fp8x4(z[0] * qs, z[1] * qs, z[2] * qs, z[3] * qs, ACT == 7 ? false : ACT == 8 ? true : p.c8_bf8 != 0);
                if (st) amax = fmaxf(amax, fmaxf(fmaxf(fabsf(z[0]), fabsf(z[1])), fmaxf(fabsf(z[2]), fabsf(z[3]))));
              }
            }
          }
          if (!NOCS && st) csum[nh][ni] += v;
        }
    }
  if (!OUTF32) {
    constexpr int CPR = TN / 8;
    const int ldimg = ACT == 7 ? p.ldc2 : p.ldc;
    bf16_t* const cbase = (ACT == 7 ? p.C2 : p.C) + (size_t)(bm * TM) * ldimg + bn * TN;
    const int rows_ok = p.Mstore - bm * TM;
    __syncthreads();
#if NT_DBG & 32
    st_[3] = __builtin_amdgcn_s_memrealtime();
#endif
    if (want16) {
#pragma unroll 4
      for (int c = tid; c < TM * CPR; c += 512) {
        const int r = c / CPR, cc = c - r * CPR;
        const uint4 v = *(const uint4*)&smem[r * OROW + cc * 8];
        if (r < rows_ok) out_store<OUT_NT>(cbase + (size_t)r * ldimg + cc * 8, v);
      }
    }
    if (ACT == 1) {
      __syncthreads();
#pragma unroll
      for (int mh = 0; mh < NAH; ++mh)
#pragma unroll
        for (int mi = 0; mi < 4; ++mi)
#pragma unroll
          for (int nh = 0; nh < NBH; ++nh)
#pragma unroll
            for (int ni = 0; ni < 2; ++ni) {
              const uint2 o = keep[mh][mi][nh][ni];
              uint2 g;
              g.x = pack_bf2(gelu_new_f(bf_lo(o.x)), gelu_new_f(bf_hi(o.x)));
              g.y = pack_bf2(gelu_new_f(bf_lo(o.y)), gelu_new_f(bf_hi(o.y)));
              *(uint2*)&smem[(mh * 128 + wm * 64 + mi * 16 + frow) * OROW + nh * 128 + wn * 32 + ni * 16 + fq * 4] = g;
              if constexpr (FP8) {
                if (want8) {
                  const float g0 = bf_lo(g.x), g1 = bf_hi(g.x), g2 = bf_lo(g.y), g3 = bf_hi(g.y);
                  k8[mh][mi][nh][ni] = pack_fp8x4(g0 * qs, g1 * qs, g2 * qs, g3 * qs, p.c8_bf8 != 0);
                  if (bm * TM + mh * 128 + wm * 64 + mi * 16 + frow < p.Mstore)
                    amax = fmaxf(amax, fmaxf(fmaxf(fabsf(g0), fabsf(g1)), fmaxf(fabsf(g2), fabsf(g3))));
                }
              }
            }
      __syncthreads();
      bf16_t* const gbase = p.C2 + (size_t)(bm * TM) * p.ldc2 + bn * TN;
#pragma unroll 4
      for (int c = tid; c < TM * CPR; c += 512) {
        const int r = c / CPR, cc = c - r * CPR;
        const uint4 v = *(const uint4*)&smem[r * OROW + cc * 8];
        if (r < rows_ok) out_store<OUT_NT>(gbase + (size_t)r * p.ldc2 + cc * 8, v);
      }
    }
    if constexpr (FP8) {
      if (want8) {
        unsigned char* const img8 = reinterpret_cast<unsigned char*>(smem);
        __syncthreads();
#pragma unroll
        for (int mh = 0; mh < NAH; ++mh)
#pragma unroll
          for (int mi = 0; mi < 4; ++mi)
#pragma unroll
            for (int nh = 0; nh < NBH; ++nh)
#pragma unroll
              for (int ni = 0; ni < 2; ++ni)
                *(uint32_t*)&img8[(mh * 128 + wm * 64 + mi * 16 + frow) * OROW + nh * 128 + wn * 32 + ni * 16 + fq * 4] =
                    k8[mh][mi][nh][ni];
        __syncthreads();
        constexpr int CPR8 = TN / 16;
        unsigned char* const qbase = p.C8 + (size_t)(bm * TM) * p.ldc8 + bn * TN;
#pragma unroll 4
        for (int c = tid; c < TM * CPR8; c += 512) {
          const int r = c / CPR8, cc = c - r * CPR8;
          const uint4 v = *(const uint4*)&img8[r * OROW + cc * 16];
          if (r < rows_ok) *(uint4*)(qbase + (size_t)r * p.ldc8 + cc * 16) = v;
        }
        if (p.q_amax) {
          amax = wave_max(amax);
          if (lane == 0) atomic_max_abs(p.q_amax, amax, blockIdx.x * 8 + uw);
        }
      }
    }
  }
  if (!NOCS && p.colpart) {
#pragma unroll
    for (int nh = 0; nh < NBH; ++nh)
#pragma unroll
      for (int ni = 0; ni < 2; ++ni) {
        f32x4 v = csum[nh][ni];
        v = f32x4{row16_sum(v[0]), row16_sum(v[1]), row16_sum(v[2]), row16_sum(v[3])};
        if (frow == 0)
          *(float4*)(p.colpart + (size_t)(bm * 2 + wm) * p.N + bn * TN + nh * 128 + wn * 32 + ni * 16 + fq * 4) =
              make_float4(v[0], v[1], v[2], v[3]);
      }
  }
#if NT_DBG & 32
  st_[4] = __builtin_amdgcn_s_memrealtime();
  asm volatile("s_waitcnt vmcnt(0)" ::: "memory");
  st_[5] = __builtin_amdgcn_s_memrealtime();
  if ((blockIdx.x % 256) == 17 && tid == 0)
    printf("blk %d: start %llu | fill %llu | kloop %llu | image %llu | stores issued %llu | drained %llu (x10 ns)\n", (int)blockIdx.x,
           st_[0] % 1000000ull, st_[1] - st_[0], st_[2] - st_[1], st_[3] - st_[2], st_[4] - st_[3], st_[5] - st_[4]);
#endif
}

inline int ln_launch_check(const PlbGemmNT* p, int mode, int kmult) {
  if (mode != 5 && mode != 6) return 1;
  if (p->M % 1024 || p->K % kmult || p->M <= 0 || p->N <= 0 || p->K <= 0) return 3;
  const int tile = p->N % 384 == 0 ? 384 : p->N % 256 == 0 ? 256 : 0;
  if (!tile || p->N / tile > 4) return 3;
  if (!p->ln_gamma || !p->ln_mean || !p->ln_rstd || !p->ln_xchg || !p->ln_err || !p->C) return 1;
  if (mode == 5 && (!p->ln_beta || !p->C2)) return 1;
  if (mode == 6 && (!p->aux || !p->colpart)) return 1;
  if (p->res && (((uintptr_t)p->res & 15) || p->ldr % 8)) return 1;
  if (mode == 6 && (((uintptr_t)p->aux & 15) || p->ldaux % 8)) return 1;
  return 0;
}

}
```

plbert_amd/csrc/plbert_kernels.h:

```cpp
#pragma once
#include <hip/hip_runtime.h>
#include <stdint.h>

typedef uint16_t bf16_t;

extern "C" {

enum PlbKernelClass {
  PLB_K_GEMM_NT = 0, PLB_K_GEMM_NT_GELU, PLB_K_GEMM_NT_GELUBWD, PLB_K_GEMM_NT_F32, PLB_K_GEMM_TN,
  PLB_K_ATTN_FWD, PLB_K_ATTN_BWD_DQ, PLB_K_ATTN_BWD_DKV, PLB_K_LN_FWD, PLB_K_LN_BWD, PLB_K_EMBED_FWD,
  PLB_K_EMBED_BWD, PLB_K_COLSUM, PLB_K_REDUCE, PLB_K_ROWS, PLB_K_CE, PLB_K_ADAMW, PLB_K_CAST, PLB_K_TOKEN_CE, PLB_K_GEMM_NT_CE, PLB_K_GEMM_NT_SMALL, PLB_K_FP8, PLB_K_ATTN_BWD,
  PLB_K_GEMM_NT_FP8, PLB_K_GEMM_NT_GELU_FP8, PLB_K_GEMM_NT_GELUBWD_FP8,
  PLB_K_GEMM_NT_LNFWD, PLB_K_GEMM_NT_LNBWD,
  PLB_K_GEMM_NT_LNFWD_FP8, PLB_K_GEMM_NT_LNBWD_FP8, PLB_K_GEMM_TN_FP8,
  PLB_K_NCLASS
};
int plb_prof_begin(int cls, hipStream_t s, double flops, double bytes);
void plb_prof_end(int tok, hipStream_t s);

typedef struct {
  const bf16_t* A; int lda;
  const bf16_t* B; int ldb;
  int M, N, K;
  int Mstore;
  const float* bias;
  const bf16_t* res; int ldr;
  const bf16_t* aux; int ldaux;
  bf16_t* C; int ldc;
  bf16_t* C2; int ldc2;
  float* Cf; int ldcf;
  float* colpart;
  int ce_cols;
  const int64_t* ce_tgt;
  float* ce_pmax; float* ce_psum;
  float* ce_tlogit;
  const float* ce_lse;
  const float* ce_w;
  const float* deq_a; const float* deq_b;
  uint8_t* C8; int ldc8;
  const float* q_scale;
  float* q_amax;
  int c8_bf8;
  const float* ln_gamma; const float* ln_beta;
  float* ln_mean; float* ln_rstd;
  float ln_eps;
  unsigned long long* ln_xchg;
  unsigned int* ln_err;
  int ln_fault;
} PlbGemmNT;
int plb_launch_gemm_nt_ln(const PlbGemmNT* p, int mode, hipStream_t stream);
int plb_launch_gemm_nt_gelud(const PlbGemmNT* p, int backward, hipStream_t stream);
int plb_launch_gemm_nt_fp8(const PlbGemmNT* p, int act, int a_bf8, hipStream_t stream);
int plb_launch_gemm_nt_fp8_ln(const PlbGemmNT* p, int mode, int a_bf8, hipStream_t stream);
int plb_launch_gemm_nt_fp8_gelud(const PlbGemmNT* p, int backward, int a_bf8, hipStream_t stream);
int plb_gemm_nt_fp8_gelud_tile_rows(int M);
int plb_ln_fault_take(void);
int plb_launch_gemm_nt(const PlbGemmNT* p, int act, int out_f32, hipStream_t stream);
int plb_launch_gemm_nt_big(const PlbGemmNT* p, int tile, int act, int out_f32, hipStream_t stream);
int plb_gemm_nt_colpart_rows(int M, int N, int K);
void plb_set_gemm_nt_tile(int tile);
void plb_set_gemm_nt_prefetch(int on);

typedef struct {
  const bf16_t* A; int lda; int Ncols;
  const bf16_t* B; int ldb;
  int Mtot, N, K;
  int rows_per_split, splits;
  float* slab;
  const float* deq_a; const float* deq_b;
} PlbGemmTN;
int plb_launch_gemm_tn(const PlbGemmTN* p, hipStream_t stream);
int plb_launch_gemm_tn_fp8(const PlbGemmTN* p, hipStream_t stream);
int plb_launch_gemm_tn_big(const PlbGemmTN* p, hipStream_t stream);

int plb_launch_reduce_slabs(const float* slab, int splits, size_t n, float* out, int accumulate, hipStream_t stream);

typedef struct {
  const int64_t* ids; int T, S, E, V;
  const float *word, *pos, *type0, *gamma, *beta;
  float eps;
  bf16_t* out; int ldo;
  const bf16_t* dout; int lddo;
  float* dx;
  float *dword, *dpos;
  float* partials;
  int nblocks;
  const int32_t* row_start; const int32_t* lengths; int B; int fill_slots;
} PlbEmbed;
int plb_launch_embed_fwd(const PlbEmbed* p, hipStream_t stream);
int plb_launch_embed_bwd(const PlbEmbed* p, hipStream_t stream);
int plb_launch_embed_scatter(const PlbEmbed* p, int P, hipStream_t stream);

typedef struct {
  const bf16_t* x; int ldx;
  const float *gamma, *beta; float eps;
  bf16_t* y; int ldy;
  float *mean, *rstd;
  int T, H;
  int Tzero;
  const bf16_t* dy; int lddy;
  bf16_t* dx; int lddx;
  float* partials; int nblocks;
  int accumulate;
  uint8_t* out8; int ld8; const float* q_scale; float* q_amax;
} PlbLayerNorm;
int plb_launch_amax(const void* x, int is_bf16, size_t rows, int cols, int ld, float* amax, hipStream_t stream);
int plb_launch_fp8_scales(float* amax, float* scale, float* deq, int n, float fmax, int group, hipStream_t stream);
int plb_launch_fp8_scales2(float* amax, float* scale, float* deq, int n, float fmax, int group, int n2, float fmax2,
                           float* stats, int hist_from, hipStream_t stream);
int plb_launch_quantize(const void* x, int is_bf16, size_t rows, int cols, int ld, const float* scale, uint8_t* out, int ldo,
                        int bf8, hipStream_t stream);
int plb_launch_quantize_multi(int n, const void* const* src, const int* is_bf16, const size_t* elements,
                              const float* const* scale, uint8_t* const* dst, float* const* amax, hipStream_t stream);
int plb_launch_ln_fwd(const PlbLayerNorm* p, hipStream_t stream);
int plb_launch_ln_bwd(const PlbLayerNorm* p, hipStream_t stream);

int plb_launch_colsum(const void* X, int is_bf16, size_t R, int N, int ld, float* out, int Nout, int accumulate,
                      float* scratch, int nsplit, hipStream_t stream);

int plb_launch_copy_cols(const float* scratch, int nsplit, int N, int col0, int Nout, float* out, hipStream_t stream);

int plb_launch_pooler(const float* hidden, int B, int S, int H, const float* W, const float* bias, float* pooled,
                      hipStream_t stream);

typedef struct {
  const bf16_t* qkv; int ldqkv;
  const int32_t* lengths;
  int B, S, NH, H;
  float scale;
  bf16_t* ctx; int ldctx;
  float* lse;
  const bf16_t* dctx; int lddctx;
  float* delta;
  bf16_t* dqkv; int lddqkv;
  float* colpart;
  int colpart_accumulate;
  uint8_t* ctx8; int ldctx8; const float* ctx_scale; float* ctx_amax;
  uint8_t* dqkv8; int lddqkv8; const float* dqkv_scale; float* dqkv_amax;
  const int32_t* qoff; const bf16_t* q; int ldq; int nq_total; bf16_t* dq; int lddq; uint8_t* dq8; int lddq8;
  const int32_t* row_start;
} PlbAttn;
int plb_launch_attn_fwd(const PlbAttn* p, hipStream_t stream);
int plb_launch_attn_bwd(const PlbAttn* p, hipStream_t stream);
int plb_launch_attn_bwd_fused(const PlbAttn* p, hipStream_t stream);
void plb_debug_skip_piece(int index);
void plb_debug_ln_fault(int mode, int launches);
void plb_set_attn_bwd_fused(int on);

int plb_launch_gather_rows(const bf16_t* src, int lds_, const int32_t* rows, int n, int npad, int H, bf16_t* dst,
                           int ldd, hipStream_t stream);
int plb_launch_scatter_rows(const bf16_t* src, int lds_, const int32_t* rows, int n, int H, bf16_t* dst, int ldd,
                            hipStream_t stream);
int plb_launch_ce_prepare(const int32_t* offsets, const int32_t* flat, const int64_t* labels, int B, int S,
                          int32_t* rows, int32_t* tgt, float* w, hipStream_t stream);
int plb_launch_ce_prepare_packed(const int32_t* offsets, const int32_t* flat, const int64_t* labels, int B, int S,
                                 const int32_t* row_start, int32_t* rows, int32_t* tgt, float* w, hipStream_t stream);
int plb_launch_unpack_rows(const void* src, int src_is_bf16, int lds_, const int32_t* row_start, const int32_t* lengths,
                           int B, int S, int C, float* dst, hipStream_t stream);
int plb_launch_seed_dy(const float* d_hidden, const int32_t* lengths, const int32_t* row_start, int B, int S, int H, int Tp,
                       bf16_t* dy, hipStream_t stream);
int plb_launch_ce_fwd_bwd(const float* logits, int ldl, int V, const int32_t* tgt, const float* w, int n, int npad,
                          float* loss_rows, bf16_t* dlogits, int ldd, hipStream_t stream);
int plb_launch_sum_rows(const float* x, int n, float* out, hipStream_t stream);
int plb_launch_token_ce_combine(const float* pmax, const float* psum, int ntiles, const float* tlogit,
                                const int32_t* lengths, int B, int S, int rows, float* lse, float* w, float* loss_rows,
                                hipStream_t stream);
int plb_launch_token_ce_combine_packed(const float* pmax, const float* psum, int ntiles, const float* tlogit,
                                       const int32_t* lengths, const int32_t* row_start, int B, int S, int rows, float* lse,
                                       float* w, float* loss_rows, hipStream_t stream);
int plb_launch_pack_token_targets(const int64_t* token_ids, const int32_t* lengths, const int32_t* row_start, int B, int S,
                                  int rows, int64_t* out, hipStream_t stream);
int plb_launch_add_scalar(float* out, const float* a, const float* b, hipStream_t stream);

int plb_launch_masked_report_rows(const float* logits, int ldl, int V, const int32_t* tgt, int n, int topk, int32_t* pred,
                                  int32_t* rank, float* nll, int32_t* topk_ids, float* topk_logprob, float* logits_out,
                                  hipStream_t stream);
int plb_launch_masked_report_samples(const int32_t* offsets, int B, const int32_t* rank, const float* nll, int topk,
                                     float* sample_loss, int32_t* sample_top1, int32_t* sample_topk, int32_t* totals,
                                     hipStream_t stream);
int plb_launch_token_top1(const float* pmax, int ntiles, const float* tlogit, const float* w, int rows, int32_t* scratch,
                          int32_t* totals2, hipStream_t stream);

typedef struct {
  const int64_t* labels; const int32_t* lengths;
  int B, S;
  uint64_t seed; uint32_t step;
  float word_pred_prob, mask_prob, replace_prob;
  int mask_id, sep_id;
  int64_t* masked; int32_t *counts, *idx_padded, *offsets, *flat;
} PlbMask;
int plb_launch_mask(const PlbMask* p, hipStream_t stream);

typedef struct {
  const int64_t* ids; const int32_t *sample_off, *word_off, *word_begin, *word_len; const int8_t* action;
  const int64_t* repl; const int64_t* word_token; int64_t sep_token; const int32_t* crop_start;
  int B, S, mask_id;
  int64_t *labels, *masked, *tokens; int32_t *lengths_out, *counts, *idx_padded, *offsets, *flat;
} PlbApplyMask;
int plb_launch_apply_mask(const PlbApplyMask* p, hipStream_t stream);

int plb_launch_adamw(float* p, const float* g, float* m, float* v, bf16_t* p_bf16, size_t n, double lr, double beta1,
                     double beta2, double eps, double wd, int step, double grad_scale, unsigned int* skip_if_nonzero,
                     int count_skip, hipStream_t stream);
#define PLB_NORM_PARTS 1024
static inline size_t plb_norm_chunk(size_t n) {
  return (n + (size_t)PLB_NORM_PARTS * 1024 - 1) / ((size_t)PLB_NORM_PARTS * 1024) * 1024;
}
#define PLB_NORM_CHAIN(n) (4 * (plb_norm_chunk(n) / 1024) + 6 + 3)
int plb_launch_grad_accum(float* accum, float* grads, size_t n, int phase, float* partials, hipStream_t stream);
int plb_launch_grad_sumsq(const float* grads, size_t n, float* partials, hipStream_t stream);
int plb_launch_grad_norm_finish(const float* partials, int nparts, double grad_scale, double max_norm, float* out,
                                hipStream_t stream);
int plb_launch_adamw_clipped(float* p, const float* g, float* m, float* v, bf16_t* p_bf16, size_t n, double lr, double beta1,
                             double beta2, double eps, double wd, int step, double grad_scale,
                             unsigned int* skip_if_nonzero, int count_skip, float* norm, int count_nonfinite,
                             hipStream_t stream);
int plb_launch_step_status(unsigned int* ln_err, float* loss, unsigned int* host_mirror, const float* summed, hipStream_t stream);
int plb_launch_status_export(const unsigned int* ln_err, float* out, hipStream_t stream);
int plb_launch_cast_bf16(const float* src, bf16_t* dst, size_t n, hipStream_t stream);
int plb_launch_transpose_cast(const float* src, int R, int C, bf16_t* dst, int ldd, hipStream_t stream);
int plb_launch_transpose_cast_multi(int n, const float* const* src, const int* R, const int* C, bf16_t* const* dst,
                                    const int* ldd, hipStream_t stream);
int plb_launch_bf16_to_f32(const bf16_t* src, int lds_, float* dst, int ldd, int R, int C, hipStream_t stream);

}
```

Measured before the change: 1.757 million tokens/s.

## Add half-ring 128x256 GEMM variant with higher occupancy for plain and GELU NT GEMMs

Adds a HALF template form of the big NT GEMM kernel that uses a 128x256 tile with a 5-slot LDS ring instead of 10, with launch bounds allowing 4 blocks per CU. The plain bf16 NT GEMM and the GELU-derivative-stash GEMMs (forward and backward) now route to this form by default when the tile grid is large. The engine tracks the chosen row tile so downstream partial-row counts match. The goal is more resident blocks and better wave-level latency hiding and tail balance. The cost is a shallower prefetch pipeline and smaller tiles, which means more operand traffic per FLOP.

```diff
diff --git a/plbert_amd/_lib.py b/plbert_amd/_lib.py
--- a/plbert_amd/_lib.py
+++ b/plbert_amd/_lib.py
@@ -232,6 +232,13 @@
     "plb_prof_end": (None, [i32, vp]),
     "plb_launch_gemm_nt_ln": (i32, [P(PlbGemmNT), i32, vp]),
     "plb_launch_gemm_nt_gelud": (i32, [P(PlbGemmNT), i32, vp]),
+    "plb_launch_gemm_nt_gelud_rows": (i32, [P(PlbGemmNT), i32, i32, vp]),
+    "plb_gemm_nt_gelud_tile_rows": (i32, [i32, i32, i32]),
+    "plb_launch_gemm_nt_half": (i32, [P(PlbGemmNT), i32, vp]),
+    "plb_set_gemm_nt_half_ring": (None, [i32]),
+    "plb_gemm_nt_half_ring": (i32, []),
+    "plb_gemm_nt_half_ring_takes": (i32, [i32, i32, i32, i32]),
+    "plb_gemm_nt_half_occupancy": (i32, [i32]),
     "plb_launch_gemm_nt_fp8": (i32, [P(PlbGemmNT), i32, i32, vp]),
     "plb_launch_gemm_nt_fp8_ln": (i32, [P(PlbGemmNT), i32, i32, vp]),
     "plb_launch_gemm_nt_fp8_gelud": (i32, [P(PlbGemmNT), i32, i32, vp]),
diff --git a/plbert_amd/build.py b/plbert_amd/build.py
--- a/plbert_amd/build.py
+++ b/plbert_amd/build.py
@@ -7,7 +7,7 @@
 HERE = os.path.dirname(os.path.abspath(__file__))
 CSRC = os.path.join(HERE, "csrc")
 LIB = os.path.join(HERE, "libplbert_hip.so")
-SOURCES = ["gemm.hip", "gemm_big.hip", "gemm_fp8.hip", "gemm_fp8_ln.hip", "gemm_tn_fp8.hip", "gemm_ln.hip", "attn.hip", "attn_bwd_fused.hip", "mask.hip",
+SOURCES = ["gemm.hip", "gemm_big.hip", "gemm_fp8.hip", "gemm_fp8_ln.hip", "gemm_tn_fp8.hip", "gemm_ln.hip", "gemm_half.hip", "attn.hip", "attn_bwd_fused.hip", "mask.hip",
            "embed.hip", "layernorm.hip", "reduce.hip", "loss_rows.hip", "eval_rows.hip", "optim.hip", "operand_images.hip",
            "engine.cpp", "engine_prof.cpp", "engine_comm.cpp", "engine_fp8.cpp", "engine_layers.cpp", "engine_calls.cpp", "engine_eval.cpp", "engine_optim.cpp"]
 HEADERS = ["exports.map", "common.h", "plbert_kernels.h", "gemm_epilogue.h", "gemm_nt_pipeline.h", "attn_common.h", "row_common.h", "engine_internal.h", os.path.join("..", "..", "include", "plbert.h")]
diff --git a/plbert_amd/csrc/engine_internal.h b/plbert_amd/csrc/engine_internal.h
--- a/plbert_amd/csrc/engine_internal.h
+++ b/plbert_amd/csrc/engine_internal.h
@@ -93,6 +93,7 @@
   int64_t o_f8amax = 0, o_f8scale = 0, o_f8deq = 0, o_f8stats = 0;
   bool fp8_on = false, fp8_ready = false, fp8_bwd_ready = false, fp8_wstale = true;
   bool u_is_derivative = false;
+  int gelud_rows = 256;
   bool tn8_call = false;
   int part_rows_used = 0;
   int pruned_rows = 0;
diff --git a/plbert_amd/csrc/engine_layers.cpp b/plbert_amd/csrc/engine_layers.cpp
--- a/plbert_amd/csrc/engine_layers.cpp
+++ b/plbert_amd/csrc/engine_layers.cpp
@@ -55,8 +55,8 @@
   PlbGemmNT q = f8_operands(g, f8);
   return plb_launch_gemm_nt_fp8_ln(&q, mode, f8->a_bf8, s);
 }
-static int gemm_nt_gelud_any(PlbGemmNT* g, int backward, const F8Op* f8, hipStream_t s) {
-  if (!f8) return plb_launch_gemm_nt_gelud(g, backward, s);
+static int gemm_nt_gelud_any(PlbGemmNT* g, int backward, int rows, const F8Op* f8, hipStream_t s) {
+  if (!f8) return plb_launch_gemm_nt_gelud_rows(g, backward, rows, s);
   PlbGemmNT q = f8_operands(g, f8);
   return plb_launch_gemm_nt_fp8_gelud(&q, backward, f8->a_bf8, s);
 }
@@ -95,6 +95,7 @@
 }
 static bool gelu_dstash(PlbEngine* e, int64_t Tp, bool f8_call) {
   e->u_is_derivative = e->gelu_dstash_on && (f8_call ? Tp % 128 == 0 : Tp % 256 == 0) && e->I % 256 == 0;
+  e->gelud_rows = (e->u_is_derivative && !f8_call) ? plb_gemm_nt_gelud_tile_rows((int)Tp, e->I, e->H) : 256;
   return e->u_is_derivative;
 }
 static void ln_fields(const PlbEngine* e, PlbGemmNT* g, const float* gamma, const float* beta, float* mean, float* rstd) {
@@ -267,7 +268,7 @@
     const F8Op o1 = f8_op(sl.a8, sA, F8Weight(e, F8W_1), 0);
     if (dstash) {
       if (tn8) { g.C2 = nullptr; g.ldc2 = 0; }
-      TRY(gemm_nt_gelud_any(&g, 0, f8 ? &o1 : nullptr, s));
+      TRY(gemm_nt_gelud_any(&g, 0, e->gelud_rows, f8 ? &o1 : nullptr, s));
     } else {
       TRY(gemm_nt_any(&g, 1, f8 ? &o1 : nullptr, s));
     }
@@ -336,7 +337,7 @@
   const F8Op ou = f8_op(sl.dp8, sDP, F8Weight(e, F8W_2T), 1);
   if (e->u_is_derivative) {
     if (e->tn8_call) g.C = nullptr;
-    TRY(gemm_nt_gelud_any(&g, 1, c.f8 ? &ou : nullptr, s));
+    TRY(gemm_nt_gelud_any(&g, 1, e->gelud_rows, c.f8 ? &ou : nullptr, s));
   } else {
     TRY(gemm_nt_any(&g, 2, c.f8 ? &ou : nullptr, s));
   }
@@ -438,7 +439,7 @@
   const int Tp = (int)c.Tp;
   c.f8 = f8_call(e, Tp, true);
   c.calib = e->fp8_on && !c.f8;
-  c.du_rows = e->u_is_derivative ? (c.f8 ? 2 * (Tp / plb_gemm_nt_fp8_gelud_tile_rows(Tp)) : 2 * (Tp / 256))
+  c.du_rows = e->u_is_derivative ? (c.f8 ? 2 * (Tp / plb_gemm_nt_fp8_gelud_tile_rows(Tp)) : 2 * (Tp / e->gelud_rows))
                                  : (c.f8 ? 2 * (Tp / 128) : plb_gemm_nt_colpart_rows(Tp, I, e->H));
   c.fuse_b = ln_fusable(e, Tp, 2);
   c.prows = c.fuse_b ? 2 * Tp / 128 : e->ln_blocks;
diff --git a/plbert_amd/csrc/gemm.hip b/plbert_amd/csrc/gemm.hip
--- a/plbert_amd/csrc/gemm.hip
+++ b/plbert_amd/csrc/gemm.hip
@@ -196,6 +196,7 @@
   if (g_nt_tile == 256) return ok256 ? 256 : 128;
   if (g_nt_tile == 384) return ok384 ? 384 : (ok256 ? 256 : 128);
   if (g_nt_tile == 1256) return ok1256 ? 1256 : 128;
+  if (g_nt_tile == 5256) return ok1256 ? 5256 : 128;
   if ((long)p->M * p->N < 256L * 256 * 64) return 128;
   double e256 = 0, e384 = 0, e1256 = 0;
   if (ok256) { const long t = (long)(p->M / 256) * (p->N / 256); e256 = (double)t / (double)(((t + 255) / 256) * 256); }
@@ -210,7 +211,7 @@
   PlbGemmNT q;
   q.M = M; q.N = N; q.K = K;
   const int tile = pick_tile(&q);
-  return tile == 256 ? 2 * (M / 256) : (tile == 384 || tile == 1256) ? 2 * (M / 128) : 0;
+  return tile == 256 ? 2 * (M / 256) : (tile == 384 || tile == 1256 || tile == 5256) ? 2 * (M / 128) : 0;
 }
 
 extern "C" int plb_launch_gemm_nt(const PlbGemmNT* p, int act, int out_f32, hipStream_t stream) {
@@ -218,7 +219,10 @@
   const int nbn = (p->N + BN - 1) / BN;
   dim3 grid((p->M / BM) * nbn), block(256);
   const int cls = out_f32 ? PLB_K_GEMM_NT_F32 : act == 1 ? PLB_K_GEMM_NT_GELU : act == 2 ? PLB_K_GEMM_NT_GELUBWD : PLB_K_GEMM_NT;
-  const int tile = pick_tile(p);
+  int tile = pick_tile(p);
+  const bool half_form = act == 0 && !out_f32 && !p->colpart && p->K % 64 == 0;
+  if (tile == 5256 && !half_form) tile = 1256;
+  if (g_nt_tile == 0 && half_form && plb_gemm_nt_half_ring_takes(p->M, p->N, p->K, 1)) tile = 5256;
   if (p->colpart && tile == 128) return 1;
   const double mnk = (double)p->M * p->N * p->K;
   const double algo_bytes = 2.0 * ((double)p->M * p->K + (double)p->N * p->K) +
diff --git a/plbert_amd/csrc/gemm_big.hip b/plbert_amd/csrc/gemm_big.hip
--- a/plbert_amd/csrc/gemm_big.hip
+++ b/plbert_amd/csrc/gemm_big.hip
@@ -259,6 +259,7 @@
 extern "C" void plb_set_gemm_nt_prefetch(int on) { g_nt_prefetch = on; }
 
 extern "C" int plb_launch_gemm_nt_big(const PlbGemmNT* p, int tile, int act, int out_f32, hipStream_t stream) {
+  if (tile == 5256) return (act == 0 && !out_f32) ? plb_launch_gemm_nt_half(p, 0, stream) : 1;
   const bool pf = g_nt_prefetch < 0 ? (tile != 256 || act != 0) : (g_nt_prefetch != 0);
   if (pf)
     return tile == 384 ? launch_big<3, true>(p, act, out_f32, stream)
diff --git a/plbert_amd/csrc/gemm_half.hip b/plbert_amd/csrc/gemm_half.hip
--- /dev/null
+++ b/plbert_amd/csrc/gemm_half.hip
@@ -0,0 +1,44 @@
+#include <cstdlib>
+#include "gemm_nt_pipeline.h"
+
+static constexpr int HALF_DEFAULT = 3;
+static int g_half_mode = -1;
+extern "C" void plb_set_gemm_nt_half_ring(int mode) { g_half_mode = mode; }
+extern "C" int plb_gemm_nt_half_ring(void) {
+  static const int env = [] { const char* v = getenv("PLBERT_NT_HALF_RING"); return v ? atoi(v) : HALF_DEFAULT; }();
+  return g_half_mode < 0 ? env : g_half_mode;
+}
+extern "C" int plb_gemm_nt_half_ring_takes(int M, int N, int K, int cls) {
+  const int mode = plb_gemm_nt_half_ring();
+  if (!(mode & cls) || M <= 0 || N <= 0 || K <= 0 || M % 128 || N % 256 || K % 64) return 0;
+  return (mode & 4) || (long)(M / 128) * (N / 256) >= 512;
+}
+
+extern "C" int plb_launch_gemm_nt_half(const PlbGemmNT* p, int act, hipStream_t stream) {
+  if (p->M % 128 || p->N % 256 || p->K % 64 || p->M <= 0 || p->N <= 0 || p->K <= 0) return 1;
+  dim3 grid((p->M / 128) * (p->N / 256)), block(512);
+  if (act == 0) {
+    if (p->colpart || !p->C) return 1;
+    hipLaunchKernelGGL((gemm_nt_big_kernel<1, 0, false, false, false, false, true, true>), grid, block, 0, stream, *p);
+  } else if (act == 7) {
+    if (!p->C || !p->C2) return 1;
+    if (p->colpart) hipLaunchKernelGGL((gemm_nt_big_kernel<1, 7, false, false, false, false, false, true>), grid, block, 0, stream, *p);
+    else hipLaunchKernelGGL((gemm_nt_big_kernel<1, 7, false, false, false, false, true, true>), grid, block, 0, stream, *p);
+  } else if (act == 8) {
+    if (!p->C || !p->aux) return 1;
+    hipLaunchKernelGGL((gemm_nt_big_kernel<1, 8, false, false, false, false, false, true>), grid, block, 0, stream, *p);
+  } else {
+    return 1;
+  }
+  return hipGetLastError() == hipSuccess ? 0 : 2;
+}
+
+extern "C" int plb_gemm_nt_half_occupancy(int act) {
+  int n = -1;
+  hipError_t rc = hipErrorInvalidValue;
+  if (act == 0) rc = hipOccupancyMaxActiveBlocksPerMultiprocessor(&n, gemm_nt_big_kernel<1, 0, false, false, false, false, true, true>, 512, 0);
+  else if (act == 7) rc = hipOccupancyMaxActiveBlocksPerMultiprocessor(&n, gemm_nt_big_kernel<1, 7, false, false, false, false, true, true>, 512, 0);
+  else if (act == 17) rc = hipOccupancyMaxActiveBlocksPerMultiprocessor(&n, gemm_nt_big_kernel<1, 7, false, false, false, false, false, true>, 512, 0);
+  else if (act == 8) rc = hipOccupancyMaxActiveBlocksPerMultiprocessor(&n, gemm_nt_big_kernel<1, 8, false, false, false, false, false, true>, 512, 0);
+  return rc == hipSuccess ? n : -1;
+}
diff --git a/plbert_amd/csrc/gemm_ln.hip b/plbert_amd/csrc/gemm_ln.hip
--- a/plbert_amd/csrc/gemm_ln.hip
+++ b/plbert_amd/csrc/gemm_ln.hip
@@ -30,13 +30,23 @@
   return hipGetLastError() == hipSuccess ? 0 : 2;
 }
 
+extern "C" int plb_gemm_nt_gelud_tile_rows(int M, int N, int K) { return plb_gemm_nt_half_ring_takes(M, N, K, 2) ? 128 : 256; }
 extern "C" int plb_launch_gemm_nt_gelud(const PlbGemmNT* p, int backward, hipStream_t stream) {
-  if (p->M % 256 || p->N % 256 || p->K % 64 || p->M <= 0 || p->N <= 0 || p->K <= 0) return 3;
+  return plb_launch_gemm_nt_gelud_rows(p, backward, 256, stream);
+}
+extern "C" int plb_launch_gemm_nt_gelud_rows(const PlbGemmNT* p, int backward, int tile_rows, hipStream_t stream) {
+  if (tile_rows != 128 && tile_rows != 256) return 1;
+  if (p->M % tile_rows || p->N % 256 || p->K % 64 || p->M <= 0 || p->N <= 0 || p->K <= 0) return 3;
   if (!p->C || (!backward && !p->C2) || (backward && !p->aux)) return 1;
   dim3 grid((p->M / 256) * (p->N / 256)), block(512);
   const double mnk = (double)p->M * p->N * p->K;
   const double bytes = 2.0 * ((double)p->M * p->K + (double)p->N * p->K) + 4.0 * p->M * p->N;
   const int tok = plb_prof_begin(backward ? PLB_K_GEMM_NT_GELUBWD : PLB_K_GEMM_NT_GELU, stream, 2.0 * mnk, bytes);
+  if (tile_rows == 128) {
+    const int rc = plb_launch_gemm_nt_half(p, backward ? 8 : 7, stream);
+    plb_prof_end(tok, stream);
+    return rc;
+  }
   if (backward) hipLaunchKernelGGL((gemm_nt_big_kernel<2, 8, false, true>), grid, block, 0, stream, *p);
   else if (p->colpart) hipLaunchKernelGGL((gemm_nt_big_kernel<2, 7, false, true>), grid, block, 0, stream, *p);
   else hipLaunchKernelGGL((gemm_nt_big_kernel<2, 7, false, true, false, false, true>), grid, block, 0, stream, *p);
diff --git a/plbert_amd/csrc/gemm_nt_pipeline.h b/plbert_amd/csrc/gemm_nt_pipeline.h
--- a/plbert_amd/csrc/gemm_nt_pipeline.h
+++ b/plbert_amd/csrc/gemm_nt_pipeline.h
@@ -29,7 +29,9 @@
 
 constexpr int HT = 128 * 64;
 constexpr int RING = 10;
-DEVI int ring_slot(int x) { return x >= 2 * RING ? x - 2 * RING : (x >= RING ? x - RING : x); }
+constexpr int RING_HALF = 5;
+template <int R = RING>
+DEVI int ring_slot(int x) { return x >= 2 * R ? x - 2 * R : (x >= R ? x - R : x); }
 
 typedef __attribute__((address_space(1))) const void* gptr_t;
 typedef __attribute__((address_space(3))) void* lptr_t;
@@ -41,13 +43,15 @@
   } while (0)
 #define PIN() __builtin_amdgcn_sched_barrier(0)
 
-template <int V, int ACT, bool OUTF32, bool PF, bool FP8 = false, bool ABF8 = false, bool NOCS = false>
-__global__ __launch_bounds__(512) void gemm_nt_big_kernel(PlbGemmNT p) {
+template <int V, int ACT, bool OUTF32, bool PF, bool FP8 = false, bool ABF8 = false, bool NOCS = false, bool HALF = false>
+__global__ __launch_bounds__(512, HALF ? 4 : 2) void gemm_nt_big_kernel(PlbGemmNT p) {
+  static_assert(!HALF || (V == 1 && !PF && !FP8), "half-ring form: 128x256 tile, staggered loop, bf16 operands");
+  constexpr int NSLOT = HALF ? RING_HALF : RING;
   constexpr int NAH = (V == 2) ? 2 : 1;
   constexpr int NBH = (V == 3) ? 3 : 2;
   constexpr int TM = NAH * 128, TN = NBH * 128;
   constexpr int NH = NAH + NBH;
-  __shared__ __attribute__((aligned(16))) bf16_t smem[RING * HT];
+  __shared__ __attribute__((aligned(16))) bf16_t smem[NSLOT * HT];
   int tid = threadIdx.x, lane = tid & 63;
   const int uw = __builtin_amdgcn_readfirstlane(tid >> 6);
   const int wm = uw >> 2, wn = uw & 3;
@@ -101,7 +105,7 @@
   } while (0)
 #define ISSUE(c)                                                          \
   do {                                                                    \
-    if (NH * t + (c) < htot) STAGE_I((c) % NH, ring_slot(rb + (c)), t + (c) / NH); \
+    if (NH * t + (c) < htot) STAGE_I((c) % NH, ring_slot<NSLOT>(rb + (c)), t + (c) / NH); \
   } while (0)
 
   int frow = lane & 15, fq = lane >> 4;
@@ -170,7 +174,11 @@
 
   const int htot = NH * nk;
   int rb = 0;
-  {
+  if constexpr (HALF) {
+    const int t = 0;
+    ISSUE(0); ISSUE(1); ISSUE(2); ISSUE(3);
+    LANDED(htot > 3, 4);
+  } else {
     const int t = 0;
     ISSUE(0); ISSUE(1); ISSUE(2); ISSUE(3); ISSUE(4); ISSUE(5); ISSUE(6); ISSUE(7); ISSUE(8);
     if constexpr (V == 2) {
@@ -287,7 +295,17 @@
   if (wm == 1) BARRIER();
 
   for (int t = 0; t < nk; ++t) {
-    if constexpr (V == 1) {
+    if constexpr (HALF) {
+      ISSUE(4);
+      LANDED(NH * t + 4 < htot, 4);
+      READ_B(0, ring_slot<NSLOT>(rb + 1));
+      READ_A(0, ring_slot<NSLOT>(rb));
+      MFMA_PART(0, 0, 0);
+      ISSUE(5); ISSUE(6);
+      LANDED(NH * t + 6 < htot, 4);
+      READ_B(1, ring_slot<NSLOT>(rb + 2));
+      MFMA_PART(0, 1, 1);
+    } else if constexpr (V == 1) {
       ISSUE(9);
       READ_B(0, ring_slot(rb + 1));
       READ_A(0, ring_slot(rb));
@@ -323,7 +341,7 @@
       MFMA_PART(0, 2, 0);
     }
     rb += NH;
-    rb = rb >= RING ? rb - RING : rb;
+    rb = rb >= NSLOT ? rb - NSLOT : rb;
   }
   if (wm == 0) BARRIER();
   }
@@ -356,7 +374,7 @@
   constexpr int OROW_PAD = 8;
   constexpr int OROW = TN + OROW_PAD;
   constexpr bool OUT_NT = ACT == 1 || ACT == 2 || ACT == 5 || ACT == 6 || ACT == 7 || ACT == 8;
-  static_assert(TM * OROW <= RING * HT, "output image must fit the ring");
+  static_assert(TM * OROW <= NSLOT * HT, "output image must fit the ring");
   f32x4 csum[NBH][2];
   float4 bz[NBH][2];
 #pragma unroll
@@ -451,7 +469,7 @@
     constexpr int R2OFF = IMG + 128 * 4 * 2 * 4 + 128 * 2 * 4;
     constexpr int GAMOFF = R2OFF + 64 * OROW * 2;
     constexpr int TAB3OFF = GAMOFF + TN * 4;
-    static_assert(GAMOFF + (ACT == 6 ? TN * 4 : 0) + (LEAN ? 1024 : 0) <= RING * HT * 2, "staging regions must fit the LDS");
+    static_assert(GAMOFF + (ACT == 6 ? TN * 4 : 0) + (LEAN ? 1024 : 0) <= NSLOT * HT * 2, "staging regions must fit the LDS");
     float* const tab3 = reinterpret_cast<float*>(reinterpret_cast<char*>(smem) + TAB3OFF);
     if constexpr (LEAN) {
       if (tid < TM) { tab3[tid * 2] = p.ln_mean[bm * TM + tid]; tab3[tid * 2 + 1] = p.ln_rstd[bm * TM + tid]; }
@@ -750,7 +768,7 @@
     return;
   }
   uint4* const lane_stash = reinterpret_cast<uint4*>(ACT == 7 ? p.C : const_cast<bf16_t*>(p.aux));
-  constexpr int SQD = 3;
+  constexpr int SQD = HALF ? 2 : 3;
   uint4 sq[SQD + 1][NBH];
   uint2 keep[NAH][4][NBH][2];
   uint32_t k8[NAH][4][NBH][2];
diff --git a/plbert_amd/csrc/plbert_kernels.h b/plbert_amd/csrc/plbert_kernels.h
--- a/plbert_amd/csrc/plbert_kernels.h
+++ b/plbert_amd/csrc/plbert_kernels.h
@@ -50,6 +50,13 @@
 } PlbGemmNT;
 int plb_launch_gemm_nt_ln(const PlbGemmNT* p, int mode, hipStream_t stream);
 int plb_launch_gemm_nt_gelud(const PlbGemmNT* p, int backward, hipStream_t stream);
+int plb_launch_gemm_nt_gelud_rows(const PlbGemmNT* p, int backward, int tile_rows, hipStream_t stream);
+int plb_gemm_nt_gelud_tile_rows(int M, int N, int K);
+int plb_launch_gemm_nt_half(const PlbGemmNT* p, int act, hipStream_t stream);
+void plb_set_gemm_nt_half_ring(int mode);
+int plb_gemm_nt_half_ring(void);
+int plb_gemm_nt_half_ring_takes(int M, int N, int K, int cls);
+int plb_gemm_nt_half_occupancy(int act);
 int plb_launch_gemm_nt_fp8(const PlbGemmNT* p, int act, int a_bf8, hipStream_t stream);
 int plb_launch_gemm_nt_fp8_ln(const PlbGemmNT* p, int mode, int a_bf8, hipStream_t stream);
 int plb_launch_gemm_nt_fp8_gelud(const PlbGemmNT* p, int backward, int a_bf8, hipStream_t stream);
```

Result: no change. 1.764 million tokens/s, median of 6 (+0.4%).
